# skhu101/TDNN-F_NAS

Hardware: AMD Instinct MI355X
Metric: LF-MMI training frames/sec per node (SWBD 7q TDNN-F) (higher is better)
Workload: dtype f32

## Files before the change

include/tdnnf_hip.h:

```cpp
#ifndef TDNNF_HIP_H_
#define TDNNF_HIP_H_

#include <stddef.h>
#include <stdint.h>

#ifdef __cplusplus
extern "C" {
#endif

#define TDNNF_OK 0
#define TDNNF_EINVAL 1
#define TDNNF_EHIP 2

#define TDNNF_MAX_OFFSETS 16

typedef struct {
  float *data;
  int rows, cols, stride;
} tdnnf_mat;

typedef void *tdnnf_stream;
typedef struct tdnnf_ng tdnnf_ng;

const char *tdnnf_last_error(void);
int tdnnf_abi_version(void);
int tdnnf_set_option(const char *name, int value);
int tdnnf_get_option(const char *name, int *value_out);

#define TDNNF_DARTS_USE_GUMBEL 1
#define TDNNF_DARTS_FREE_SELECT 2
#define TDNNF_DARTS_UNIFORM_SAMPLE 4
#define TDNNF_DARTS_USE_ENTROPY 8
#define TDNNF_DARTS_UPDATE_ALPHA 16

typedef struct {
  int row_stride;
  int num_offsets;
  int row_offsets[TDNNF_MAX_OFFSETS];
} tdnnf_tdnn_indexes;


int tdnnf_tdnn_darts_coef(const float *log_alpha_dev, int K, int flags, float temp_proportion,
                          const float *gumbel_u_dev, const float *sample_u_dev, int share_index,
                          float *coef_memo_dev, float *eff_coef_dev, tdnnf_stream stream);

int tdnnf_tdnn_propagate(const tdnnf_tdnn_indexes *indexes, const tdnnf_mat *in,
                         const float *linear_params_dev, int ldw, int Do, int Di,
                         const float *bias_dev, const float *eff_coef_dev, int init_mode,
                         tdnnf_mat *out, tdnnf_stream stream);

int tdnnf_tdnn_backprop_data(const tdnnf_tdnn_indexes *indexes, const tdnnf_mat *out_deriv,
                             const float *linear_params_dev, int ldw, int Do, int Di,
                             const float *eff_coef_dev, tdnnf_mat *in_deriv, tdnnf_stream stream);

size_t tdnnf_tdnn_update_workspace_bytes(int Do, int Di, int K, int num_rows);
int tdnnf_tdnn_update_simple(const tdnnf_tdnn_indexes *indexes, const tdnnf_mat *in_value,
                             const tdnnf_mat *out_deriv, int Do, int Di,
                             const float *eff_coef_dev, float lr, float *W_acc_dev, int ldw,
                             float *bias_acc_dev, void *workspace_dev, size_t workspace_bytes,
                             tdnnf_stream stream);

#define TDNNF_TAP_DOTS_SLABS 64
#define TDNNF_TAP_DOTS_DOUBLES(K) ((K) * (1 + TDNNF_TAP_DOTS_SLABS))

int tdnnf_tdnn_darts_alpha_update(const float *tap_grad_dev, int ldg, const float *linear_params_dev,
                                  int ldw, int Do, int Di, int K, const float *coef_memo_dev,
                                  int flags, int share_index, float temp_proportion, float lr,
                                  float *alpha_acc_dev, double *tap_dots_dev ,
                                  tdnnf_stream stream);

size_t tdnnf_tdnn_update_natural_gradient_workspace_bytes(int Do, int Di, int K, int num_rows, int has_bias);
int tdnnf_tdnn_update_natural_gradient(const tdnnf_tdnn_indexes *indexes, const tdnnf_mat *in_value,
                                       const tdnnf_mat *out_deriv, int Do, int Di,
                                       const float *linear_params_dev, int ldw_params,
                                       const float *coef_memo_dev, const float *eff_coef_dev, int flags,
                                       int share_index, float temp_proportion,
                                       tdnnf_ng *preconditioner_in, tdnnf_ng *preconditioner_out,
                                       float learning_rate, float *W_acc_dev, int ldw, float *bias_acc_dev,
                                       float *alpha_acc_dev, void *workspace_dev, size_t workspace_bytes,
                                       tdnnf_stream stream);


size_t tdnnf_colreduce_workspace_bytes(int rows, int cols);

int tdnnf_batchnorm_propagate(const tdnnf_mat *in, float epsilon, float target_rms, tdnnf_mat *out,
                              float *memo_dev, void *workspace_dev, size_t workspace_bytes, tdnnf_stream stream);
int tdnnf_batchnorm_backprop(const tdnnf_mat *out_value, const tdnnf_mat *out_deriv, float target_rms,
                             float *memo_dev, tdnnf_mat *in_deriv, void *workspace_dev, size_t workspace_bytes,
                             tdnnf_stream stream);
int tdnnf_batchnorm_store_stats(const float *memo_dev, int D, int num_frames, double *stats_dev,
                                tdnnf_stream stream);
int tdnnf_batchnorm_compute_derived(const double *stats_dev, int D, float epsilon, float target_rms,
                                    float *scale_dev, float *offset_dev, tdnnf_stream stream);
int tdnnf_batchnorm_test_propagate(const tdnnf_mat *in, const float *scale_dev, const float *offset_dev,
                                   tdnnf_mat *out, tdnnf_stream stream);
int tdnnf_batchnorm_test_backprop(const tdnnf_mat *out_deriv, const float *scale_dev, tdnnf_mat *in_deriv,
                                  tdnnf_stream stream);


int tdnnf_softmax_flops_propagate(const tdnnf_mat *in, const float *gumbel_u_dev, float temp_proportion,
                                  tdnnf_mat *out, tdnnf_stream stream);
int tdnnf_softmax_flops_backprop(const tdnnf_mat *out_value, tdnnf_mat *out_deriv, float scale,
                                 const float *flops_dev, int dim, float temp_proportion,
                                 tdnnf_mat *in_deriv, tdnnf_stream stream);
int tdnnf_onehot_propagate(const float *sample_u_dev, tdnnf_mat *out, tdnnf_stream stream);
int tdnnf_onehot_backprop(const tdnnf_mat *out_deriv, float lr, float *output_acc_dev, void *workspace_dev,
                          size_t workspace_bytes, tdnnf_stream stream);
int tdnnf_copyn_propagate(const tdnnf_mat *in, float scale, tdnnf_mat *out, tdnnf_stream stream);
int tdnnf_copyn_backprop(const tdnnf_mat *out_deriv, float scale, tdnnf_mat *in_deriv, tdnnf_stream stream);
int tdnnf_constant_function_propagate(const float *output_dev, tdnnf_mat *out, tdnnf_stream stream);
int tdnnf_constant_function_backprop(const tdnnf_mat *out_deriv, float lr, float *output_acc_dev,
                                     void *workspace_dev, size_t workspace_bytes, tdnnf_stream stream);
int tdnnf_flops_constraint_backprop(const float *flops_dev, float scale, int rows_in, int cols_in,
                                    tdnnf_mat *in_deriv, tdnnf_stream stream);

int tdnnf_elementwise_product_propagate(const tdnnf_mat *in, int output_dim, tdnnf_mat *out, tdnnf_stream);
int tdnnf_elementwise_product_backprop(const tdnnf_mat *in_value, const tdnnf_mat *out_deriv, int output_dim,
                                       tdnnf_mat *in_deriv, tdnnf_stream);
int tdnnf_relu_propagate(const tdnnf_mat *in, tdnnf_mat *out, tdnnf_stream);
int tdnnf_relu_backprop(const tdnnf_mat *out_value, const tdnnf_mat *out_deriv, tdnnf_mat *in_deriv, tdnnf_stream);
int tdnnf_relu_repair(const double *stats_dev, int dim, float self_repair_scale, float lower, float upper,
                      tdnnf_mat *in_deriv, tdnnf_stream);
int tdnnf_relu_store_stats(const tdnnf_mat *out_value, double *stats_dev, void *workspace_dev,
                           size_t workspace_bytes, tdnnf_stream);
int tdnnf_affine_propagate(const tdnnf_mat *in, const float *W_dev, int ldw, const float *bias_dev, int Do,
                           tdnnf_mat *out, tdnnf_stream);
int tdnnf_affine_backprop(const tdnnf_mat *out_deriv, const float *W_dev, int ldw, int Di, tdnnf_mat *in_deriv,
                          tdnnf_stream);
int tdnnf_affine_update_simple(const tdnnf_mat *in_value, const tdnnf_mat *out_deriv, float lr, float *W_acc_dev,
                               int ldw, float *bias_acc_dev, void *workspace_dev, size_t workspace_bytes,
                               tdnnf_stream);
size_t tdnnf_affine_update_natural_gradient_workspace_bytes(int Do, int Di, int num_rows, int has_bias);
int tdnnf_affine_update_natural_gradient(const tdnnf_mat *in_value, const tdnnf_mat *out_deriv,
                                         tdnnf_ng *preconditioner_in, tdnnf_ng *preconditioner_out,
                                         float learning_rate, float *W_acc_dev, int ldw, float *bias_acc_dev,
                                         void *workspace_dev, size_t workspace_bytes, tdnnf_stream);
int tdnnf_log_softmax_propagate(const tdnnf_mat *in, tdnnf_mat *out, tdnnf_stream);
int tdnnf_log_softmax_backprop(const tdnnf_mat *out_value, const tdnnf_mat *out_deriv, tdnnf_mat *in_deriv,
                               tdnnf_stream);
int tdnnf_sum_scaled(const tdnnf_mat *a, float sa, const tdnnf_mat *b, float sb, tdnnf_mat *out, tdnnf_stream);
int tdnnf_add_scaled(const tdnnf_mat *a, float s, tdnnf_mat *out, tdnnf_stream);
int tdnnf_general_dropout(const tdnnf_mat *in, const float *mask_dev, int num_seq, tdnnf_mat *out, tdnnf_stream);
int tdnnf_general_dropout_mask(const float *uniform_dev, long long n, float proportion, int continuous, float *mask_dev, tdnnf_stream);

typedef struct tdnnf_den_graph tdnnf_den_graph;
typedef struct tdnnf_supervision tdnnf_supervision;

int tdnnf_den_graph_create(int num_states, int num_arcs, int num_pdfs, const int *arc_src, const int *arc_dst,
                           const int *arc_pdf, const float *arc_prob, const float *initial_probs, int start_state,
                           tdnnf_den_graph **out);
void tdnnf_den_graph_destroy(tdnnf_den_graph *);
int tdnnf_supervision_create(int num_sequences, int frames_per_sequence, const int *seq_state_begin,
                             const int *seq_arc_begin, const int *state_time, const float *final_logprob,
                             const int *arc_src, const int *arc_dst, const int *arc_pdf, const float *arc_logprob,
                             float weight, tdnnf_supervision **out);
void tdnnf_supervision_destroy(tdnnf_supervision *);
int tdnnf_supervision_info(const tdnnf_supervision *, int *num_states, int *num_arcs, int *max_states_per_frame, int *wide);

int tdnnf_chain_set_denominator_mode(int mode);
int tdnnf_chain_den_mw_status(int *fallbacks, int *disabled, int reset);
size_t tdnnf_chain_workspace_bytes(const tdnnf_den_graph *, int num_sequences, int frames_per_sequence);
int tdnnf_chain_objf_and_deriv(const tdnnf_den_graph *, const tdnnf_supervision *, const tdnnf_mat *nnet_output,
                               const tdnnf_mat *xent_output , float leaky_hmm_coefficient,
                               float l2_regularize, float xent_regularize, double *results_dev,
                               tdnnf_mat *nnet_output_deriv, tdnnf_mat *xent_deriv, void *workspace_dev,
                               size_t workspace_bytes, tdnnf_stream);
int tdnnf_chain_numerator_part(const tdnnf_den_graph *, const tdnnf_supervision *, const tdnnf_mat *nnet_output, int part, double *results_dev,
                               tdnnf_mat *nnet_output_deriv, tdnnf_mat *xent_deriv, void *workspace_dev, size_t workspace_bytes, tdnnf_stream);

int tdnnf_ng_create(int rank, int update_period, float num_samples_history, float alpha, tdnnf_ng **out);
void tdnnf_ng_destroy(tdnnf_ng *);
int tdnnf_ng_freeze(tdnnf_ng *, int freeze);
int tdnnf_ng_precondition(tdnnf_ng *, tdnnf_mat *X, float *scale_host, tdnnf_stream);
size_t tdnnf_ng_stats_pass_workspace_bytes(int rank, int Di, int num_taps, int N);
int tdnnf_ng_stats_pass(const tdnnf_tdnn_indexes *ix, const tdnnf_mat *X, int Di, const float *eff_dev, const float *WT_dev,
                        const float *W_dev, int ldw, const float *bias_dev, tdnnf_mat *H, double *sumsq_dev, int sumsq_cap, int form,
                        void *workspace_dev, size_t workspace_bytes, tdnnf_stream);
const float *tdnnf_ng_scale_dev(const tdnnf_ng *);

size_t tdnnf_constrain_orthonormal_workspace_bytes(int rows, int cols);
int tdnnf_constrain_orthonormal(float scale, float *M_dev, int rows, int cols, int ld, void *workspace_dev,
                                size_t workspace_bytes, tdnnf_stream);
int tdnnf_axpy(const float *x_dev, float a, float *y_dev, size_t n, tdnnf_stream);
int tdnnf_dot(const float *x_dev, const float *y_dev, size_t n, double *result_host, tdnnf_stream);
size_t tdnnf_max_change_workspace_bytes(int num_comp);
int tdnnf_update_with_max_change(float *params_dev, float *delta_dev, int num_comp, const long long *comp_begin_host,
                                 const float *max_change_host, float max_param_change, float max_change_scale,
                                 float scale, int zero_delta, void *workspace_dev, size_t workspace_bytes,
                                 float *info_dev, tdnnf_stream);

int tdnnf_splice_input(const tdnnf_mat *feats, const tdnnf_mat *ivectors, int num_seq, int num_splice,
                       tdnnf_mat *out, tdnnf_stream);
int tdnnf_reorder_rows(const tdnnf_mat *in, int num_seq, int rho, int to_rho, tdnnf_mat *out, tdnnf_stream);

#define TDNNF_NET_MAX_LAYERS 32
typedef struct {
  int feat_dim, ivector_dim, num_pdfs;
  int hidden_dim, prefinal_small_dim;
  int num_layers;
  int bottleneck_dim[TDNNF_NET_MAX_LAYERS];
  int time_stride[TDNNF_NET_MAX_LAYERS];
  float bypass_scale;
  int frames_per_chunk, num_sequences;
  int frame_subsampling;
  float leaky_hmm, xent_regularize, chain_l2_regularize;
  float l2_hidden, l2_output;
// ... 121 lines not shown
```

tdnn-f_nas_amd/csrc/abi_tdnn.hip:

```cpp
#include <dlfcn.h>
#include <stdlib.h>
#include <string.h>

#include <string>

#include "common.h"
#include "gemm_f32.h"
#include "planes_gemm.h"

namespace tdnnf {

static thread_local std::string g_last_error;

void set_error(const char *fmt, ...) {
  char buf[1024];
  va_list ap;
  va_start(ap, fmt);
  vsnprintf(buf, sizeof(buf), fmt, ap);
  va_end(ap);
  g_last_error = buf;
}
int hip_status(hipError_t e, const char *what) {
  set_error("HIP error %d (%s) in %s", (int)e, hipGetErrorString(e), what);
  return TDNNF_EHIP;
}

Options &options() {
  static Options o;
  return o;
}

namespace {
typedef int (*roctx_push_t)(const char *);
typedef int (*roctx_pop_t)();
roctx_push_t g_roctx_push = nullptr;
roctx_pop_t g_roctx_pop = nullptr;
bool roctx_ready() {
  static const bool ok = [] {
    const char *e = getenv("TDNNF_ROCTX");
    if (e && atoi(e) == 0) return false;
    for (const char *lib : {"librocprofiler-sdk-roctx.so", "librocprofiler-sdk-roctx.so.1", "libroctx64.so", "libroctx64.so.4"}) {
      void *h = dlopen(lib, RTLD_NOW | RTLD_GLOBAL);
      if (!h) continue;
      g_roctx_push = (roctx_push_t)dlsym(h, "roctxRangePushA");
      g_roctx_pop = (roctx_pop_t)dlsym(h, "roctxRangePop");
      if (g_roctx_push && g_roctx_pop) return true;
    }
    return false;
  }();
  return ok;
}
}
TraceRange::TraceRange(const char *name) : on(roctx_ready()) {
  if (on) g_roctx_push(name);
}
TraceRange::~TraceRange() {
  if (on) g_roctx_pop();
}

static bool tdnn_rows_ok(const tdnnf_tdnn_indexes *ix, int rows_in, int N) {
  if (!ix || ix->num_offsets < 1 || ix->num_offsets > TDNNF_MAX_OFFSETS || ix->row_stride < 1) return false;
  for (int i = 0; i < ix->num_offsets; i++) {
    const long long need = (long long)ix->row_offsets[i] + (long long)ix->row_stride * N - (ix->row_stride - 1);
    if (ix->row_offsets[i] < 0 || (N > 0 && rows_in < need)) return false;
  }
  return true;
}

}

using namespace tdnnf;

extern "C" {

const char *tdnnf_last_error(void) { return g_last_error.c_str(); }
int tdnnf_abi_version(void) { return 1; }

static int *option_slot(const char *name) {
  Options &o = options();
  if (!name) return nullptr;
  const struct { const char *n; int *p; } table[] = {{"ng_grouped", &o.ng_grouped}, {"ng_fuse", &o.ng_fuse}, {"ng_early_in", &o.ng_early_in},
                                                     {"wgrad_stream", &o.wgrad_stream}, {"gemm_ring", &o.gemm_ring}, {"planes", &o.planes}, {"den_split", &o.den_split}, {"phase_events", &o.phase_events}, {"wgrad_lag", &o.wgrad_lag}, {"ng_bk", &o.ng_bk}, {"ng_valu", &o.ng_valu}, {"ng_pform", &o.ng_pform}, {"planes_group", &o.planes_group}, {"xent_behind_den", &o.xent_behind_den}, {"ng_early_fork", &o.ng_early_fork}, {"ng_diag_skip", &o.ng_diag_skip}, {"wgrad_small", &o.wgrad_small}, {"splitk_per_cu", &o.splitk_per_cu}, {"gemm_alt_taps", &o.gemm_alt_taps}, {"reverse_passes", &o.reverse_passes}, {"splitk_partial_round", &o.splitk_partial_round}, {"wgrad_on_caller", &o.wgrad_on_caller}, {"den_mw_test_abort", &o.den_mw_test_abort}, {"planes_check_bound", &o.planes_check_bound}, {"den_gamma_pairs", &o.den_gamma_pairs}, {"num_form", &o.num_form}, {"num_frontier_cap", &o.num_frontier_cap}};
  for (auto &e : table)
    if (strcmp(e.n, name) == 0) return e.p;
  return nullptr;
}
int tdnnf_set_option(const char *name, int value) {
  int *p = option_slot(name);
  TDNNF_REQUIRE(p, "set_option: unknown option '%s' (ng_grouped, ng_fuse, ng_early_in, wgrad_stream, gemm_ring, planes, den_split)", name ? name : "(null)");
  *p = value;
  return TDNNF_OK;
}
int tdnnf_get_option(const char *name, int *value) {
  int *p = option_slot(name);
  TDNNF_REQUIRE(p && value, "get_option: unknown option '%s'", name ? name : "(null)");
  *value = *p;
  return TDNNF_OK;
}

}

namespace tdnnf {
int tdnn_propagate_impl(const tdnnf_tdnn_indexes *ix, const tdnnf_mat *in, const float *W, int ldw, int Do, int Di,
                        const float *bias, const float *eff_coef, int init_mode, int relu, tdnnf_mat *out, tdnnf_stream stream,
                        float *colstats, int *colstats_rows) {
  TDNNF_REQUIRE(mat_ok(in) && mat_ok(out) && W, "tdnn_propagate: bad matrices");
  TDNNF_REQUIRE(Do > 0 && Di > 0 && in->cols == Di && out->cols == Do, "tdnn_propagate: dims: in.cols=%d Di=%d out.cols=%d Do=%d",
                in ? in->cols : -1, Di, out ? out->cols : -1, Do);
  TDNNF_REQUIRE(tdnn_rows_ok(ix, in->rows, out->rows), "tdnn_propagate: input has too few rows for the time offsets");
  TDNNF_REQUIRE(ldw >= ix->num_offsets * Di, "tdnn_propagate: ldw < K*Di");
  TDNNF_REQUIRE(init_mode >= 0 && init_mode <= 2 && (init_mode != 1 || bias), "tdnn_propagate: init_mode 1 needs a bias");
  RowsGemmArgs a;
  memset(&a, 0, sizeof(a));
  a.A = in->data;
  a.lda = (long long)in->stride * ix->row_stride;
  a.B = W;
  a.ldb = ldw;
  a.C = out->data;
  a.ldc = out->stride;
  a.M = out->rows;
  a.N = Do;
  a.bias = bias;
  a.coef = eff_coef;
  a.init_mode = init_mode;
  a.relu = relu;
  a.colstats = colstats;
  a.colstats_rows = colstats_rows;
  a.nseg = ix->num_offsets;
  for (int i = 0; i < a.nseg; i++) {
    a.seg[i].a_off = (long long)ix->row_offsets[i] * in->stride;
    a.seg[i].b_off = (long long)i * Di;
    a.seg[i].klen = Di;
    a.seg[i].m_lo = 0;
    a.seg[i].m_hi = out->rows;
  }
  TDNNF_HIP(rows_gemm(a, true, (hipStream_t)stream));
  return TDNNF_OK;
}
}

extern "C" {

int tdnnf_tdnn_propagate(const tdnnf_tdnn_indexes *ix, const tdnnf_mat *in, const float *W, int ldw, int Do, int Di,
                         const float *bias, const float *eff_coef, int init_mode, tdnnf_mat *out, tdnnf_stream stream) {
  return tdnn_propagate_impl(ix, in, W, ldw, Do, Di, bias, eff_coef, init_mode, 0, out, stream);
}

}

namespace tdnnf {
int tdnn_backprop_data_impl(const tdnnf_tdnn_indexes *ix, const tdnnf_mat *out_deriv, const float *W, int ldw, int Do,
                            int Di, const float *eff_coef, int overwrite, const tdnnf_mat *add, float add_scale, int add_lo,
                            tdnnf_mat *in_deriv, tdnnf_stream stream) {
  TDNNF_REQUIRE(mat_ok(in_deriv) && mat_ok(out_deriv) && W, "tdnn_backprop_data: bad matrices");
  TDNNF_REQUIRE(Do > 0 && Di > 0 && in_deriv->cols == Di && out_deriv->cols == Do, "tdnn_backprop_data: bad dims");
  TDNNF_REQUIRE(tdnn_rows_ok(ix, in_deriv->rows, out_deriv->rows), "tdnn_backprop_data: in_deriv has too few rows for the time offsets");
  TDNNF_REQUIRE(ldw >= ix->num_offsets * Di, "tdnn_backprop_data: ldw < K*Di");
  const int rho = ix->row_stride, N = out_deriv->rows, K = ix->num_offsets;
  if (N == 0) return TDNNF_OK;
  for (int cls = 0; cls < rho; cls++) {
    RowsGemmArgs a;
    memset(&a, 0, sizeof(a));
    float cf_dummy = 0;
    (void)cf_dummy;
    int nseg = 0, u_max = 0;
    int seg_tap[kMaxSeg];
    for (int i = 0; i < K; i++) {
      if (ix->row_offsets[i] % rho != cls) continue;
      const int shift = (ix->row_offsets[i] - cls) / rho;
      a.seg[nseg].a_off = -(long long)shift * out_deriv->stride;
      a.seg[nseg].b_off = (long long)i * Di;
      a.seg[nseg].klen = Do;
      a.seg[nseg].m_lo = shift;
      a.seg[nseg].m_hi = shift + N;
      if (shift + N > u_max) u_max = shift + N;
      seg_tap[nseg] = i;
      nseg++;
    }
    if (nseg == 0) continue;
    bool contiguous = true;
    for (int s = 1; s < nseg; s++) contiguous = contiguous && seg_tap[s] == seg_tap[s - 1] + 1;
    a.A = out_deriv->data;
    a.lda = out_deriv->stride;
    a.B = W;
    a.ldb = ldw;
    const float *WT = (ldw == K * Di && !planes_hint_b()) ? transposed_weights(W) : nullptr;
    if (WT) {
      a.B = WT;
      a.ldb = Do;
      for (int sg = 0; sg < nseg; sg++) a.seg[sg].b_off = (long long)seg_tap[sg] * Di * Do;
    }
    a.C = in_deriv->data + (long long)cls * in_deriv->stride;
    a.ldc = (long long)in_deriv->stride * rho;
    a.M = u_max;
    a.N = Di;
    a.init_mode = 0;
    if (overwrite) {
      TDNNF_REQUIRE(rho == 1 && u_max == in_deriv->rows, "tdnn_backprop_data: overwrite needs row_stride 1 and full row coverage");
      a.init_mode = 2;
    }
    if (add) {
      TDNNF_REQUIRE(rho == 1 && add->cols == Di && add_lo >= 0 && add_lo + add->rows <= in_deriv->rows, "tdnn_backprop_data: bad addend");
      a.add = add->data;
      a.ldadd = add->stride;
      a.add_scale = add_scale;
      a.add_lo = add_lo;
      a.add_hi = add_lo + add->rows;
    }
    TDNNF_REQUIRE(!(overwrite || add) || !eff_coef || contiguous, "tdnn_backprop_data: fused overwrite/addend needs a single launch");
    if (!eff_coef || contiguous) {
      a.coef = eff_coef ? eff_coef + seg_tap[0] : nullptr;
      a.nseg = nseg;
      TDNNF_HIP(rows_gemm(a, WT != nullptr, (hipStream_t)stream));
    } else {
      for (int s = 0; s < nseg; s++) {
        RowsGemmArgs b = a;
        b.seg[0] = a.seg[s];
        b.nseg = 1;
        b.coef = eff_coef + seg_tap[s];
        b.M = a.seg[s].m_hi;
        TDNNF_HIP(rows_gemm(b, WT != nullptr, (hipStream_t)stream));
      }
    }
  }
  return TDNNF_OK;
}
}

extern "C" {

int tdnnf_tdnn_backprop_data(const tdnnf_tdnn_indexes *ix, const tdnnf_mat *out_deriv, const float *W, int ldw, int Do,
                             int Di, const float *eff_coef, tdnnf_mat *in_deriv, tdnnf_stream stream) {
  return tdnn_backprop_data_impl(ix, out_deriv, W, ldw, Do, Di, eff_coef, 0, nullptr, 0.f, 0, in_deriv, stream);
}

size_t tdnnf_tdnn_update_workspace_bytes(int Do, int Di, int K, int num_rows) {
  return wgrad_workspace_bytes(Do, Di, K, num_rows);
}

}

namespace tdnnf {
int tdnn_update_simple_impl(const tdnnf_tdnn_indexes *ix, const tdnnf_mat *in_value, const tdnnf_mat *out_deriv, int Do,
                            int Di, const float *eff_coef, float lr, float *W_acc, int ldw, float *bias_acc, void *ws,
                            size_t ws_bytes, const int *active_dev, int max_active, tdnnf_stream stream, bool overwrite) {
  TDNNF_REQUIRE(mat_ok(in_value) && mat_ok(out_deriv) && W_acc, "tdnn_update_simple: bad matrices");
  TDNNF_REQUIRE(Do > 0 && Di > 0 && in_value->cols == Di && out_deriv->cols == Do, "tdnn_update_simple: bad dims");
  TDNNF_REQUIRE(tdnn_rows_ok(ix, in_value->rows, out_deriv->rows), "tdnn_update_simple: in_value has too few rows for the time offsets");
  TDNNF_REQUIRE(ldw >= ix->num_offsets * Di, "tdnn_update_simple: ldw < K*Di");
  if (out_deriv->rows == 0) return TDNNF_OK;
  TDNNF_REQUIRE(ws && ws_bytes >= wgrad_workspace_bytes(Do, Di, ix->num_offsets, out_deriv->rows), "tdnn_update_simple: workspace too small");
  WgradArgs a;
  memset(&a, 0, sizeof(a));
  a.dY = out_deriv->data;
  a.lddy = out_deriv->stride;
  a.X = in_value->data;
  a.ldx = in_value->stride;
  a.Do = Do;
  a.Di = Di;
  a.K = ix->num_offsets;
  a.N = out_deriv->rows;
  a.row_stride = ix->row_stride;
  for (int i = 0; i < a.K; i++) a.row_offsets[i] = ix->row_offsets[i];
  a.coef = eff_coef;
  a.scale = lr;
  a.G = W_acc;
  a.ldg = ldw;
  a.accumulate = overwrite ? 0 : 1;
  a.bias_acc = bias_acc;
  a.active = active_dev;
  a.max_active = max_active;
  TDNNF_HIP(wgrad(a, ws, ws_bytes, (hipStream_t)stream));
  return TDNNF_OK;
}
}

extern "C" {

int tdnnf_tdnn_update_simple(const tdnnf_tdnn_indexes *ix, const tdnnf_mat *in_value, const tdnnf_mat *out_deriv, int Do,
                             int Di, const float *eff_coef, float lr, float *W_acc, int ldw, float *bias_acc, void *ws,
                             size_t ws_bytes, tdnnf_stream stream) {
  return tdnn_update_simple_impl(ix, in_value, out_deriv, Do, Di, eff_coef, lr, W_acc, ldw, bias_acc, ws, ws_bytes, nullptr, 0, stream);
}

int tdnnf_affine_propagate(const tdnnf_mat *in, const float *W, int ldw, const float *bias, int Do, tdnnf_mat *out,
                           tdnnf_stream stream) {
  TDNNF_REQUIRE(mat_ok(in) && mat_ok(out) && W && Do > 0 && out->cols == Do && in->rows == out->rows && ldw >= in->cols,
                "affine_propagate: bad arguments");
  tdnnf_tdnn_indexes ix;
  memset(&ix, 0, sizeof(ix));
  ix.row_stride = 1;
  ix.num_offsets = 1;
  return tdnnf_tdnn_propagate(&ix, in, W, ldw, Do, in->cols, bias, nullptr, bias ? 1 : 2, out, stream);
}

int tdnnf_affine_backprop(const tdnnf_mat *out_deriv, const float *W, int ldw, int Di, tdnnf_mat *in_deriv, tdnnf_stream stream) {
  TDNNF_REQUIRE(mat_ok(out_deriv) && mat_ok(in_deriv) && W && Di > 0 && in_deriv->cols == Di && in_deriv->rows == out_deriv->rows && ldw >= Di,
                "affine_backprop: bad arguments");
  if (out_deriv->rows == 0) return TDNNF_OK;
  RowsGemmArgs a;
  memset(&a, 0, sizeof(a));
  a.A = out_deriv->data;
  a.lda = out_deriv->stride;
  a.B = W;
  a.ldb = ldw;
  const float *WT = (ldw == Di && !planes_hint_b()) ? transposed_weights(W) : nullptr;
  if (WT) {
    a.B = WT;
    a.ldb = out_deriv->cols;
  }
  a.C = in_deriv->data;
  a.ldc = in_deriv->stride;
  a.M = out_deriv->rows;
  a.N = Di;
  a.init_mode = 2;
  a.nseg = 1;
  a.seg[0].klen = out_deriv->cols;
  a.seg[0].m_lo = 0;
  a.seg[0].m_hi = out_deriv->rows;
  TDNNF_HIP(rows_gemm(a, WT != nullptr, (hipStream_t)stream));
  return TDNNF_OK;
}

int tdnnf_affine_update_simple(const tdnnf_mat *in_value, const tdnnf_mat *out_deriv, float lr, float *W_acc, int ldw,
                               float *bias_acc, void *ws, size_t ws_bytes, tdnnf_stream stream) {
  TDNNF_REQUIRE(mat_ok(in_value) && mat_ok(out_deriv) && in_value->rows == out_deriv->rows, "affine_update_simple: bad matrices");
  tdnnf_tdnn_indexes ix;
  memset(&ix, 0, sizeof(ix));
  ix.row_stride = 1;
  ix.num_offsets = 1;
  return tdnnf_tdnn_update_simple(&ix, in_value, out_deriv, out_deriv->cols, in_value->cols, nullptr, lr, W_acc, ldw,
                                  bias_acc, ws, ws_bytes, stream);
}

}
```

tdnn-f_nas_amd/csrc/common.h:

```cpp
#pragma once
#include <hip/hip_runtime.h>
#include <stdarg.h>
#include <stdio.h>

#include "tdnnf_hip.h"

namespace tdnnf {

struct MatView {
  float *data;
  int rows, cols, stride;
};
inline MatView view(const tdnnf_mat *m) { return MatView{m->data, m->rows, m->cols, m->stride}; }

void set_error(const char *fmt, ...);
int hip_status(hipError_t e, const char *what);

inline bool mat_ok(const tdnnf_mat *m) {
  return m && m->rows >= 0 && m->cols >= 0 && m->stride >= m->cols && (m->data || m->rows * m->cols == 0);
}
inline bool same_dim(const tdnnf_mat *a, const tdnnf_mat *b) { return a->rows == b->rows && a->cols == b->cols; }

inline bool vec4_ok(const MatView &m) {
  return (reinterpret_cast<uintptr_t>(m.data) & 15) == 0 && m.stride % 4 == 0 && m.cols % 4 == 0;
}

#define TDNNF_REQUIRE(cond, ...)            \
  do {                                      \
    if (!(cond)) {                          \
      ::tdnnf::set_error(__VA_ARGS__);      \
      return TDNNF_EINVAL;                  \
    }                                       \
  } while (0)

#define TDNNF_HIP(expr)                                         \
  do {                                                          \
    hipError_t e__ = (expr);                                    \
    if (e__ != hipSuccess) return ::tdnnf::hip_status(e__, #expr); \
  } while (0)

#define TDNNF_LAUNCH_CHECK(name) TDNNF_HIP(hipGetLastError())

struct Options {
  int ng_grouped = 1;
  int ng_fuse = 1;
  int ng_early_in = 1;
  int wgrad_stream = -1;
  int gemm_ring = 1;
  int planes = 1;
  int den_mw_test_abort = 0;
  int planes_group = 1;
  int planes_check_bound = 0;
  int wgrad_lag = 3;
  int wgrad_on_caller = 0;
  int splitk_partial_round = 1;
  int reverse_passes = 0;
  int gemm_alt_taps = 1;
  int splitk_per_cu = 2;
  int wgrad_small = 0;
  int ng_bk = 0;
  int ng_early_fork = 1;
  int xent_behind_den = -1;
  int ng_pform = 1;
  int ng_valu = 0;
  int ng_diag_skip = 0;
  int phase_events = 0;
  int den_split = -1;
  int num_form = 0;
  int num_frontier_cap = 0;
  int den_gamma_pairs = 0;
};
Options &options();

struct TraceRange {
  explicit TraceRange(const char *name);
  ~TraceRange();
  bool on;
};

__host__ __device__ inline float floor_keep_nan(float x, float f) { return x < f ? f : x; }

inline int grid_for(long long work, int block, int cap = 2048) {
  long long g = (work + block - 1) / block;
  if (g > cap) g = cap;
  if (g < 1) g = 1;
  return (int)g;
}

inline unsigned long long tdnnf_decision(unsigned long long step, unsigned long long k) {
  unsigned long long z = step * 0x9E3779B97F4A7C15ULL + k * 0xBF58476D1CE4E5B9ULL + 0x94D049BB133111EBULL;
  z = (z ^ (z >> 30)) * 0xBF58476D1CE4E5B9ULL;
  z = (z ^ (z >> 27)) * 0x94D049BB133111EBULL;
  return (z ^ (z >> 31)) >> 8;
}

constexpr int kFinCols = 8, kFinLanes = 32, kFinThreads = kFinCols * kFinLanes;
inline unsigned finalize_grid(int D) { return (unsigned)((D + kFinCols - 1) / kFinCols); }
#ifdef __HIPCC__
template <int NQ, class Acc>
__device__ __forceinline__ void finalize_sums(const float *partial, int chunks, long long qstride_rows, int D, int nq, Acc (&q)[NQ], Acc *red) {
  const int tc = threadIdx.x & (kFinCols - 1), lane = threadIdx.x / kFinCols, d = blockIdx.x * kFinCols + tc;
#pragma unroll
  for (int k = 0; k < NQ; k++) q[k] = 0;
  if (d < D) {
    const float *p = partial + d;
    const long long qs = qstride_rows * D;
    int c = lane;
    for (; c + 3 * kFinLanes < chunks; c += 4 * kFinLanes) {
      float v[NQ][4];
#pragma unroll
      for (int k = 0; k < NQ; k++) {
        if (k < nq) {
          const float *pk = p + (long long)k * qs;
          v[k][0] = pk[(long long)c * D]; v[k][1] = pk[(long long)(c + kFinLanes) * D];
          v[k][2] = pk[(long long)(c + 2 * kFinLanes) * D]; v[k][3] = pk[(long long)(c + 3 * kFinLanes) * D];
        }
      }
#pragma unroll
      for (int k = 0; k < NQ; k++) {
        if (k < nq) { q[k] += v[k][0]; q[k] += v[k][1]; q[k] += v[k][2]; q[k] += v[k][3]; }
      }
    }
    for (; c < chunks; c += kFinLanes) {
      float v[NQ];
#pragma unroll
      for (int k = 0; k < NQ; k++)
        if (k < nq) v[k] = p[(long long)k * qs + (long long)c * D];
#pragma unroll
      for (int k = 0; k < NQ; k++)
        if (k < nq) q[k] += v[k];
    }
  }
#pragma unroll
  for (int k = 0; k < NQ; k++) red[(k * kFinLanes + lane) * (kFinCols + 1) + tc] = q[k];
  __syncthreads();
  if (lane == 0) {
#pragma unroll
    for (int k = 0; k < NQ; k++) {
      Acc s = 0;
      for (int l = 0; l < kFinLanes; l++) s += red[(k * kFinLanes + l) * (kFinCols + 1) + tc];
      q[k] = s;
    }
  }
}
#endif

struct BnSync {
  int (*fn)(void *ctx, double *buf, long long count, tdnnf_stream stream);
  void *ctx;
  double *buf;
  int world;
};
BnSync *bn_sync_current();
struct BnSyncScope {
  BnSync *prev;
  explicit BnSyncScope(BnSync *b);
  ~BnSyncScope();
};

struct FroBoundScope {
  double *prev_buf;
  int *prev_blocks;
  FroBoundScope(double *buf, int *blocks);
  ~FroBoundScope();
};
double *fro_bound_buf();
int *fro_bound_blocks();

struct ColReducePlan {
  int chunks, rows_per_chunk;
};
ColReducePlan colreduce_plan(int rows, int cols);
size_t colreduce_bytes(int rows, int cols);
hipError_t colreduce_partial(int kind, MatView a, MatView b, float *partial, hipStream_t s);
hipError_t colreduce_partial_into(int kind, MatView a, MatView b, int chunks, int rows_per_chunk, int sq_row_offset, float *partial, hipStream_t s);
hipError_t batchnorm_stats_from_partials(const float *partial, int chunks, int rows, int cols, float epsilon, float target_rms, float *memo, hipStream_t s,
                                         double *store_stats = nullptr);
hipError_t batchnorm_stats(MatView a, float epsilon, float target_rms, float *memo, void *ws, hipStream_t s, double *store_stats = nullptr);
hipError_t colsum_add(MatView a, float scale, float *acc, void *ws, hipStream_t s);

bool log_softmax_propagate_with_aux(const tdnnf_mat *in, tdnnf_mat *out, tdnnf_mat *aux, float aux_scale, hipStream_t s);
float chain_supervision_weight(const tdnnf_supervision *sp);
size_t chain_split_region_bytes(const tdnnf_den_graph *g, int B, int T);
int chain_den(const tdnnf_den_graph *g, const tdnnf_supervision *sp, const tdnnf_mat *y, float leaky, tdnnf_mat *deriv, void *ws, hipStream_t s,
              bool beside_other_work = false, hipStream_t caller_aux = nullptr, hipEvent_t ev_recursions = nullptr, bool *ev_recorded = nullptr);
int chain_num_recursion(const tdnnf_supervision *sp, const tdnnf_den_graph *g, const tdnnf_mat *y, void *ws, hipStream_t s);
int chain_num_xent(const tdnnf_den_graph *g, const tdnnf_supervision *sp, const tdnnf_mat *y, const tdnnf_mat *xent_output, float xent_regularize,
                   tdnnf_mat *xent_deriv, void *ws, hipStream_t s, bool xent_deriv_initialised = false);
int chain_num(const tdnnf_den_graph *g, const tdnnf_supervision *sp, const tdnnf_mat *y, const tdnnf_mat *xent_output,
              float xent_regularize, tdnnf_mat *xent_deriv, void *ws, hipStream_t s, bool xent_deriv_initialised = false);
int chain_finish(const tdnnf_den_graph *g, const tdnnf_supervision *sp, const tdnnf_mat *y, float l2_regularize, double *results,
                 tdnnf_mat *deriv, tdnnf_mat *xent_deriv, void *ws, hipStream_t s);

int tdnn_propagate_impl(const tdnnf_tdnn_indexes *ix, const tdnnf_mat *in, const float *W, int ldw, int Do, int Di,
                        const float *bias, const float *eff_coef, int init_mode, int relu, tdnnf_mat *out, tdnnf_stream stream,
                        float *colstats = nullptr, int *colstats_rows = nullptr);
int tdnn_update_simple_impl(const tdnnf_tdnn_indexes *ix, const tdnnf_mat *in_value, const tdnnf_mat *out_deriv, int Do, int Di,
                            const float *eff_coef, float lr, float *W_acc, int ldw, float *bias_acc, void *ws, size_t ws_bytes,
                            const int *active_dev, int max_active, tdnnf_stream stream, bool overwrite = false);
int tdnn_backprop_data_impl(const tdnnf_tdnn_indexes *ix, const tdnnf_mat *out_deriv, const float *W, int ldw, int Do, int Di,
                            const float *eff_coef, int overwrite, const tdnnf_mat *add, float add_scale, int add_lo,
                            tdnnf_mat *in_deriv, tdnnf_stream stream);

}
```

tdnn-f_nas_amd/csrc/fused.h:

```cpp
#pragma once
#include "common.h"

namespace tdnnf {

struct PlanesSink {
  void *P;
  long long R;
  const float *rec;
};
hipError_t bn_apply_bypass(MatView x, const float *memo, int D, int period, MatView prev, float bypass, MatView out, hipStream_t s,
                           const float *mask = nullptr, int B = 1, const PlanesSink *planes = nullptr);

struct BwdPlanes {
  void *P;
  long long R;
  int lead;
  float *rec;
};

struct NgFuse {
  const float *W;
  int Rp, ldw;
  float *H;
  double *part;
  int part_cap;
};
bool bn_relu_bwd_ng_ok(MatView x, MatView dz, MatView d_aff, int Rp);
bool bn_relu_bwd_ng_pays(int rows);

size_t bn_relu_bwd_workspace_bytes(int rows, int cols);
hipError_t bn_relu_bwd(MatView x, MatView dz, float *memo, float target_rms, bool bn_test_mode, double *relu_stats, bool store_relu_stats,
                       bool self_repair, float self_repair_scale, MatView d_aff, float *bias_acc, float bias_scale,
                       void *ws, size_t ws_bytes, hipStream_t s, const float *mask = nullptr, int B = 1,
                       const NgFuse *ng = nullptr,
                       double *oderiv_stats = nullptr,
                       const BwdPlanes *planes = nullptr);

}
```

tdnn-f_nas_amd/csrc/fused.hip:

```cpp
#include <algorithm>

#include "common.h"
#include "device.h"
#include "fused.h"
#include "gemm_f32.h"
#include "planes_gemm.h"

namespace tdnnf {
namespace {

__device__ __forceinline__ void ld(const float *p, float (&v)[4], bool vec) {
  if (vec) {
    const float4 t = *reinterpret_cast<const float4 *>(p);
    v[0] = t.x; v[1] = t.y; v[2] = t.z; v[3] = t.w;
  } else {
    v[0] = p[0];
  }
}
__device__ __forceinline__ void st(float *p, const float (&v)[4], bool vec) {
  if (vec) *reinterpret_cast<float4 *>(p) = make_float4(v[0], v[1], v[2], v[3]);
  else p[0] = v[0];
}

__device__ __forceinline__ void store_planes4(const PlanesSink &pk, float ps, long long ra, int c, const float (&v)[4]) {
// ... 277 lines not shown
      wv[j] = make_float4(0.f, 0.f, 0.f, 0.f);
      if (n < ng.Rp) wv[j] = *reinterpret_cast<const float4 *>(ng.W + (long long)n * ng.ldw + k0 + kk);
    }
  };
  request(0);
  for (int k0 = 0; k0 < D; k0 += BK) {
    const int col = k0 + c4 * 4;
    const float4 mu = mu_n, sc = sc_n, vdm = vdm_n, tmp = tmp_n;
    float rep[4] = {0.f, 0.f, 0.f, 0.f};
    if (repairing) {
#pragma unroll
      for (int j = 0; j < 4; j++) {
        const float stv = (float)stv_n[j];
        const float v = (stv - 0.05f * count > 0.f ? 1.f : 0.f) + (stv - 0.95f * count > 0.f ? 1.f : 0.f) - 1.f;
        rep[j] = v * (-self_repair_scale / 0.5f);
      }
    }
    const float mu_[4] = {mu.x, mu.y, mu.z, mu.w}, sc_[4] = {sc.x, sc.y, sc.z, sc.w}, vdm_[4] = {vdm.x, vdm.y, vdm.z, vdm.w},
                tmp_[4] = {tmp.x, tmp.y, tmp.z, tmp.w};
    float cs[4] = {0.f, 0.f, 0.f, 0.f};
    float o[4][4];
#pragma unroll
    for (int i = 0; i < 4; i++) {
      const int r = r0 + rr + 32 * i;
#pragma unroll
      for (int j = 0; j < 4; j++) o[i][j] = 0.f;
      if (FULL || r < x.rows) {
        if (MASK) {
          const float *mk = mask + (long long)(r % B) * x.cols + col;
#pragma unroll
          for (int j = 0; j < 4; j++) dv[i][j] *= mk[j];
        }
#pragma unroll
        for (int j = 0; j < 4; j++) {
          const float z = (xv[i][j] - mu_[j]) * sc_[j];
          const float dr = (dv[i][j] + tmp_[j]) * sc_[j] + z * vdm_[j];
          float v = (xv[i][j] > 0.f ? 1.f : 0.f) * dr;
          if (rep[j] != 0.f) v += rep[j];
          o[i][j] = v;
          cs[j] += v;
          ssq += v * v;
        }
      }
      *reinterpret_cast<float4 *>(As + (rr + 32 * i) * LD + c4 * 4) = make_float4(o[i][0], o[i][1], o[i][2], o[i][3]);
    }
#pragma unroll
    for (int j = 0; j < NT; j++) {
      const int idx = t + 256 * j, n = idx >> 3, kk = (idx & 7) * 4;
      *reinterpret_cast<float4 *>(Bs + n * LD + kk) = wv[j];
    }
    if (k0 + BK < D) request(k0 + BK);
#pragma unroll
    for (int i = 0; i < 4; i++) {
      const int r = r0 + rr + 32 * i;
      if (FULL || r < x.rows) {
        st(d_aff.data + (long long)r * d_aff.stride + col, o[i], true);
        if constexpr (PLANES) store_planes4(pk, pks, (long long)pk_lead + r, col, o[i]);
      }
    }
#pragma unroll
    for (int j = 0; j < 4; j++) {
      float v = cs[j];
      v += __shfl_xor(v, 8, 64);
      v += __shfl_xor(v, 16, 64);
      v += __shfl_xor(v, 32, 64);
      if (lane < 8) colred[wave][lane * 4 + j] = v;
    }
    __syncthreads();
    {
      const float *as = As + (wave * 32 + li) * LD + lh * 4;
      const float *bs = Bs + li * LD + lh * 4;
#pragma unroll
      for (int kg = 0; kg < BK / 8; kg++) {
        const float4 a = *reinterpret_cast<const float4 *>(as + kg * 8);
#pragma unroll
        for (int j = 0; j < NT; j++) {
          const float4 b = *reinterpret_cast<const float4 *>(bs + j * 32 * LD + kg * 8);
          acc[j] = __builtin_amdgcn_mfma_f32_32x32x2f32(a.x, b.x, acc[j], 0, 0, 0);
          acc[j] = __builtin_amdgcn_mfma_f32_32x32x2f32(a.y, b.y, acc[j], 0, 0, 0);
          acc[j] = __builtin_amdgcn_mfma_f32_32x32x2f32(a.z, b.z, acc[j], 0, 0, 0);
          acc[j] = __builtin_amdgcn_mfma_f32_32x32x2f32(a.w, b.w, acc[j], 0, 0, 0);
        }
      }
    }
    if (t < BK) partial[(long long)blk * D + k0 + t] = (colred[0][t] + colred[1][t]) + (colred[2][t] + colred[3][t]);
    __syncthreads();
  }
#pragma unroll
  for (int j = 0; j < NT; j++) {
    const int n = j * 32 + li;
#pragma unroll
    for (int e = 0; e < 16; e++) {
      const int r = r0 + wave * 32 + (e & 3) + 8 * (e >> 2) + 4 * lh;
      if (n < ng.Rp && r < x.rows) ng.H[(long long)r * ng.Rp + n] = acc[j][e];
    }
  }
  double v = ssq;
  for (int o = 32; o > 0; o >>= 1) v += __shfl_xor(v, o, 64);
  if (lane == 0) red[wave] = v;
  __syncthreads();
  if (t == 0) ng.part[blk] = (red[0] + red[1]) + (red[2] + red[3]);
  if (blk == 0)
    for (int i = gridDim.x + t; i < ng.part_cap; i += 256) ng.part[i] = 0.0;
}

template <int NT, bool MASK, bool PLANES>
__global__ __launch_bounds__(256) void bn_relu_bwd_apply_ng_kernel(MatView x, MatView dz, const float *memo, int D, const double *repair_stats,
                                                                   float self_repair_scale, MatView d_aff, float *partial, const float *mask, int B,
                                                                   NgFuse ng, PlanesSink pk, int pk_lead, int rev) {
  const int blk = rev ? (int)gridDim.x - 1 - (int)blockIdx.x : (int)blockIdx.x;
  if (blk * 128 + 128 <= x.rows)
    bn_relu_bwd_apply_ng_body<NT, MASK, true, PLANES>(x, dz, memo, D, repair_stats, self_repair_scale, d_aff, partial, mask, B, ng, pk, pk_lead, blk);
  else bn_relu_bwd_apply_ng_body<NT, MASK, false, PLANES>(x, dz, memo, D, repair_stats, self_repair_scale, d_aff, partial, mask, B, ng, pk, pk_lead, blk);
}

__global__ __launch_bounds__(kFinThreads) void colsum_add_kernel(const float *partial, int chunks, int D, float scale, float *acc) {
  __shared__ float red[kFinLanes * (kFinCols + 1)];
  const int d = blockIdx.x * kFinCols + (threadIdx.x & (kFinCols - 1));
  float q[1];
  finalize_sums<1, float>(partial, chunks, chunks, D, 1, q, red);
  if (threadIdx.x < kFinCols && d < D) acc[d] += scale * q[0];
}

}

hipError_t bn_apply_bypass(MatView x, const float *memo, int D, int period, MatView prev, float bypass, MatView out, hipStream_t s, const float *mask, int B,
                           const PlanesSink *planes) {
  if (x.rows == 0) return hipSuccess;
  const bool vec = vec4_ok(x) && vec4_ok(out) && (!prev.data || vec4_ok(prev)) && D % 4 == 0 && (reinterpret_cast<uintptr_t>(memo) & 15) == 0 &&
                   (!mask || (reinterpret_cast<uintptr_t>(mask) & 15) == 0);
  const long long work = (long long)x.rows * (vec ? x.cols / 4 : x.cols);
  if (planes && !(vec && x.cols == D && D % 32 == 0 && planes->P && planes->rec)) return hipErrorInvalidValue;
  ProfHbmRange prof(4, 4.0 * x.rows * x.cols * ((prev.data ? 3.0 : 2.0) + (planes ? 1.0 : 0.0)), s);
  const PlanesSink none{nullptr, 0, nullptr};
  if (planes) hipLaunchKernelGGL((bn_apply_bypass_kernel<4, true>), dim3(grid_for((long long)((x.rows + 7) / 8) * 8 * (x.cols / 4), 256)), dim3(256), 0, s, x, memo, memo + 2 * D, D, period, prev, bypass, out, mask, B, *planes, 0);
  else if (vec) hipLaunchKernelGGL((bn_apply_bypass_kernel<4, false>), dim3(grid_for(work, 256)), dim3(256), 0, s, x, memo, memo + 2 * D, D, period, prev, bypass, out, mask, B, none, options().reverse_passes & 1);
  else hipLaunchKernelGGL((bn_apply_bypass_kernel<1, false>), dim3(grid_for(work, 256)), dim3(256), 0, s, x, memo, memo + 2 * D, D, period, prev, bypass, out, mask, B, none, 0);
  return hipGetLastError();
}

bool bn_relu_bwd_ng_ok(MatView x, MatView dz, MatView d_aff, int Rp) {
  return vec4_ok(x) && vec4_ok(dz) && vec4_ok(d_aff) && x.cols % 32 == 0 && Rp >= 1 && Rp <= 96 && x.rows >= 1;
}

bool bn_relu_bwd_ng_pays(int rows) {
  const int slots = 2 * device_cus();
  const int blocks = (rows + 127) / 128, rounds = (blocks + slots - 1) / slots;
  return 4 * blocks >= 3 * rounds * slots;
}

size_t bn_relu_bwd_workspace_bytes(int rows, int cols) {
  ColReducePlan p = colreduce_plan(rows, cols);
  const size_t blocks128 = ((size_t)rows + 127) / 128;
  return sizeof(float) * (5 * (size_t)p.chunks + std::max((size_t)p.chunks, blocks128)) * cols + 64;
}

hipError_t bn_relu_bwd(MatView x, MatView dz, float *memo, float target_rms, bool bn_test_mode, double *relu_stats, bool store_relu_stats,
                       bool self_repair, float self_repair_scale, MatView d_aff, float *bias_acc, float bias_scale,
                       void *ws, size_t ws_bytes, hipStream_t s, const float *mask, int B, const NgFuse *ng, double *oderiv_stats, const BwdPlanes *planes) {
  if (x.rows == 0) return hipSuccess;
  if (ws_bytes < bn_relu_bwd_workspace_bytes(x.rows, x.cols)) return hipErrorInvalidValue;
  if (ng && (!bn_relu_bwd_ng_ok(x, dz, d_aff, ng->Rp) || (reinterpret_cast<uintptr_t>(memo) & 15) || (reinterpret_cast<uintptr_t>(ng->W) & 15) || ng->ldw % 4))
    return hipErrorInvalidValue;
  const int D = x.cols;
  ProfHbmRange prof(5, 4.0 * x.rows * x.cols * 5.0, s);
  ColReducePlan pl = colreduce_plan(x.rows, D);
  const bool vec = vec4_ok(x) && vec4_ok(dz) && vec4_ok(d_aff);
  const int per = vec ? 256 : 64;
  dim3 grid((D + per - 1) / per, pl.chunks), block(256);
  float *partial = (float *)ws;
  float *bias_partial = partial + 5 * (size_t)pl.chunks * D;
  if (store_relu_stats) {
    if (vec) hipLaunchKernelGGL((bn_relu_bwd_reduce_kernel<4, true>), grid, block, 0, s, x, dz, memo, memo + 2 * D, pl.rows_per_chunk, pl.chunks, partial, mask, B);
    else hipLaunchKernelGGL((bn_relu_bwd_reduce_kernel<1, true>), grid, block, 0, s, x, dz, memo, memo + 2 * D, pl.rows_per_chunk, pl.chunks, partial, mask, B);
  } else {
    if (vec) hipLaunchKernelGGL((bn_relu_bwd_reduce_kernel<4, false>), grid, block, 0, s, x, dz, memo, memo + 2 * D, pl.rows_per_chunk, pl.chunks, partial, mask, B);
    else hipLaunchKernelGGL((bn_relu_bwd_reduce_kernel<1, false>), grid, block, 0, s, x, dz, memo, memo + 2 * D, pl.rows_per_chunk, pl.chunks, partial, mask, B);
  }
  double *fro2 = fro_bound_buf();
  if (fro2 && fro_bound_blocks()) *fro_bound_blocks() = (int)finalize_grid(D);
  const float repair_abs = self_repair ? 2.0f * fabsf(self_repair_scale) : 0.f;
  if (BnSync *sy = bn_test_mode ? nullptr : bn_sync_current()) {
    hipLaunchKernelGGL(bn_relu_bwd_finalize_kernel, dim3(finalize_grid(D)), dim3(kFinThreads), 0, s, partial, pl.chunks, D, x.rows, target_rms, memo,
                       store_relu_stats ? relu_stats : (double *)nullptr, 0, (double *)nullptr, sy->buf, (const double *)nullptr, 0);
    if (sy->fn(sy->ctx, sy->buf, 3LL * D, (tdnnf_stream)s)) return hipErrorUnknown;
    hipLaunchKernelGGL(bn_relu_bwd_finalize_kernel, dim3(finalize_grid(D)), dim3(kFinThreads), 0, s, partial, pl.chunks, D, x.rows * sy->world, target_rms, memo,
                       store_relu_stats ? relu_stats : (double *)nullptr, 0, oderiv_stats, (double *)nullptr, (const double *)sy->buf, x.rows, fro2, repair_abs);
  } else {
    hipLaunchKernelGGL(bn_relu_bwd_finalize_kernel, dim3(finalize_grid(D)), dim3(kFinThreads), 0, s, partial, pl.chunks, D, x.rows, target_rms, memo,
                       store_relu_stats ? relu_stats : (double *)nullptr, bn_test_mode ? 1 : 0, oderiv_stats, (double *)nullptr, (const double *)nullptr, 0, fro2,
                       repair_abs);
  }
  const double *rep = self_repair ? relu_stats : nullptr;
  PlanesSink pk{nullptr, 0, nullptr};
  int pk_lead = 0;
  if (planes && planes->P) {
    if (!(fro2 && vec && x.cols % 16 == 0)) return hipErrorInvalidValue;
    hipError_t e = planes_scale_bound(fro2, (int)finalize_grid(D), (double)x.rows * D, 1.0f, 0.0f, nullptr, planes->rec, s);
    if (e != hipSuccess) return e;
    pk = PlanesSink{planes->P, planes->R, planes->rec};
    pk_lead = planes->lead;
  }
  if (ng) {
    const int blocks = (x.rows + 127) / 128;
#define APPLY_NG(NT)                                                                                                                                     \
  do {                                                                                                                                               \
    if (pk.P && mask) hipLaunchKernelGGL((bn_relu_bwd_apply_ng_kernel<NT, true, true>), dim3(blocks), block, 0, s, x, dz, memo, D, rep, self_repair_scale, d_aff, bias_partial, mask, B, *ng, pk, pk_lead, (options().reverse_passes >> 1) & 1); \
    else if (pk.P) hipLaunchKernelGGL((bn_relu_bwd_apply_ng_kernel<NT, false, true>), dim3(blocks), block, 0, s, x, dz, memo, D, rep, self_repair_scale, d_aff, bias_partial, mask, B, *ng, pk, pk_lead, (options().reverse_passes >> 1) & 1); \
    else if (mask) hipLaunchKernelGGL((bn_relu_bwd_apply_ng_kernel<NT, true, false>), dim3(blocks), block, 0, s, x, dz, memo, D, rep, self_repair_scale, d_aff, bias_partial, mask, B, *ng, pk, pk_lead, (options().reverse_passes >> 1) & 1); \
    else hipLaunchKernelGGL((bn_relu_bwd_apply_ng_kernel<NT, false, false>), dim3(blocks), block, 0, s, x, dz, memo, D, rep, self_repair_scale, d_aff, bias_partial, mask, B, *ng, pk, pk_lead, (options().reverse_passes >> 1) & 1);    \
  } while (0)
    if (ng->Rp <= 32) APPLY_NG(1);
    else if (ng->Rp <= 64) APPLY_NG(2);
    else APPLY_NG(3);
#undef APPLY_NG
    if (bias_acc) hipLaunchKernelGGL(colsum_add_kernel, dim3(finalize_grid(D)), dim3(kFinThreads), 0, s, bias_partial, blocks, D, bias_scale, bias_acc);
    return hipGetLastError();
  }
  if (pk.P) hipLaunchKernelGGL((bn_relu_bwd_apply_kernel<4, true>), grid, block, 0, s, x, dz, memo, D, rep, self_repair_scale, pl.rows_per_chunk, pl.chunks, d_aff, bias_partial, mask, B, pk, pk_lead, (options().reverse_passes >> 1) & 1);
  else if (vec) hipLaunchKernelGGL((bn_relu_bwd_apply_kernel<4, false>), grid, block, 0, s, x, dz, memo, D, rep, self_repair_scale, pl.rows_per_chunk, pl.chunks, d_aff, bias_partial, mask, B, pk, pk_lead, (options().reverse_passes >> 1) & 1);
  else hipLaunchKernelGGL((bn_relu_bwd_apply_kernel<1, false>), grid, block, 0, s, x, dz, memo, D, rep, self_repair_scale, pl.rows_per_chunk, pl.chunks, d_aff, bias_partial, mask, B, pk, pk_lead, (options().reverse_passes >> 1) & 1);
  if (bias_acc) hipLaunchKernelGGL(colsum_add_kernel, dim3(finalize_grid(D)), dim3(kFinThreads), 0, s, bias_partial, pl.chunks, D, bias_scale, bias_acc);
  return hipGetLastError();
}

}
```

tdnn-f_nas_amd/csrc/gemm_f32.h:

```cpp
#pragma once
#include <hip/hip_runtime.h>
#include <stddef.h>
#include <stdint.h>

#include <vector>

#include "prof.h"

namespace tdnnf {

constexpr int kMaxSeg = 16;

struct GemmSeg {
  long long a_off;
  long long b_off;
  int klen;
  int m_lo, m_hi;
};

struct RowsGemmArgs {
  const float *A;
  long long lda;
  const float *B;
  long long ldb;
  float *C;
  long long ldc;
  int M, N;
  const float *bias;
  const float *coef;
  int init_mode;
  int relu;
  int c_vec;
  const float *add;
  long long ldadd;
  float add_scale;
  int add_lo, add_hi;
  int ksplit;
  int kchunk;
  float *partial;
  double *sumsq;
  int sumsq_cap;
  float *colstats;
  int *colstats_rows;
  int colstats_stride;
  int prec;
  int serial_epilogue;
  int alt_seg_order;
  int nseg;
  GemmSeg seg[kMaxSeg];
  const float *col_scale;
  const float *col_offset;
  int post_add;
  const int *row_map;
};
inline bool rows_gemm_has_post(const RowsGemmArgs &a) { return a.col_scale || a.col_offset || a.post_add || a.row_map; }

struct SplitKScratchOverride {
  float *prev_buf;
  size_t prev_bytes;
  SplitKScratchOverride(float *buf, size_t bytes);
  ~SplitKScratchOverride();
};

struct GemmPrecisionScope {
  int prev;
  explicit GemmPrecisionScope(int prec);
  ~GemmPrecisionScope();
};
int gemm_precision_default();
struct TransposedWeightsScope {
  const float *prev_w, *prev_wt;
  long long prev_n;
  TransposedWeightsScope(const float *w_base, const float *wt_base, long long n);
  ~TransposedWeightsScope();
};
const float *transposed_weights(const float *W);

inline bool aligned16(const void *p) { return (reinterpret_cast<uintptr_t>(p) & 15) == 0; }

inline int rows_gemm_colstats_cap(int M) { return (M + 63) / 64 + 64; }
inline int rows_gemm_sumsq_blocks(int M) { return (M + 127) / 128 > 1024 ? (M + 127) / 128 : 1024; }

hipError_t rows_gemm(const RowsGemmArgs &args, bool b_kcontig, hipStream_t stream);

struct RowsGemmGroup;
bool rows_gemm_group_ok(const RowsGemmArgs &a);
hipError_t rows_gemm_group(const std::vector<RowsGemmArgs> &calls, RowsGemmGroup **cache, hipStream_t stream);
void rows_gemm_group_destroy(RowsGemmGroup *g);

struct WgradArgs {
  const float *dY;
  long long lddy;
  const float *X;
  long long ldx;
  int Do, Di, K, N;
  int row_stride;
  int row_offsets[kMaxSeg];
  const float *coef;
  float scale;
  float *G;
  long long ldg;
  int accumulate;
  float *bias_acc;
  const int *active;
  int max_active;
  int prec;
  int xcd_order;
};
size_t wgrad_workspace_bytes(int Do, int Di, int K, int N);
hipError_t wgrad(const WgradArgs &args, void *workspace, size_t workspace_bytes, hipStream_t stream);

}
```

tdnn-f_nas_amd/csrc/net_step.hip:

```cpp
#include <math.h>
#include <string.h>

#include <string>
#include <vector>

#include "common.h"
#include "fused.h"
#include "gemm_f32.h"
#include "net.h"
#include "ng.h"

namespace tdnnf {
namespace {

__global__ void add_scaled_taps_kernel(const float *G, const float *coef, float *acc, int Do, int KDi, int Di) {
  const long long total = (long long)Do * KDi;
  for (long long e = blockIdx.x * 256LL + threadIdx.x; e < total; e += gridDim.x * 256LL) acc[e] += coef[(e % KDi) / Di] * G[e];
}
__global__ void scaled_taps_to_kernel(const float *G, const float *coef, int Do, int KDi, int Di, float *T, int ldT) {
  const long long total = (long long)Do * KDi;
  for (long long e = blockIdx.x * 256LL + threadIdx.x; e < total; e += gridDim.x * 256LL) {
    const int o = (int)(e / KDi), c = (int)(e % KDi);
    T[(size_t)o * ldT + c] = (coef ? coef[c / Di] : 1.0f) * G[e];
  }
// ... 125 lines not shown
}

using namespace tdnnf;

namespace {

__global__ void dropout_mask_kernel(const float *u, float p, long long n, float *mask) {
  for (long long i = blockIdx.x * (long long)blockDim.x + threadIdx.x; i < n; i += (long long)gridDim.x * blockDim.x)
    mask[i] = 1.0f - 2.0f * p + 4.0f * p * u[i];
}

__global__ void bn_test_memo_kernel(const double *stats, int D, float epsilon, float target_rms, float *memo) {
  const int d = blockIdx.x * blockDim.x + threadIdx.x;
  if (d >= D) return;
  const double count = stats[0];
  const float off = (float)(stats[1 + d] * (-1.0 / count));
  float sc = (float)(stats[1 + D + d] * (1.0 / count));
  sc += -1.0f * off * off;
  memo[D + d] = sc;
  sc = floor_keep_nan(sc, 0.f) + epsilon;
  sc = target_rms / sqrtf(sc);
  memo[d] = -off;
  memo[2 * D + d] = sc;
  memo[3 * D + d] = 0.f;
  memo[4 * D + d] = 0.f;
}
int bn_test_memo(float *memo, const double *stats, int cols, hipStream_t s) {
  hipLaunchKernelGGL(bn_test_memo_kernel, dim3((cols + 255) / 256), dim3(256), 0, s, stats, cols, 1.0e-3f, 1.0f, memo);
  TDNNF_LAUNCH_CHECK();
  return TDNNF_OK;
}
int bn_fwd(tdnnf_net *n, float *in, float *out, int rows, int cols, float *memo, double *stats, hipStream_t s) {
  tdnnf_mat a = M(in, rows, cols), o = M(out, rows, cols);
  if (n->cfg.cv_update) {
    CK(bn_test_memo(memo, stats, cols, s));
    const MatView none{nullptr, 0, 0, 0};
    TDNNF_HIP(bn_apply_bypass(view(&a), memo, cols, ldpad(cols), none, 0.f, view(&o), s));
    return TDNNF_OK;
  }
  CK(tdnnf_batchnorm_propagate(&a, 1.0e-3f, 1.0f, &o, memo, n->ws, n->ws_bytes, s));
  return tdnnf_batchnorm_store_stats(memo, cols, rows, stats, s);
}
int affine_relu_bn_stats(tdnnf_net *n, const tdnnf_tdnn_indexes *ix, const tdnnf_mat *in, const float *W, int ldw, int Do, int Di, const float *bias,
                         const float *eff, tdnnf_mat *out, float *memo, double *stats, hipStream_t s) {
  if (n->cfg.cv_update) {
    CK(tdnn_propagate_impl(ix, in, W, ldw, Do, Di, bias, eff, 1, 1, out, s));
    return bn_test_memo(memo, stats, Do, s);
  }
  int prows = 0;
  const bool room = n->ws_bytes >= sizeof(float) * 2 * (size_t)Do * rows_gemm_colstats_cap(out->rows);
  CK(tdnn_propagate_impl(ix, in, W, ldw, Do, Di, bias, eff, 1, 1, out, s, room ? (float *)n->ws : nullptr, room ? &prows : nullptr));
  if (prows > 0) TDNNF_HIP(batchnorm_stats_from_partials((const float *)n->ws, prows, out->rows, Do, 1.0e-3f, 1.0f, memo, s, stats));
  else TDNNF_HIP(batchnorm_stats(view(out), 1.0e-3f, 1.0f, memo, n->ws, s, stats));
  return TDNNF_OK;
}
int bn_stats(tdnnf_net *n, float *x, int rows, int cols, float *memo, double *stats, hipStream_t s) {
  if (n->cfg.cv_update) return bn_test_memo(memo, stats, cols, s);
  tdnnf_mat a = M(x, rows, cols);
  TDNNF_HIP(batchnorm_stats(view(&a), 1.0e-3f, 1.0f, memo, n->ws, s, stats));
  return TDNNF_OK;
}

BnChoice bn_choice(const tdnnf_net_config &c) {
  BnChoice bc;
  memset(&bc, 0, sizeof(bc));
  bc.C = c.bn_num_choices;
  bc.mode = c.bn_mode;
  int run = 0;
  for (int k = 0; k < 8; k++) {
    if (k < bc.C) run += c.bn_choice_dims[k];
    bc.cum[k] = run;
  }
  bc.flops_scale = c.bn_flops_scale;
  bc.temp = c.bn_mode == 2 ? c.bn_temp_proportion : 1.0f;
  return bc;
}

bool den_uses_split() { return options().den_split >= 0 ? options().den_split != 0 : true; }

int create_streams_and_events(tdnnf_net *n, const tdnnf_den_graph *den) {
  n->den_split = den_uses_split();
  n->chain_ws_bytes = tdnnf_chain_workspace_bytes(den, n->B, n->Tout) - (n->den_split ? 0 : chain_split_region_bytes(den, n->B, n->Tout));
  TDNNF_HIP(hipMalloc(&n->chain_ws, n->chain_ws_bytes));
  TDNNF_HIP(hipStreamCreateWithFlags(&n->s2, hipStreamNonBlocking));
  TDNNF_HIP(hipEventCreateWithFlags(&n->ev_fork, hipEventDisableTiming));
  TDNNF_HIP(hipEventCreateWithFlags(&n->ev_den, hipEventDisableTiming));
  TDNNF_HIP(hipEventCreateWithFlags(&n->ev_num, hipEventDisableTiming));
  TDNNF_HIP(hipStreamCreateWithFlags(&n->s3, hipStreamNonBlocking));
  TDNNF_HIP(hipEventCreateWithFlags(&n->ev_s3, hipEventDisableTiming));
  TDNNF_HIP(hipEventCreateWithFlags(&n->ev_fin0, hipEventDisableTiming));
  TDNNF_HIP(hipEventCreateWithFlags(&n->ev_fin, hipEventDisableTiming));
  if (n->early_on) {
    TDNNF_HIP(hipEventCreateWithFlags(&n->ev_early_in, hipEventDisableTiming));
    TDNNF_HIP(hipEventCreateWithFlags(&n->ev_early, hipEventDisableTiming));
    n->early.assign(n->comps.size(), tdnnf_net::EarlyIn());
  }
  if (n->early_on && !n->wg_on) TDNNF_HIP(hipStreamCreateWithFlags(&n->s4, hipStreamNonBlocking));
  if (n->wg_on) {
    TDNNF_HIP(hipStreamCreateWithFlags(&n->s4, hipStreamNonBlocking));
    if (n->ws5) TDNNF_HIP(hipStreamCreateWithFlags(&n->s5, hipStreamNonBlocking));
    for (int i = 0; i < 4; i++) TDNNF_HIP(hipEventCreateWithFlags(&n->ev_pg[i], hipEventDisableTiming));
    TDNNF_HIP(hipEventCreateWithFlags(&n->ev_pg_in, hipEventDisableTiming));
  }
  TDNNF_HIP(hipEventCreateWithFlags(&n->ev_ngc, hipEventDisableTiming));
  return TDNNF_OK;
}

enum { kP = 1, kT = 2 };
struct FroBound {
  int blocks = 0;
  float mul = 1.0f, add_coef = 0.0f;
  const float *add_rec = nullptr;
};
const PlanesOperand *hint_of(const PlanesOperand &o) { return o.base ? &o : nullptr; }
int max_off(const Tdnn &td) {
  int m = 0;
  for (int i = 0; i < td.K; i++) m = std::max(m, td.ix.row_offsets[i]);
  return m;
}

struct Step {
  tdnnf_net *const n;
  const tdnnf_mat *const feats, *const ivectors;
  const tdnnf_den_graph *const den;
  const tdnnf_supervision *const sup;
  double *const results;
  const long long step;
  const hipStream_t s;
  const tdnnf_net_config &c = n->cfg;
  const int B = n->B, Hd = c.hidden_dim, S = c.prefinal_small_dim, P = c.num_pdfs, lda_dim = 3 * c.feat_dim + c.ivector_dim;
  const int N0 = N_of(n->g_lda, B), No = n->Tout * B, np = n->planes_np, Ltop = c.num_layers - 1;
  const bool cv = c.cv_update != 0;
  const bool use_ng = c.use_natural_gradient != 0;
  const bool pl_on = np != 0 && !n->wg_on;
  const bool lag3 = n->wg_on && n->wg_lag == 3 && n->dC2 != nullptr;
  const bool early_at_fork = n->early_on && !n->wg_on && !n->early_group && options().ng_early_fork != 0;
  const bool drop = n->dropout_masks && n->dropout_proportion > 0.f;
  const float mask_max = drop ? 1.0f + 2.0f * n->dropout_proportion : 1.0f;
  tdnnf_tdnn_indexes ix1;
  const MatView none{nullptr, 0, 0, 0};
  tdnnf_mat lda_out = M(n->lda_out, N0, lda_dim), pl = M(n->prefinal_l_out, No, S), top;
  tdnnf_mat y = M(n->head[0].y, No, P), dy = M(n->d_y, No, P), dx = M(n->d_xent, No, P), lsm = M(n->xent_logsoftmax, No, P);
  tdnnf_mat d_pl = M(n->d_small, No, S);
  bool early_refresh = false;
  bool darts_coef_done = false;
  std::vector<PlanesSplitArgs> wsplits;
  unsigned long long coin_k = 0, relu_k = 0;
  std::vector<PlanesOperand> po_in = std::vector<PlanesOperand>(n->layers.size()), po_lin = po_in;
  PlanesOperand po_lda, po_top, po_pl, po_b1[2], po_b2[2], po_dpl;
  FroBound fb_next;
  PlanesOperand po_next;
  float *prev = nullptr;
  int fused_comp = -1;
  bool den_joined = false;
  bool caller_used = false;
  float *d_cur = n->dA, *d_next = n->dB;

  Step(tdnnf_net *n_, const tdnnf_mat *feats_, const tdnnf_mat *ivectors_, const tdnnf_den_graph *den_, const tdnnf_supervision *sup_, double *results_,
       long long step_, hipStream_t s_)
      : n(n_), feats(feats_), ivectors(ivectors_), den(den_), sup(sup_), results(results_), step(step_), s(s_) {
    memset(&ix1, 0, sizeof(ix1));
    ix1.row_stride = 1;
    ix1.num_offsets = 1;
  }

  int coin() { return (int)(::tdnnf::tdnnf_decision((unsigned long long)step, 2 * coin_k++) & 1); }
  const float *mask_of(int m) const { return drop ? n->dropout_masks + (size_t)m * B * Hd : nullptr; }
  const PlanesOperand *wplanes(int comp) const { return pl_on && n->pw[comp].P ? &n->pw[comp] : nullptr; }
  float *dC_of(int l) const { return !lag3 ? n->dC : (((Ltop - l) & 1) ? n->dC2 : n->dC); }
  float *dS_of(int l) const { return !lag3 ? nullptr : n->dS[(Ltop - l) & 1]; }
  unsigned side_streams() const { return 1u + (n->wg_two ? 1u : 0u) + (n->s5 ? 1u : 0u); }
  std::vector<tdnnf_ng *> all_ng() const {
    std::vector<tdnnf_ng *> v;
    for (auto *list : {&n->ng_in, &n->ng_out})
      for (tdnnf_ng *g : *list)
        if (g) v.push_back(g);
    return v;
  }
  int wait_last_wgrads(hipStream_t st, unsigned streams) {
    for (unsigned b = 1; b <= streams && b <= n->pg_count; b++) TDNNF_HIP(hipStreamWaitEvent(st, n->ev_pg[(n->pg_count - b) & 3], 0));
    return TDNNF_OK;
  }

  static bool slot_same_shape(tdnnf_net::PlaneSlot &ps, const tdnnf_mat &m, int lead, long long R, int layouts) {
    const long long cfg5[5] = {m.rows, m.cols, lead, R, layouts};
    const bool same = memcmp(cfg5, ps.last, sizeof(cfg5)) == 0;
    memcpy(ps.last, cfg5, sizeof(cfg5));
    return same;
  }
  PlanesOperand slot_operand(const tdnnf_mat &m, const tdnnf_net::PlaneSlot &ps, long long R, int lead, long long kb_alloc) const {
    PlanesOperand o;
    o.base = m.data; o.rows = m.rows; o.cols = m.cols; o.ld = m.stride; o.np = np;
    o.P = ps.P; o.R = R; o.lead = lead; o.kb_alloc = kb_alloc; o.scale = np == 2 ? ps.scale : nullptr;
    return o;
  }
  int split(const tdnnf_mat &m, int lead, int want, PlanesOperand *o, hipStream_t st, const FroBound &fb = FroBound()) {
    *o = PlanesOperand();
    if (!pl_on) return TDNNF_OK;
    auto it = n->plane_slots.find(m.data);
    if (it == n->plane_slots.end() || m.rows <= 0) return TDNNF_OK;
    tdnnf_net::PlaneSlot &ps = it->second;
    if (m.cols >= 1024) want = kP;
    PlanesSplitArgs a;
    a.np = np; a.x = view(&m); a.scale = ps.scale; a.sumsq_ws = n->planes_ws;
    if (np == 2 && fb.blocks > 0 && (fb.add_coef == 0.f || fb.add_rec)) {
      a.fro2_bound = n->fro_buf; a.fro2_blocks = fb.blocks; a.fro_mul = fb.mul; a.add_coef = fb.add_coef; a.add_rec = fb.add_rec;
    }
    lead = (lead + 15) & ~15;
    a.lead = lead;
    a.R = planes_rows_padded((long long)2 * lead + m.rows + 256);
    a.Rt = planes_rows_padded(((m.cols + 255) / 256) * 256LL);
    a.P = (want & kP) ? ps.P : nullptr;
    a.PT = (want & kT) ? ps.PT : nullptr;
    const long long kb_alloc = (planes_kblocks(m.cols) + 15) / 16 * 16;
    TDNNF_REQUIRE(planes_bytes(np, a.R, kb_alloc) <= ps.bytesP && planes_bytes(np, a.Rt, planes_t_kblocks(m.rows)) <= ps.bytesPT,
                  "net_forward_backward: plane slot too small for a %d x %d matrix", m.rows, m.cols);
    a.pads_done = slot_same_shape(ps, m, lead, a.R, want);
    TDNNF_HIP(planes_split(a, st));
    *o = slot_operand(m, ps, a.R, lead, kb_alloc);
    o->P = a.P; o->PT = a.PT; o->Rt = a.Rt;
    return TDNNF_OK;
  }
  int split_weights(int comp, const float *coef, int period, bool group = false) {
    PlanesOperand &o = n->pw[comp];
    if (!o.P) return TDNNF_OK;
    o.base = net_W(n, comp);
    o.coef = coef;
    o.coef_period = period;
    PlanesSplitArgs a;
    a.np = np; a.x = MatView{net_W(n, comp), o.rows, o.cols, o.cols}; a.lead = 0; a.R = o.R; a.P = const_cast<void *>(o.P); a.Rt = o.Rt;
    a.PT = const_cast<void *>(o.PT); a.scale = n->pw_scale[comp]; a.sumsq_ws = n->planes_ws;
    a.col_coef = coef; a.col_coef_period = period;
    o.scale = np == 2 ? n->pw_scale[comp] : nullptr;
    a.pads_done = n->fb_count > 1;
    if (group && options().planes_group && planes_split_group_ok(a)) wsplits.push_back(a);
    else TDNNF_HIP(planes_split(a, s));
    return TDNNF_OK;
  }
  int bwd_planes(const tdnnf_mat &d, int lead, BwdPlanes *bp, PlanesOperand *po) {
    *bp = BwdPlanes{nullptr, 0, 0, nullptr};
    *po = PlanesOperand();
    if (!(pl_on && np == 2 && d.cols % 16 == 0 && d.cols >= 1024)) return TDNNF_OK;
    auto it = n->plane_slots.find(d.data);
    if (it == n->plane_slots.end()) return TDNNF_OK;
    tdnnf_net::PlaneSlot &ps = it->second;
    lead = (lead + 15) & ~15;
    const long long R = planes_rows_padded((long long)2 * lead + d.rows + 256), kb_alloc = (planes_kblocks(d.cols) + 15) / 16 * 16;
    TDNNF_REQUIRE(planes_bytes(np, R, kb_alloc) <= ps.bytesP, "net_forward_backward: plane slot too small for a %d x %d matrix", d.rows, d.cols);
    if (!slot_same_shape(ps, d, lead, R, kP)) TDNNF_HIP(planes_pad(np, ps.P, planes_kblocks(d.cols), R, lead, d.rows, s));
    *bp = BwdPlanes{ps.P, R, lead, ps.scale};
    *po = slot_operand(d, ps, R, lead, kb_alloc);
    return TDNNF_OK;
  }
  int bn_apply_planes(const tdnnf_mat &x, const float *memo, const MatView &byp, float bypass, const tdnnf_mat &out, const float *mask, const FroBound &fb,
                      PlanesOperand *po) {
    *po = PlanesOperand();
    auto it = (pl_on && np == 2 && fb.blocks > 0 && (fb.add_coef == 0.f || fb.add_rec) && out.cols == Hd && out.stride == ldpad(Hd)) ? n->plane_slots.find(out.data)
                                                                                                                                         : n->plane_slots.end();
    if (it == n->plane_slots.end()) {
      TDNNF_HIP(bn_apply_bypass(view(&x), memo, Hd, ldpad(Hd), byp, bypass, view(&out), s, mask, B));
      return TDNNF_OK;
    }
    tdnnf_net::PlaneSlot &ps = it->second;
    const long long R = planes_rows_padded((long long)out.rows + 256), kb_alloc = (planes_kblocks(out.cols) + 15) / 16 * 16;
    TDNNF_REQUIRE(planes_bytes(np, R, kb_alloc) <= ps.bytesP, "net_forward_backward: plane slot too small for a %d x %d matrix", out.rows, out.cols);
    TDNNF_HIP(planes_scale_bound(n->fro_buf, fb.blocks, (double)out.rows * out.cols, fb.mul, fb.add_coef, fb.add_rec, ps.scale, s));
    const bool held = ps.last[0] >= 0;
    if (!slot_same_shape(ps, out, 0, R, kP) && held) {
      TDNNF_HIP(planes_pad(np, ps.P, planes_kblocks(out.cols), R, 0, out.rows, s));
    }
    const PlanesSink sink{ps.P, R, ps.scale};
    TDNNF_HIP(bn_apply_bypass(view(&x), memo, Hd, ldpad(Hd), byp, bypass, view(&out), s, mask, B, &sink));
    if (options().planes_check_bound) TDNNF_HIP(planes_check_bound(view(&out), ps.scale, n->planes_ws, s));
    *po = slot_operand(out, ps, R, 0, kb_alloc);
    return TDNNF_OK;
  }
  int darts_coef(TdnnfLayer &L) {
    for (Tdnn *td : {&L.lin, &L.aff}) {
      const float *u = n->draws + td->draw0;
      CK(tdnnf_tdnn_darts_coef(net_alpha(n, td->comp), td->K, c.darts_flags, c.darts_temp_proportion, u, u + td->K, td->share, td->memo,
                               td->memo + TDNNF_MAX_OFFSETS, s));
      hipLaunchKernelGGL(active_taps_kernel, dim3(1), dim3(64), 0, s, td->memo + TDNNF_MAX_OFFSETS, td->K, td->active);
    }
    return TDNNF_OK;
  }

  int begin() {
    n->fb_count++;
    CK(phase_mark(n, 0, s));
    n->wg_two = false;
    TDNNF_HIP(hipMemsetAsync(n->gtmp, 0, sizeof(float) * (size_t)n->num_params, s));
    if (n->ng_bsum_all && n->ng_bsum_floats) TDNNF_HIP(hipMemsetAsync(n->ng_bsum_all, 0, sizeof(float) * n->ng_bsum_floats, s));
    n->pg_count = 0;
    n->early_any = false;
    n->ng_cur.clear();
    if (!(c.use_natural_gradient && n->s3)) return TDNNF_OK;
    TDNNF_HIP(hipEventRecord(n->ev_fin0, s));
    TDNNF_HIP(hipStreamWaitEvent(n->s3, n->ev_fin0, 0));
    SplitKScratchOverride side_scratch(n->s3_scratch, n->s3_scratch_bytes);
    if (n->ngfin) {
      int did = 0;
      CK(ng_fin_run(n->ngfin, n->s3, false, &did));
      early_refresh = did != 0;
    } else {
      for (tdnnf_ng *g : all_ng()) {
        int did = 0;
// ... 150 lines not shown
  }
  bool early_eligible(int comp, int which) const {
    const auto &E = n->early[comp];
    if (E.done == n->fb_count || (which == 0 && is_head_comp(comp))) return false;
    if (E.recorded != n->fb_count - 1 || !n->ng_in[comp] || !n->ng_out[comp] || ng_dim(n->ng_in[comp]) == 0 || ng_dim(n->ng_out[comp]) == 0) return false;
    return n->comps[comp].lr_factor != 0.f && n->ngc[comp].H_in;
  }
  int launch_early_in(int which) {
    if (!(use_ng && n->early_on)) return TDNNF_OK;
    std::vector<int> who;
    for (int comp = (int)n->comps.size() - 1; comp >= 0; comp--)
      if (early_eligible(comp, which)) who.push_back(comp);
    if (who.empty()) return TDNNF_OK;
    TDNNF_HIP(hipEventRecord(n->ev_early_in, s));
    TDNNF_HIP(hipStreamWaitEvent(n->s4, n->ev_early_in, 0));
    if (early_refresh) TDNNF_HIP(hipStreamWaitEvent(n->s4, n->ev_fin, 0));
    NgInput xin;
    if (n->early_group) {
      std::vector<RowsGemmArgs> calls;
      std::vector<int> grouped;
      for (int comp : who) {
        memcpy(&xin, n->early[comp].xin, sizeof(xin));
        RowsGemmArgs a;
        CK(ng_stats_main_prepare(n->ng_in[comp], xin, n->ngc[comp].H_in, n->ngc[comp].part_in, n->s4, &a));
        if (!rows_gemm_group_ok(a)) continue;
        calls.push_back(a);
        grouped.push_back(comp);
      }
      if (calls.empty()) return TDNNF_OK;
      TDNNF_HIP(rows_gemm_group(calls, &n->early_launch, n->s4));
      for (int comp : grouped) n->early[comp].done = n->fb_count;
    } else {
      SplitKScratchOverride early_scratch(n->s4_scratch, n->s4_scratch_bytes);
      for (int comp : who) {
        memcpy(&xin, n->early[comp].xin, sizeof(xin));
        CK(ng_stats_main(n->ng_in[comp], xin, n->ngc[comp].H_in, n->ngc[comp].part_in, n->ws4, n->ws_bytes, n->s4));
        n->early[comp].done = n->fb_count;
      }
    }
    TDNNF_HIP(hipEventRecord(n->ev_early, n->s4));
    n->early_any = true;
    return TDNNF_OK;
  }

  int forward_heads_and_objective() {
    if (early_at_fork) {
      CK(finish_refreshes());
      CK(launch_early_in(0));
    }
    top = M(prev, No, Hd);
    if (po_next.base == top.data && po_next.rows == top.rows) po_top = po_next;
    else CK(split(top, 0, kP | kT, &po_top, s, fb_next));
    {
      PlanesHintScope ph(hint_of(po_top), wplanes(n->c_prefinal_l));
      CK(tdnnf_affine_propagate(&top, net_W(n, n->c_prefinal_l), Hd, nullptr, S, &pl, s));
    }
    CK(split(pl, 0, kP | kT, &po_pl, s));
    for (int h = 0; h < 2; h++) {
      CK(forward_head(h));
      if (h == 0) CK(fork_objective());
    }
    tdnnf_mat yx = M(n->head[1].y, No, P);
    const bool dense_first = log_softmax_propagate_with_aux(&yx, &lsm, &dx, -c.xent_regularize * chain_supervision_weight(sup), s);
    if (!dense_first) CK(tdnnf_log_softmax_propagate(&yx, &lsm, s));
    TDNNF_HIP(hipStreamWaitEvent(s, n->ev_num, 0));
    CK(chain_num_xent(den, sup, &y, &lsm, c.xent_regularize, &dx, n->chain_ws, s, dense_first));
    if (!dense_first) CK(tdnnf_log_softmax_backprop(&lsm, &dx, &dx, s));
    return phase_mark(n, 2, s);
  }
  int forward_head(int h) {
    auto &H = n->head[h];
    tdnnf_mat ar = M(H.aff_relu, No, Hd), lo = M(H.lin_out, No, S), b1 = M(H.bn1_out, No, Hd), b2 = M(H.bn2_out, No, S), yh = M(H.y, No, P);
    FroBound fb_b1;
    {
      PlanesHintScope ph(hint_of(po_pl), wplanes(H.c_affine));
      FroBoundScope fbs(pl_on ? n->fro_buf : nullptr, &fb_b1.blocks);
      CK(affine_relu_bn_stats(n, &ix1, &pl, net_W(n, H.c_affine), S, Hd, S, net_bias(n, H.c_affine), nullptr, &ar, H.bn1_memo, H.bn1_stats, s));
    }
    CK(bn_apply_planes(ar, H.bn1_memo, none, 0.f, b1, nullptr, fb_b1, &po_b1[h]));
    if (!po_b1[h].base) CK(split(b1, 0, kP | kT, &po_b1[h], s, fb_b1));
    {
      PlanesHintScope ph(hint_of(po_b1[h]), wplanes(H.c_linear));
      CK(tdnnf_affine_propagate(&b1, net_W(n, H.c_linear), Hd, nullptr, S, &lo, s));
    }
    CK(bn_fwd(n, H.lin_out, H.bn2_out, No, S, H.bn2_memo, H.bn2_stats, s));
    CK(split(b2, 0, kP | kT, &po_b2[h], s));
    PlanesHintScope ph(hint_of(po_b2[h]), wplanes(H.c_output));
    return tdnnf_affine_propagate(&b2, net_W(n, H.c_output), S, net_bias(n, H.c_output), P, &yh, s);
  }
  int fork_objective() {
    TraceRange trace_den("chain denominator forward-backward (second stream)");
    TDNNF_HIP(hipEventRecord(n->ev_fork, s));
    TDNNF_HIP(hipStreamWaitEvent(n->s2, n->ev_fork, 0));
    const bool den_split = n->den_split;
    TDNNF_HIP(hipStreamWaitEvent(n->s3, n->ev_fork, 0));
    const int xbd = options().xent_behind_den;
    const bool behind = den_split && (xbd > 0 || (xbd < 0 && !n->wg_on));
    if (behind && !n->ev_den_rec) TDNNF_HIP(hipEventCreateWithFlags(&n->ev_den_rec, hipEventDisableTiming));
    bool rec = false;
    CK(chain_den(den, sup, &y, c.leaky_hmm, &dy, n->chain_ws, n->s2, !den_split, n->s3, behind ? n->ev_den_rec : nullptr, &rec));
    if (rec) TDNNF_HIP(hipStreamWaitEvent(s, n->ev_den_rec, 0));
    TDNNF_HIP(hipEventRecord(n->ev_den, n->s2));
    hipStream_t sn = n->s3;
    if (n->wg_on && den_split) {
      sn = n->s4;
      TDNNF_HIP(hipStreamWaitEvent(sn, n->ev_fork, 0));
    }
    CK(chain_num_recursion(sup, den, &y, n->chain_ws, sn));
    TDNNF_HIP(hipEventRecord(n->ev_num, sn));
    return TDNNF_OK;
  }

  int capture(const std::string &name, const tdnnf_mat &m) {
    if (!n->capture_on) return TDNNF_OK;
    tdnnf_mat *dst = nullptr;
    for (auto &kv : n->named)
      if (kv.first == name) dst = &kv.second;
    if (!dst) {
      float *p = nullptr;
      TDNNF_HIP(hipMalloc((void **)&p, sizeof(float) * (size_t)std::max(1, m.rows) * ldpad(m.cols)));
      n->captured.push_back(p);
      n->named.push_back({name, M(p, m.rows, m.cols)});
      dst = &n->named.back().second;
    }
    TDNNF_REQUIRE(dst->rows == m.rows && dst->cols == m.cols, "net_forward_backward: captured %s changed shape", name.c_str());
    return tdnnf_sum_scaled(&m, 1.0f, nullptr, 0.f, dst, s);
  }
  int out_stats_fuse(int comp, MatView xv, MatView dzv, MatView dv, NgFuse &f) {
    fused_comp = -1;
    if (!c.use_natural_gradient || n->ng_out.empty() || !n->ng_out[comp] || n->comps[comp].lr_factor == 0.f) return 0;
    if (options().ng_fuse == 0) return 0;
    const bool fuse_always = options().ng_fuse == 2;
    auto &C = n->ngc[comp];
    const float *W = nullptr;
    int Rp = 0, ldw = 0;
    CK(ng_external_begin(n->ng_out[comp], dv.cols, &W, &Rp, &ldw, s));
    if (!W || !bn_relu_bwd_ng_ok(xv, dzv, dv, Rp) || !(fuse_always || bn_relu_bwd_ng_pays(dv.rows))) return 0;
    f.W = W; f.Rp = Rp; f.ldw = ldw; f.H = C.H_out; f.part = C.part_out; f.part_cap = rows_gemm_sumsq_blocks(dv.rows);
    fused_comp = comp;
    return 1;
  }
  double *oderiv_of(double *relu_stats, int relu_index) {
    std::vector<char> &nz = *n->oderiv_nonzero;
    if ((int)nz.size() < c.num_layers + 3) nz.resize(c.num_layers + 3, 0);
    const bool skip = nz[relu_index] && ::tdnnf::tdnnf_decision((unsigned long long)step, 2 * (4096 + relu_k)) % 4 == 0;
    relu_k++;
    if (!skip) nz[relu_index] = 1;
    return skip ? nullptr : relu_stats + 1 + 2 * Hd;
  }
  int bn_relu_backward(float *relu_out, const tdnnf_mat &d_in, const tdnnf_mat &d_out, int lead, float *memo, double *relu_stats, float *bias_acc, int comp,
                       int relu_index, const float *mask, FroBound *fb, PlanesOperand *po) {
    const bool store = coin() || step == 0;
    const bool repair = c.relu_self_repair_scale > 0.f && coin();
    tdnnf_mat x = M(relu_out, d_in.rows, Hd);
    NgFuse f;
    const int fuse = out_stats_fuse(comp, view(&x), view(&d_in), view(&d_out), f);
    if (fuse < 0) return TDNNF_EINVAL;
    FroBoundScope fbs(pl_on ? n->fro_buf : nullptr, &fb->blocks);
    BwdPlanes bp{nullptr, 0, 0, nullptr};
    PlanesOperand tmp;
    CK(bwd_planes(d_out, lead, &bp, &tmp));
    TDNNF_HIP(bn_relu_bwd(view(&x), view(&d_in), memo, 1.0f, cv, relu_stats, store, repair, c.relu_self_repair_scale, view(&d_out), bias_acc, 1.0f,
                          n->ws, n->ws_bytes, s, mask, B, fuse ? &f : nullptr, oderiv_of(relu_stats, relu_index), bp.P ? &bp : nullptr));
    if (bp.P) *po = tmp;
    if (bp.P && options().planes_check_bound) TDNNF_HIP(planes_check_bound(view(&d_out), bp.rec, n->planes_ws, s));
    return TDNNF_OK;
  }
  int close_bucket(int key) {
    if (use_ng) CK(ng_close(key));
    for (auto &gb : n->buckets) {
      if (gb.close_key != key) continue;
      hipStream_t cs = s;
      if (!use_ng && n->wg_on && n->pg_count > 0) CK(wait_last_wgrads(s, side_streams()));
      if (use_ng) {
        TDNNF_HIP(hipEventRecord(gb.handoff, s));
        TDNNF_HIP(hipStreamWaitEvent(n->s3, gb.handoff, 0));
        cs = n->s3;
      }
      const long long cnt = gb.end - gb.begin;
      if (cnt > 0)
        hipLaunchKernelGGL(commit_grads_kernel, dim3(grid_for(cnt, 256)), dim3(256), 0, cs, n->grads + gb.begin, n->gtmp + gb.begin, cnt, results);
      TDNNF_HIP(hipEventRecord(gb.ready, cs));
    }
    return TDNNF_OK;
  }
  float *bias_target(int comp) const {
    if (n->comps[comp].lr_factor == 0.f) return nullptr;
    if (!use_ng) return net_Bg(n, comp);
    return n->ngc[comp].bsum;
  }
  int handed_off(hipStream_t sw, bool on_caller) {
    if (!n->wg_on || on_caller) return TDNNF_OK;
    TDNNF_HIP(hipEventRecord(n->ev_pg[n->pg_count & 3], sw));
    const unsigned lag = lag3 ? 3u : 1u;
    if (n->pg_count >= lag) TDNNF_HIP(hipStreamWaitEvent(s, n->ev_pg[(n->pg_count - lag) & 3], 0));
    n->pg_count++;
    return TDNNF_OK;
  }
  int param_grad(int comp, const tdnnf_tdnn_indexes &ix, int K, int Di, int Do, tdnnf_mat *x, tdnnf_mat *dyv, const float *eff, bool bias_done,
                 const int *active, int max_active, bool from_tapgrad) {
    const int ldw = K * Di;
    float *bias_acc = net_Bg(n, comp);
    if (n->comps[comp].lr_factor == 0.f) return TDNNF_OK;
    hipStream_t sw = s;
    void *wsw = n->ws;
    const bool on_caller = n->wg_on && options().wgrad_on_caller != 0 && n->early_any && !den_joined;
    if (on_caller) caller_used = true;
    float *scr = nullptr;
    if (n->wg_on && !on_caller) {
      const int ns = (n->wg_two ? 2 : 1) + (n->s5 ? 1 : 0), k = (int)(n->pg_count % (unsigned)ns);
      const int which = k == 0 ? 0 : (k == 1 && n->wg_two) ? 1 : 2;
      sw = which == 0 ? n->s4 : which == 1 ? n->s2 : n->s5;
      wsw = which == 0 ? n->ws4 : which == 1 ? n->ws2 : n->ws5;
      scr = which == 0 ? n->s4_scratch : which == 1 ? n->s2_scratch : n->s5_scratch;
      TDNNF_HIP(hipEventRecord(n->ev_pg_in, s));
      TDNNF_HIP(hipStreamWaitEvent(sw, n->ev_pg_in, 0));
    }
    SplitKScratchOverride sw_scratch(scr, scr ? n->s4_scratch_bytes : 0);
    if (!use_ng) {
      CK(tdnn_update_simple_impl(&ix, x, dyv, Do, Di, eff, 1.0f, net_Wg(n, comp), ldw, bias_done ? nullptr : bias_acc, wsw, n->ws_bytes, active, max_active, sw));
      return handed_off(sw, on_caller);
    }
    const int N = dyv->rows, ones = bias_acc ? 1 : 0, Dx = ldw + ones, ldT = (Dx + 3) & ~3;
    auto &C = n->ngc[comp];
    TDNNF_REQUIRE(C.T && C.N == N, "net_forward_backward: component %s has no natural-gradient buffers for %d rows", n->comps[comp].name.c_str(), N);
    float *T = C.T;
    const bool grouped = n->ng_grouped && ng_dim(n->ng_in[comp]) != 0 && ng_dim(n->ng_out[comp]) != 0;
    const bool overwrite = !from_tapgrad && !active && eff == nullptr && (ones || ldT == ldw);
    if (!overwrite) TDNNF_HIP(hipMemsetAsync(T, 0, sizeof(float) * (size_t)Do * ldT, sw));
    if (from_tapgrad)
      hipLaunchKernelGGL(scaled_taps_to_kernel, dim3(grid_for((long long)Do * ldw, 256)), dim3(256), 0, sw, n->tapgrad, eff, Do, ldw, Di, T, ldT);
    else
      CK(tdnn_update_simple_impl(&ix, x, dyv, Do, Di, eff, 1.0f, T, ldT, nullptr, wsw, n->ws_bytes, active, max_active, sw, overwrite));
    if (ones) {
      if (!bias_done) TDNNF_HIP(colsum_add(view(dyv), 1.0f, C.bsum, wsw, sw));
      if (!grouped) hipLaunchKernelGGL(set_column_kernel, dim3((Do + 255) / 256), dim3(256), 0, sw, C.bsum, Do, T, ldT, ldw);
    }
    NgInput xin;
    memset(&xin, 0, sizeof(xin));
    xin.x = view(x); xin.ix = ix; xin.Di = Di; xin.ones = ones; xin.N = N; xin.eff = eff; xin.active = active; xin.max_active = max_active;
    static_assert(sizeof(NgInput) <= sizeof(tdnnf_net::EarlyIn::xin), "EarlyIn::xin too small");
    if (n->early_on && n->early[comp].done == n->fb_count) {
      TDNNF_REQUIRE(memcmp(n->early[comp].xin, &xin, sizeof(xin)) == 0, "net_forward_backward: the input of component %s moved between minibatches",
                    n->comps[comp].name.c_str());
      if (n->early_group) {
        TDNNF_HIP(hipStreamWaitEvent(sw, n->ev_early, 0));
        CK(ng_stats_main_finish(n->ng_in[comp], xin, C.H_in, wsw, n->ws_bytes, sw));
      }
    } else {
      CK(ng_stats_main(n->ng_in[comp], xin, C.H_in, C.part_in, wsw, n->ws_bytes, sw));
    }
    if (n->early_on) {
      memcpy(n->early[comp].xin, &xin, sizeof(xin));
      n->early[comp].recorded = n->fb_count;
    }
    NgInput yin;
    memset(&yin, 0, sizeof(yin));
    yin.x = view(dyv); yin.ix.row_stride = 1; yin.ix.num_offsets = 1; yin.Di = Do; yin.N = N;
    if (fused_comp == comp) {
      fused_comp = -1;
      CK(ng_external_end(n->ng_out[comp], yin, C.H_out, wsw, n->ws_bytes, sw));
    } else {
      CK(ng_stats_main(n->ng_out[comp], yin, C.H_out, C.part_out, wsw, n->ws_bytes, sw));
    }
    if (grouped) {
      n->ng_cur.push_back(comp);
      CK(handed_off(sw, on_caller));
      if (from_tapgrad && n->wg_on) TDNNF_HIP(hipStreamWaitEvent(s, n->ev_pg[(n->pg_count - 1) & 3], 0));
      return TDNNF_OK;
    }
    TDNNF_HIP(hipEventRecord(n->ev_ngc, sw));
    TDNNF_HIP(hipStreamWaitEvent(n->s3, n->ev_ngc, 0));
    {
      SplitKScratchOverride side_scratch(n->s3_scratch, n->s3_scratch_bytes);
      CK(ng_stats_side(n->ng_in[comp], C.H_in, C.part_in, n->ng_side_ws, n->ngset_ws_bytes, n->s3));
      CK(ng_stats_side(n->ng_out[comp], C.H_out, C.part_out, n->ng_side_ws, n->ngset_ws_bytes, n->s3));
      CK(ng_project(n->ng_in[comp], n->ng_out[comp], T, Do, Dx, ldT, n->ngTmp, n->s3));
    }
    hipLaunchKernelGGL(ng_commit_kernel, dim3(grid_for((long long)Do * Dx, 256)), dim3(256), 0, n->s3, T, ldT, Do, ldw, ng_scale_dev(n->ng_in[comp]),
                       ng_scale_dev(n->ng_out[comp]), net_Wg(n, comp), bias_acc);
    CK(handed_off(sw, on_caller));
    if (from_tapgrad && n->wg_on) TDNNF_HIP(hipStreamWaitEvent(s, n->ev_pg[(n->pg_count - 1) & 3], 0));
    return TDNNF_OK;
  }
  int ng_close(int key) {
    if (n->ng_cur.empty()) return TDNNF_OK;
    bool closes = false;
    for (auto &gb : n->buckets) closes = closes || gb.close_key == key;
    if (!closes) return TDNNF_OK;
    tdnnf_net::NgBucket *nb = nullptr;
    for (auto &b : n->ng_buckets)
      if (b.key == key) nb = &b;
    if (!nb) {
      std::vector<NgGroupComp> gc;
      for (int comp : n->ng_cur) {
        const CompDesc &cd = n->comps[comp];
        auto &C = n->ngc[comp];
        NgGroupComp g;
        g.in = n->ng_in[comp]; g.out = n->ng_out[comp];
        g.T = C.T; g.Do = cd.rows; g.ldw = cd.cols; g.Dx = cd.cols + (cd.has_bias ? 1 : 0); g.ldT = (g.Dx + 3) & ~3;
        g.bsum = cd.has_bias ? C.bsum : nullptr;
        g.H_in = C.H_in; g.H_out = C.H_out; g.part_in = C.part_in; g.part_out = C.part_out; g.N = C.N;
        g.W_acc = net_Wg(n, comp); g.bias_acc = net_Bg(n, comp);
        gc.push_back(g);
      }
      NgGroup *grp = nullptr;
      CK(ng_group_create(gc, &grp));
      n->ng_buckets.push_back(tdnnf_net::NgBucket{key, n->ng_cur, grp});
      nb = &n->ng_buckets.back();
    }
    TDNNF_REQUIRE(nb->comps == n->ng_cur, "net_forward_backward: the components of gradient bucket %d changed between minibatches", key);
    if (n->wg_on && n->pg_count > 0) {
      CK(wait_last_wgrads(n->s3, side_streams()));
      if (caller_used) {
        TDNNF_HIP(hipEventRecord(n->ev_ngc, s));
        TDNNF_HIP(hipStreamWaitEvent(n->s3, n->ev_ngc, 0));
// ... 22 lines not shown
                           net_Wg(n, td.comp), td.Do, ldw, td.Di);
        if (!bias_done) TDNNF_HIP(colsum_add(view(dyv), 1.0f, net_Bg(n, td.comp), n->ws, s));
        return TDNNF_OK;
      }
    }
    const bool compact = td.darts && (c.darts_flags & TDNNF_DARTS_UNIFORM_SAMPLE) && td.K > 2;
    return param_grad(td.comp, td.ix, td.K, td.Di, td.Do, x, dyv, eff, bias_done, compact ? td.active : nullptr, compact ? 2 : 0, tap_ready);
  }

  int backward_heads() {
    if (!early_at_fork) CK(finish_refreshes());
    if (n->wg_on) CK(launch_early_in(2));
    for (int h = 1; h >= 0; h--) CK(backward_head(h));
    CK(capture("prefinal-l.deriv", d_pl));
    CK(split(d_pl, 0, kP | kT, &po_dpl, s));
    {
      PlanesHintScope ph(hint_of(po_dpl), hint_of(po_top));
      CK(param_grad(n->c_prefinal_l, ix1, 1, Hd, S, &top, &d_pl, nullptr, false, nullptr, 0, false));
    }
    CK(close_bucket(-2));
    return phase_mark(n, 3, s);
  }
  int backward_head(int h) {
    auto &H = n->head[h];
    TraceRange trace_head(h == 0 ? "backward prefinal-chain / output" : "backward prefinal-xent / output-xent");
    if (h == 0) {
      TDNNF_HIP(hipStreamWaitEvent(s, n->ev_den, 0));
      den_joined = true;
      n->wg_two = n->wg_on && n->ws2 != nullptr;
      CK(chain_finish(den, sup, &y, c.chain_l2_regularize, results, &dy, nullptr, n->chain_ws, s));
    }
    tdnnf_mat dout = h == 0 ? dy : dx;
    tdnnf_mat b2 = M(H.bn2_out, No, S), b1 = M(H.bn1_out, No, Hd);
    float *d_b1_buf = !lag3 ? n->dA : dC_of(h == 1 ? Ltop : Ltop - 1), *d_b2_buf = !lag3 ? n->d_small2 : n->dS[h == 1 ? 0 : 1];
    tdnnf_mat d_b2 = M(d_b2_buf, No, S), d_b1 = M(d_b1_buf, No, Hd);
    const std::string hname = h == 0 ? "prefinal-chain" : "prefinal-xent";
    if (h == 1) CK(capture("output-xent.deriv", dout));
    PlanesOperand po_d;
    CK(split(dout, 0, kP | kT, &po_d, s));
    {
      PlanesHintScope ph(hint_of(po_d), hint_of(po_b2[h]));
      CK(param_grad(H.c_output, ix1, 1, S, P, &b2, &dout, nullptr, false, nullptr, 0, false));
    }
    {
      PlanesHintScope ph(hint_of(po_d), wplanes(H.c_output));
      CK(tdnnf_affine_backprop(&dout, net_W(n, H.c_output), S, S, &d_b2, s));
    }
    CK(capture(hname + ".batchnorm2.deriv", d_b2));
    if (cv) CK(tdnnf_batchnorm_test_backprop(&d_b2, H.bn2_memo + 2 * S, &d_b2, s));
    else CK(tdnnf_batchnorm_backprop(&b2, &d_b2, 1.0f, H.bn2_memo, &d_b2, n->ws, n->ws_bytes, s));
    CK(capture(hname + ".linear.deriv", d_b2));
    CK(split(d_b2, 0, kP | kT, &po_d, s));
    {
      PlanesHintScope ph(hint_of(po_d), hint_of(po_b1[h]));
      CK(param_grad(H.c_linear, ix1, 1, Hd, S, &b1, &d_b2, nullptr, false, nullptr, 0, false));
    }
    {
      PlanesHintScope ph(hint_of(po_d), wplanes(H.c_linear));
      CK(tdnnf_affine_backprop(&d_b2, net_W(n, H.c_linear), Hd, Hd, &d_b1, s));
    }
    CK(capture(hname + ".batchnorm1.deriv", d_b1));
    FroBound fb_d;
    CK(bn_relu_backward(H.aff_relu, d_b1, d_b1, 0, H.bn1_memo, H.relu_stats, bias_target(H.c_affine), H.c_affine, c.num_layers + 1 + h, nullptr, &fb_d,
                        &po_d));
    CK(capture(hname + ".affine.deriv", d_b1));
    if (!po_d.base || po_d.base != d_b1.data) CK(split(d_b1, 0, kP | kT, &po_d, s, fb_d));
    {
      PlanesHintScope ph(hint_of(po_d), hint_of(po_pl));
      CK(param_grad(H.c_affine, ix1, 1, S, Hd, &pl, &d_b1, nullptr, true, nullptr, 0, false));
    }
    PlanesHintScope ph_bp(hint_of(po_d), wplanes(H.c_affine));
    if (h == 1) {
      CK(tdnnf_affine_backprop(&d_b1, net_W(n, H.c_affine), S, S, &d_pl, s));
      if (!n->wg_on) CK(launch_early_in(early_at_fork ? 1 : 2));
    } else {
      tdnnf_mat tmp = M(!lag3 ? n->d_small2 : n->dS[0], No, S);
      CK(tdnnf_affine_backprop(&d_b1, net_W(n, H.c_affine), S, S, &tmp, s));
      CK(tdnnf_add_scaled(&tmp, 1.0f, &d_pl, s));
    }
    return TDNNF_OK;
  }
  int backward_trunk() {
    {
      tdnnf_mat d_top = M(d_cur, No, Hd);
      PlanesHintScope ph(hint_of(po_dpl), wplanes(n->c_prefinal_l));
      CK(tdnnf_affine_backprop(&d_pl, net_W(n, n->c_prefinal_l), Hd, Hd, &d_top, s));
    }
    for (int l = c.num_layers - 1; l >= 0; l--) CK(backward_layer(l));
    {
      FroBound fb_d;
      PlanesOperand po_d;
      tdnnf_mat d_aff = M(d_cur, N0, Hd);
      CK(bn_relu_backward(n->t1_relu, d_aff, d_aff, 0, n->t1_bn_memo, n->t1_relu_stats, bias_target(n->tdnn1.comp), n->tdnn1.comp, 0, mask_of(0), &fb_d, &po_d));
      if (!po_d.base) CK(split(d_aff, 0, kT, &po_d, s, fb_d));
      PlanesHintScope ph(hint_of(po_d), hint_of(po_lda));
      CK(param_grad(n->tdnn1.comp, ix1, 1, lda_dim, Hd, &lda_out, &d_aff, nullptr, true, nullptr, 0, false));
    }
    CK(close_bucket(-1));
    return phase_mark(n, 4, s);
  }
  int backward_layer(int l) {
    TdnnfLayer &L = n->layers[l];
    float *in_act = l > 0 ? n->layers[l - 1].noop_out : n->t1_bn;
    const int no = L.aff.rows_out, nl = L.lin.rows_out, ni = N_of(L.gin, B);
    tdnnf_mat d_out = M(d_cur, no, Hd), d_aff = M(dC_of(l), no, Hd);
    const std::string lname = "tdnnf" + std::to_string(l + 2);
    TraceRange trace_layer(("backward " + lname).c_str());
    CK(capture(lname + ".noop.deriv", d_out));
    FroBound fb_daff;
    PlanesOperand po_daff, po_dlin;
    CK(bn_relu_backward(L.relu_out, d_out, d_aff, max_off(L.aff), L.bn_memo, L.relu_stats, bias_target(L.aff.comp), L.aff.comp, 1 + l, mask_of(l + 1), &fb_daff,
                        &po_daff));
    CK(capture(lname + ".affine.deriv", d_aff));
    tdnnf_mat lin = M(L.lin_out, nl, L.bn);
    tdnnf_mat aff_in = L.perm ? M(L.lin_perm, nl, L.bn) : (L.c_arch >= 0 ? M(L.lin_masked, nl, L.bn) : lin);
    const float *lin_eff = L.lin.darts ? L.lin.memo + TDNNF_MAX_OFFSETS : nullptr;
    const float *aff_eff = L.aff.darts ? L.aff.memo + TDNNF_MAX_OFFSETS : nullptr;
    ProfFlopsScale taps_active(L.lin.darts && (c.darts_flags & TDNNF_DARTS_UNIFORM_SAMPLE) && L.lin.K > 2 ? 2.0 / L.lin.K : 1.0);
    if (pl_on && !po_daff.base) CK(split(d_aff, max_off(L.aff), kP | kT, &po_daff, s, fb_daff));
    {
      PlanesHintScope ph(hint_of(po_daff), hint_of(po_lin[l]));
      CK(tdnn_wgrad(L.aff, &aff_in, &d_aff, aff_eff, true));
    }
    PlanesHintScope ph_aff_bp(hint_of(po_daff), wplanes(L.aff.comp));
    tdnnf_mat d_lin = M(lag3 ? (L.perm ? n->d_small2 : dS_of(l)) : n->d_small, nl, L.bn);
    if (L.perm) {
      TDNNF_HIP(hipMemsetAsync(d_lin.data, 0, sizeof(float) * (size_t)nl * d_lin.stride, s));
      CK(tdnnf_tdnn_backprop_data(&L.aff.ix, &d_aff, net_W(n, L.aff.comp), L.aff.K * L.bn, Hd, L.bn, aff_eff, &d_lin, s));
      tdnnf_mat un = M(lag3 ? dS_of(l) : n->d_small2, nl, L.bn);
      CK(tdnnf_reorder_rows(&d_lin, B, L.aff.ix.row_stride, 0, &un, s));
      d_lin = un;
    } else {
      CK(tdnn_backprop_data_impl(&L.aff.ix, &d_aff, net_W(n, L.aff.comp), L.aff.K * L.bn, Hd, L.bn, aff_eff, 1, nullptr, 0.f, 0, &d_lin, s));
    }
    if (L.c_arch >= 0) {
      const int chunks = (nl + 511) / 512;
      hipLaunchKernelGGL(colsum_prod_partial_kernel, dim3((L.bn + 255) / 256, chunks), dim3(256), 0, s, view(&lin), view(&d_lin), 512, (float *)n->ws);
      hipLaunchKernelGGL(bn_choice_backward_kernel, dim3(1), dim3(256), 0, s, bn_choice(c), (const float *)n->ws, chunks, L.arch_p, net_Wg(n, L.c_arch));
      hipLaunchKernelGGL(col_scale_kernel, dim3(grid_for((long long)nl * L.bn, 256)), dim3(256), 0, s, view(&d_lin), L.arch_mask, view(&d_lin));
    }
    CK(capture(lname + ".linear.deriv", d_lin));
    tdnnf_mat in = M(in_act, ni, Hd);
    if (pl_on) CK(split(d_lin, max_off(L.lin), kP | kT, &po_dlin, s));
    {
      PlanesHintScope ph(hint_of(po_dlin), hint_of(po_in[l]));
      CK(tdnn_wgrad(L.lin, &in, &d_lin, lin_eff, false));
    }
    CK(close_bucket(l));
    PlanesHintScope ph_lin_bp(hint_of(po_dlin), wplanes(L.lin.comp));
    tdnnf_mat d_in = M(d_next, ni, Hd);
    tdnnf_mat d_byp = sub_grid_view(d_next, L.gin, L.gout, B, Hd);
    if (d_byp.rows == d_out.rows) {
      const int row0 = (int)((d_byp.data - d_in.data) / d_in.stride);
      CK(tdnn_backprop_data_impl(&L.lin.ix, &d_lin, net_W(n, L.lin.comp), L.lin.K * Hd, L.bn, Hd, lin_eff, 1, &d_out, c.bypass_scale, row0,
                                 &d_in, s));
    } else {
      CK(tdnn_backprop_data_impl(&L.lin.ix, &d_lin, net_W(n, L.lin.comp), L.lin.K * Hd, L.bn, Hd, lin_eff, 1, nullptr, 0.f, 0, &d_in, s));
      tdnnf_mat d_o = tdnnf_mat{d_cur, L.gout.n, d_byp.cols, B * ldpad(Hd)};
      CK(tdnnf_add_scaled(&d_o, c.bypass_scale, &d_byp, s));
    }
    std::swap(d_cur, d_next);
    return TDNNF_OK;
  }
  int join() {
    if (n->wg_on) CK(wait_last_wgrads(s, 3));
    n->wg_two = false;
    if (use_ng) {
      TDNNF_HIP(hipEventRecord(n->ev_s3, n->s3));
      TDNNF_HIP(hipStreamWaitEvent(s, n->ev_s3, 0));
    }
    CK(phase_mark(n, 5, s));
    TDNNF_LAUNCH_CHECK();
    return TDNNF_OK;
  }

  int run() {
    CK(begin());
    BnSyncScope bn_sync_scope(n->bn_sync.fn && !c.cv_update ? &n->bn_sync : nullptr);
    GemmPrecisionScope gemm_arith(c.gemm_precision == 2 ? 3 : c.gemm_precision == 3 ? 4 : c.gemm_precision);
    CK(weight_planes());
    TransposedWeightsScope gemm_wt(n->params, n->paramsT, n->paramsT ? n->num_params : 0);
    CK(transpose_weights());
    TraceRange trace_step("tdnnf_net_forward_backward");
    CK(forward_trunk());
    CK(forward_heads_and_objective());
    CK(backward_heads());
    CK(backward_trunk());
    return join();
  }
};

}

extern "C" {

int tdnnf_net_forward_backward(tdnnf_net *n, const tdnnf_mat *feats, const tdnnf_mat *ivectors, const tdnnf_den_graph *den,
                               const tdnnf_supervision *sup, double *results, long long step, tdnnf_stream stream) {
  TDNNF_REQUIRE(n && n->params && n->grads, "net_forward_backward: call net_set_buffers first");
  TDNNF_REQUIRE(mat_ok(feats) && mat_ok(ivectors) && den && sup && results, "net_forward_backward: bad arguments");
  const tdnnf_net_config &c = n->cfg;
  TDNNF_REQUIRE(feats->rows == n->g_feat.n * n->B && feats->cols == c.feat_dim, "net_forward_backward: feats must be %d x %d (t-major)",
                n->g_feat.n * n->B, c.feat_dim);
  TDNNF_REQUIRE(ivectors->rows == n->B && ivectors->cols == c.ivector_dim, "net_forward_backward: ivectors must be %d x %d", n->B, c.ivector_dim);
  if (!n->chain_ws) CK(create_streams_and_events(n, den));
  return Step(n, feats, ivectors, den, sup, results, step, (hipStream_t)stream).run();
}

int tdnnf_net_phase_times(tdnnf_net *n, double *ms_out, int capacity, int *count) {
  TDNNF_REQUIRE(n && ms_out && count && capacity >= tdnnf_net::kPhases - 1, "net_phase_times: bad arguments (capacity >= 7)");
  *count = 0;
  for (int k = 0; k < tdnnf_net::kPhases; k++)
    if (!n->phase_rec[k]) return TDNNF_OK;
  TDNNF_HIP(hipEventSynchronize(n->ev_phase[tdnnf_net::kPhases - 1]));
  for (int k = 0; k + 1 < tdnnf_net::kPhases; k++) {
    float ms = 0.f;
    TDNNF_HIP(hipEventElapsedTime(&ms, n->ev_phase[k], n->ev_phase[k + 1]));
    ms_out[k] = ms;
  }
  *count = tdnnf_net::kPhases - 1;
  return TDNNF_OK;
}

}
```

tdnn-f_nas_amd/csrc/rows_gemm.hip:

```cpp
#include <algorithm>
#include <cstring>
#include <vector>

#include "common.h"
#include "device.h"
#include "gemm_f32.h"
#include "gemm_ring.h"
#include "planes_gemm.h"
#include "rows_gemm_kernels.h"

namespace tdnnf {
namespace {

float *g_scratch_override = nullptr;
size_t g_scratch_override_bytes = 0;
int g_gemm_prec = 0;
const float *g_tw_w = nullptr, *g_tw_wt = nullptr;
long long g_tw_n = 0;

struct KRange {
  long long ktot;
  bool k4;
};
KRange k_range(const RowsGemmArgs &a) {
  KRange k{0, true};
  for (int i = 0; i < a.nseg; i++) {
    k.ktot += a.seg[i].klen;
    k.k4 = k.k4 && (a.seg[i].klen % 4 == 0 || a.nseg == 1);
  }
  return k;
}
bool is_two_tap_shift(const RowsGemmArgs &a) {
  return a.nseg == 2 && a.seg[0].klen == a.seg[1].klen && a.lda > 0 && a.seg[0].a_off != a.seg[1].a_off && (a.seg[1].a_off - a.seg[0].a_off) % a.lda == 0;
}
int usable_rows(const GemmSeg &sg, int M) {
  const int lo = sg.m_lo > 0 ? sg.m_lo : 0, hi = sg.m_hi < M ? sg.m_hi : M;
  return hi > lo ? hi - lo : 0;
}
bool operands_vec4(const RowsGemmArgs &a) {
  bool vec = aligned16(a.A) && aligned16(a.B) && a.lda % 4 == 0 && a.ldb % 4 == 0;
  for (int i = 0; i < a.nseg; i++) vec = vec && a.seg[i].a_off % 4 == 0 && a.seg[i].b_off % 4 == 0;
  return vec;
}

template <int BM, int BN, int BK>
constexpr size_t rows_lds_bytes(bool b_kc) {
  return sizeof(float) * 2 * (BM * (BK + 4) + (b_kc ? BN * (BK + 4) : BK * (BN + 4)));
}
template <int BM, int BN, int BK, int NP>
constexpr size_t rows_x3_lds_bytes() {
  return sizeof(__bf16) * 2 * NP * (size_t)(BM + BN) * (BK + 8);
}

template <int WM, int WN, int TM, int TN, int BK, int NP, int TAG>
void launch_rows_x3_tagged(dim3 grid, const RowsGemmArgs &a, int ntm, int ntn, hipStream_t s) {
  constexpr int D = 1;
  constexpr size_t lds = rows_x3_lds_bytes<WM * TM * 32, WN * TN * 32, BK, NP>();
  static const bool opted = opt_in_lds(rows_gemm_x3_kernel<WM, WN, TM, TN, BK, NP, D, TAG>, lds);
  (void)opted;
  hipLaunchKernelGGL((rows_gemm_x3_kernel<WM, WN, TM, TN, BK, NP, D, TAG>), grid, dim3(256), lds, s, a, ntm, ntn);
}

template <int WM, int WN, int TM, int TN, int BK, int TAG>
void launch_rows_kernel_tagged(dim3 grid, const RowsGemmArgs &a, int ntm, int ntn, bool b_kc, bool vec, hipStream_t s) {
  constexpr int BM = WM * TM * 32, BN = WN * TN * 32;
  constexpr size_t lds_kc = rows_lds_bytes<BM, BN, BK>(true), lds_nc = rows_lds_bytes<BM, BN, BK>(false);
  static const bool opted = opt_in_lds(rows_gemm_kernel<WM, WN, TM, TN, BK, true, 4, TAG>, lds_kc) && opt_in_lds(rows_gemm_kernel<WM, WN, TM, TN, BK, true, 1, TAG>, lds_kc) &&
                            opt_in_lds(rows_gemm_kernel<WM, WN, TM, TN, BK, false, 4, TAG>, lds_nc) && opt_in_lds(rows_gemm_kernel<WM, WN, TM, TN, BK, false, 1, TAG>, lds_nc);
  (void)opted;
  const dim3 block(256);
  if (b_kc) {
    if (vec) hipLaunchKernelGGL((rows_gemm_kernel<WM, WN, TM, TN, BK, true, 4, TAG>), grid, block, lds_kc, s, a, ntm, ntn);
    else hipLaunchKernelGGL((rows_gemm_kernel<WM, WN, TM, TN, BK, true, 1, TAG>), grid, block, lds_kc, s, a, ntm, ntn);
  } else {
    if (vec) hipLaunchKernelGGL((rows_gemm_kernel<WM, WN, TM, TN, BK, false, 4, TAG>), grid, block, lds_nc, s, a, ntm, ntn);
    else hipLaunchKernelGGL((rows_gemm_kernel<WM, WN, TM, TN, BK, false, 1, TAG>), grid, block, lds_nc, s, a, ntm, ntn);
  }
}
template <int WM, int WN, int TM, int TN, int BK>
void launch_rows_kernel(dim3 grid, const RowsGemmArgs &a, int ntm, int ntn, bool b_kc, bool vec, hipStream_t s) {
  const bool ng = prof_class_override() == 3;
  if (a.prec == 1 && b_kc && vec) {
    if (ng) launch_rows_x3_tagged<WM, WN, TM, TN, BK, 2, 1>(grid, a, ntm, ntn, s);
    else launch_rows_x3_tagged<WM, WN, TM, TN, BK, 2, 0>(grid, a, ntm, ntn, s);
    return;
  }
  if (a.prec == 3 && b_kc && vec) {
    if constexpr (BK == 16) {
      if (ng) launch_rows_x3_tagged<WM, WN, TM, TN, BK, 3, 1>(grid, a, ntm, ntn, s);
      else launch_rows_x3_tagged<WM, WN, TM, TN, BK, 3, 0>(grid, a, ntm, ntn, s);
      return;
    }
  }
  if (ng) launch_rows_kernel_tagged<WM, WN, TM, TN, BK, 1>(grid, a, ntm, ntn, b_kc, vec, s);
  else launch_rows_kernel_tagged<WM, WN, TM, TN, BK, 0>(grid, a, ntm, ntn, b_kc, vec, s);
}

template <int WM, int WN, int TM, int TN>
constexpr bool kRingTile = (WM == 2 && WN == 2 && TM == 2 && TN == 2) || (WM == 4 && WN == 1 && TM == 1 && TN == 5);
inline bool ring_applies(const RowsGemmArgs &a, bool b_kc, bool vec, int tile_cols) {
  return prof_class_override() != 3 && (tile_cols == 128 || rows_gemm_ring_mode() >= 2) && rows_gemm_ring_ok(a, b_kc, vec);
}

template <int WM, int WN, int TM, int TN, int BK>
hipError_t launch_rows(const RowsGemmArgs &a, bool b_kc, bool vec, hipStream_t s) {
  constexpr int BM = WM * TM * 32, BN = WN * TN * 32;
  const int ntm = (a.M + BM - 1) / BM, ntn = (a.N + BN - 1) / BN;
  if constexpr (kRingTile<WM, WN, TM, TN>) {
    if (ring_applies(a, b_kc, vec, BN)) return rows_gemm_ring(a, b_kc, BN, s);
  }
  launch_rows_kernel<WM, WN, TM, TN, BK>(dim3(ntm * ntn), a, ntm, ntn, b_kc, vec, s);
  return hipGetLastError();
}

template <int WM, int WN, int TM, int TN, int BK>
void launch_split_k(RowsGemmArgs at, int ntm, int ntn, int S, long long ktot, float *scratch, bool b_kc, bool vec, hipStream_t s) {
  const long long kt = (ktot + BK - 1) / BK;
  at.kchunk = (int)(((kt + S - 1) / S) * BK);
  at.ksplit = (int)((ktot + at.kchunk - 1) / at.kchunk);
  at.partial = scratch;
  launch_rows_kernel<WM, WN, TM, TN, BK>(dim3(ntm * ntn * at.ksplit), at, ntm, ntn, b_kc, vec, s);
  const long long total = (long long)at.M * at.N;
  hipLaunchKernelGGL(splitk_reduce_kernel, dim3((unsigned)std::min<long long>((total + 255) / 256, 2048)), dim3(256), 0, s, at);
}

template <int WM, int WN, int TM, int TN, int BK>
int rows_slots_per_cu(int prec) {
  int per_cu = (WM * TM == 4 && WN * TN == 4 && BK == 16 && prec == 0) ? 3 : 2;
  if (prec == 3 && WN * TN == 5) per_cu = 1;
  if (WM * TM == 2 && prec == 0) per_cu = 4;
  return per_cu;
}
template <int WM, int WN, int TM, int TN, int BK>
int rows_slots(int prec) {
  return rows_slots_per_cu<WM, WN, TM, TN, BK>(prec) * device_cus();
}

constexpr size_t kScratchDefaultBytes = 64u << 20;
float *splitk_scratch(size_t *bytes) {
  if (g_scratch_override) {
    *bytes = g_scratch_override_bytes;
    return g_scratch_override;
  }
  static float *buf = nullptr;
  static bool tried = false;
  if (!tried) {
    tried = true;
    if (hipMalloc((void **)&buf, kScratchDefaultBytes) != hipSuccess) buf = nullptr;
    (void)hipGetLastError();
  }
  *bytes = kScratchDefaultBytes;
  return buf;
}

template <int WM, int WN, int TM, int TN, int BK>
hipError_t launch_rows_balanced(const RowsGemmArgs &a, bool b_kc, bool vec, int cls, double flops, hipStream_t s) {
  constexpr int BM = WM * TM * 32, BN = WN * TN * 32;
  const int ntm = (a.M + BM - 1) / BM, ntn = (a.N + BN - 1) / BN;
  int slots = rows_slots<WM, WN, TM, TN, BK>((b_kc && vec) ? a.prec : 0);
  if constexpr (kRingTile<WM, WN, TM, TN>) {
    if (ring_applies(a, b_kc, vec, BN)) slots = rows_gemm_ring_slots(BN);
  }
  const int tiles = ntm * ntn;
  const int q = tiles / slots, r = tiles % slots;
  const bool stats = a.colstats != nullptr;
  const auto [ktot, k4] = k_range(a);
  const int main_mt = (q * slots) / ntn;
  float *scratch = nullptr;
  size_t scratch_bytes = 0;
  int S_partial = 0;
  if (!stats && q == 0 && tiles * 4 > slots && k4 && options().splitk_partial_round) {
    const int cus = device_cus();
    const long long kt = (ktot + BK - 1) / BK;
    double best = (double)((tiles + cus - 1) / cus);
    for (int S = 2; S <= 8; S++) {
      if (kt / S < 24) break;
      const double cost = (double)(((long long)tiles * S + cus - 1) / cus) / S + 0.02 * S;
      if (cost < best - 1e-9) {
        best = cost;
        S_partial = S;
      }
    }
  }
  if (!stats && (tiles * 4 <= slots || S_partial >= 2) && k4 && ktot >= 16 * BK && (scratch = splitk_scratch(&scratch_bytes))) {
    const long long kt = (ktot + BK - 1) / BK;
    int S = S_partial >= 2 ? S_partial : slots / tiles;
    if (S_partial < 2 && options().splitk_per_cu == 1) S = std::max(2, device_cus() / tiles);
    if (S > kt / 4) S = (int)(kt / 4);
    const size_t need = sizeof(float) * (size_t)S * a.M * ((a.N + 3) & ~3);
    if (S >= 2 && need <= scratch_bytes) {
      ProfScope ps(cls, flops, s);
      launch_split_k<WM, WN, TM, TN, BK>(a, ntm, ntn, S, ktot, scratch, b_kc, vec, s);
      return hipGetLastError();
    }
  }
  if (q >= 1 && r > 0 && 2 * r <= slots && main_mt > 0 && main_mt < ntm && k4 && ktot >= 8 * BK && (scratch = splitk_scratch(&scratch_bytes))) {
    const int m_main = main_mt * BM;
    RowsGemmArgs am = a;
    am.M = m_main;
    const int tail_rows = a.M - m_main;
    const long long kt_tail = (ktot + BK - 1) / BK;
    const int tail_tiles0 = ((tail_rows + BM - 1) / BM) * ntn;
    int S_tail = slots / tail_tiles0;
    if (S_tail > kt_tail / 2) S_tail = (int)(kt_tail / 2);
    const bool tail_split = S_tail >= 2 && sizeof(float) * (size_t)S_tail * tail_rows * ((a.N + 3) & ~3) <= scratch_bytes;
    ColReducePlan tail_plan = colreduce_plan(tail_rows, a.N);
    if (stats) {
      am.colstats_stride = main_mt + (tail_split ? tail_plan.chunks : (tail_rows + BM - 1) / BM);
      *a.colstats_rows = am.colstats_stride;
    }
    {
      ProfScope ps(cls, flops * m_main / a.M, s);
      hipError_t e = launch_rows<WM, WN, TM, TN, BK>(am, b_kc, vec, s);
      if (e != hipSuccess) return e;
    }
    RowsGemmArgs at = a;
    at.M = a.M - m_main;
    at.A = a.A + (long long)m_main * a.lda;
    at.C = a.C + (long long)m_main * a.ldc;
    for (int i = 0; i < at.nseg; i++) {
      at.seg[i].m_lo -= m_main;
      at.seg[i].m_hi -= m_main;
    }
    at.add_lo -= m_main;
    at.add_hi -= m_main;
    if (stats) {
      at.colstats = a.colstats + (long long)main_mt * a.N;
      at.colstats_stride = am.colstats_stride;
    }
    if (tail_split) {
      {
        ProfScope ps(cls, flops * at.M / a.M, s);
        launch_split_k<WM, WN, TM, TN, BK>(at, (at.M + BM - 1) / BM, ntn, S_tail, ktot, scratch, b_kc, vec, s);
      }
      if (stats) {
        MatView ct{at.C, at.M, at.N, (int)at.ldc};
        hipError_t e = colreduce_partial_into(1, ct, ct, tail_plan.chunks, tail_plan.rows_per_chunk, am.colstats_stride, at.colstats, s);
        if (e != hipSuccess) return e;
      }
      return hipGetLastError();
    }
    ProfScope ps(cls, flops * at.M / a.M, s);
    return launch_rows<WM, WN, TM, TN, BK>(at, b_kc, vec, s);
  }
  ProfScope ps(cls, flops, s);
  if (stats) {
    RowsGemmArgs as = a;
    as.colstats_stride = ntm;
    *a.colstats_rows = ntm;
    return launch_rows<WM, WN, TM, TN, BK>(as, b_kc, vec, s);
  }
  return launch_rows<WM, WN, TM, TN, BK>(a, b_kc, vec, s);
}

template <int WM, int WN, int TM, int TN, int BK>
hipError_t launch_rows_sumsq(const RowsGemmArgs &a, bool b_kc, bool vec, hipStream_t s) {
  constexpr int BM = WM * TM * 32;
  const int tiles = (a.M + BM - 1) / BM, slots = rows_slots<WM, WN, TM, TN, BK>(0);
  const auto [ktot, k4] = k_range(a);
  float *scratch = nullptr;
  size_t scratch_bytes = 0;
  if (tiles * 4 <= slots && k4 && ktot >= 16 * BK && (scratch = splitk_scratch(&scratch_bytes))) {
    const long long kt = (ktot + BK - 1) / BK;
    int S = slots / tiles;
    if (S > kt / 4) S = (int)(kt / 4);
    if (S > 16) S = 16;
    const size_t need = sizeof(float) * (size_t)S * a.M * ((a.N + 3) & ~3);
    if (S >= 2 && need <= scratch_bytes && tiles * S <= a.sumsq_cap) {
      launch_split_k<WM, WN, TM, TN, BK>(a, tiles, 1, S, ktot, scratch, b_kc, vec, s);
      return hipGetLastError();
    }
  }
  return launch_rows<WM, WN, TM, TN, BK>(a, b_kc, vec, s);
}

template <int WM, int WN, int TM, int TN, int BK>
hipError_t launch_rows_post(const RowsGemmArgs &a, bool vec, int cls, double flops, hipStream_t s) {
  constexpr int BM = WM * TM * 32, BN = WN * TN * 32;
  const int ntm = (a.M + BM - 1) / BM, ntn = (a.N + BN - 1) / BN;
  constexpr size_t lds = rows_lds_bytes<BM, BN, BK>(true);
  static const bool opted = opt_in_lds(rows_gemm_post_kernel<WM, WN, TM, TN, BK, 4>, lds) && opt_in_lds(rows_gemm_post_kernel<WM, WN, TM, TN, BK, 1>, lds);
  (void)opted;
  ProfScope ps(cls, flops, s);
  if (vec) hipLaunchKernelGGL((rows_gemm_post_kernel<WM, WN, TM, TN, BK, 4>), dim3(ntm * ntn), dim3(256), lds, s, a, ntm, ntn);
  else hipLaunchKernelGGL((rows_gemm_post_kernel<WM, WN, TM, TN, BK, 1>), dim3(ntm * ntn), dim3(256), lds, s, a, ntm, ntn);
  return hipGetLastError();
}

inline long long floordiv(long long a, long long b) { return a >= 0 ? a / b : -((-a + b - 1) / b); }

bool planes_try_rows(const RowsGemmArgs &a, bool b_kc, int np, double flops, hipStream_t s, hipError_t *err) {
  const PlanesOperand *ha = planes_hint_a(), *hb = planes_hint_b();
  if (!ha || !hb || ha->np != np || hb->np != np || !ha->P || a.sumsq || a.ksplit > 1 || a.nseg > 16) return false;
  if (ha->coef || (a.coef == nullptr) != (hb->coef == nullptr)) return false;
  long long coef_t0 = 0;
  if (a.coef) {
    coef_t0 = a.coef - hb->coef;
    if (coef_t0 < 0 || coef_t0 >= 16 || hb->coef_period <= 0) return false;
  }
  if (a.lda != ha->ld || a.A < ha->base || (a.A - ha->base) % ha->ld != 0) return false;
  const long long arow0 = (a.A - ha->base) / ha->ld;
  const int BM = planes_gemm_tile_rows(a.N), BN = planes_gemm_tile_cols(a.N);
  const long long m_pad = (long long)((a.M + BM - 1) / BM) * BM, n_pad = (long long)((a.N + BN - 1) / BN) * BN;
  PlanesGemmArgs g;
  memset(&g, 0, sizeof(g));
  g.np = np;
  g.A = ha->P; g.RA = ha->R; g.scale_a = ha->scale; g.scale_b = hb->scale;
  if (a.ldb != hb->ld || a.B < hb->base) return false;
  const long long boff0 = a.B - hb->base;
  if (b_kc) {
    if (!hb->P) return false;
    g.B = hb->P; g.RB = hb->R;
  } else {
    if (!hb->PT) return false;
    g.B = hb->PT; g.RB = hb->Rt;
  }
  for (int i = 0; i < a.nseg; i++) {
    const GemmSeg &sg = a.seg[i];
    const long long shift = floordiv(sg.a_off, ha->ld), c0 = sg.a_off - shift * ha->ld;
    if (c0 % 16 != 0 || c0 + sg.klen > ha->cols || sg.klen <= 0) return false;
    const long long first = arow0 + shift;
    const int lo = sg.m_lo > 0 ? sg.m_lo : 0, hi = sg.m_hi < a.M ? sg.m_hi : a.M;
    if (hi <= lo) return false;
    if (first + lo < 0 || first + hi > ha->rows) return false;
    if (lo > 0 && first + lo != 0) return false;
    if (hi < a.M && first + hi != ha->rows) return false;
    if (ha->lead + first < 0 || ha->lead + first + m_pad > ha->R) return false;
    g.seg[i].a_row = ha->lead + first;
    g.seg[i].a_kb0 = (int)(c0 / 16);
    g.seg[i].nkb = (sg.klen + 15) / 16;
    if (sg.klen % 16 != 0 && c0 + sg.klen != ha->cols) return false;
    const long long bo = boff0 + sg.b_off;
    if (b_kc) {
      const long long brow = bo / hb->ld, bc0 = bo % hb->ld;
      if (bo < 0 || bc0 % 16 != 0 || bc0 + sg.klen > hb->cols || brow + a.N > hb->rows || brow + n_pad > hb->R) return false;
      if (sg.klen % 16 != 0 && bc0 + sg.klen != hb->cols) return false;
      if (a.coef && (bc0 % hb->coef_period != 0 || bc0 / hb->coef_period != coef_t0 + i || sg.klen > hb->coef_period)) return false;
      g.seg[i].b_row = brow;
      g.seg[i].b_kb0 = (int)(bc0 / 16);
    } else {
      const long long krow = bo / hb->ld, ncol = bo % hb->ld;
      if (bo < 0 || krow % 16 != 0 || krow + sg.klen > hb->rows || ncol + a.N > hb->cols || ncol + n_pad > hb->Rt) return false;
      if (sg.klen % 16 != 0 && krow + sg.klen != hb->rows) return false;
      if (a.coef && (ncol % hb->coef_period != 0 || ncol / hb->coef_period != coef_t0 + i || a.N > hb->coef_period)) return false;
      g.seg[i].b_row = ncol;
      g.seg[i].b_kb0 = (int)(krow / 16);
    }
  }
  g.nseg = a.nseg;
  g.alt_seg_order = a.alt_seg_order && a.nseg == 2 && g.seg[0].nkb == g.seg[1].nkb && g.seg[0].a_kb0 == g.seg[1].a_kb0 && g.seg[0].a_row != g.seg[1].a_row;
  if (g.alt_seg_order && options().gemm_alt_taps == 2 && g.seg[0].nkb >= 24 && !a.coef) {
    const PlanesSeg s0 = g.seg[0], s1 = g.seg[1];
    const int nchunk = std::min(16, s0.nkb / 6), per = (s0.nkb + nchunk - 1) / nchunk;
    int n = 0;
    for (int c = 0; c < nchunk; c++) {
      const int k0 = c * per, kn = std::min(per, s0.nkb - k0);
      if (kn <= 0) break;
      for (const PlanesSeg *sp : {&s0, &s1}) {
        PlanesSeg q = *sp;
        q.a_kb0 += k0;
        q.b_kb0 += k0;
        q.nkb = kn;
        g.seg[n++] = q;
      }
    }
    g.nseg = n;
    g.alt_seg_order = 0;
  }
  g.skip_coef = a.coef;
  g.C = a.C; g.ldc = a.ldc; g.M = a.M; g.N = a.N;
  g.bias = a.bias; g.init_mode = a.init_mode; g.relu = a.relu;
  g.add = a.add; g.ldadd = a.ldadd; g.add_scale = a.add_scale; g.add_lo = a.add_lo; g.add_hi = a.add_hi;
  ProfScope ps(BN == 160 ? 1 : 0, flops, s);
  g_planes_routed_rows++;
  {
    const int cus = device_cus();
    g.M = a.M;
    g.N = a.N;
    const int BMl = planes_gemm_launch_tile_rows(g);
    const int ntm = (a.M + BMl - 1) / BMl, ntn = (a.N + BN - 1) / BN, tiles = ntm * ntn, slots = cus * (BMl == 128 ? 2 : 1), q = tiles / slots, r = tiles % slots;
    int nkb = 0;
    for (int i = 0; i < g.nseg; i++) nkb += g.seg[i].nkb;
    const int main_mt = (q * slots) / ntn;
    const bool stats = a.colstats && a.colstats_rows && g.init_mode != 0;
    if (stats) {
      g.colstats = a.colstats;
      g.colstats_stride = ntm;
      *a.colstats_rows = ntm;
    }
    size_t scratch_bytes = 0;
    float *scratch = nullptr;
    if (q >= 1 && r > 0 && 2 * r <= slots && main_mt > 0 && main_mt < ntm && nkb >= 48 && BMl == BM && (scratch = splitk_scratch(&scratch_bytes))) {
      const int m_main = main_mt * BM, tail_rows = a.M - m_main, tail_tiles = ((tail_rows + BM - 1) / BM) * ntn;
      int S = std::min(cus / tail_tiles, nkb / 4);
      const long long ldp = (a.N + 3) & ~3;
      if (S >= 2 && sizeof(float) * (size_t)S * tail_rows * ldp <= scratch_bytes) {
        PlanesGemmArgs gm = g;
        gm.M = m_main;
        const ColReducePlan tail_plan = colreduce_plan(tail_rows, a.N);
        if (stats) {
          gm.colstats_stride = main_mt + tail_plan.chunks;
          *a.colstats_rows = gm.colstats_stride;
        }
        *err = planes_gemm(gm, s);
        if (*err != hipSuccess) return true;
        PlanesGemmArgs gt = g;
        gt.colstats = nullptr;
        gt.M = tail_rows;
        gt.C = g.C + (long long)m_main * g.ldc;
        for (int i = 0; i < gt.nseg; i++) gt.seg[i].a_row += m_main;
        if (gt.add) {
          gt.add_lo = g.add_lo - m_main;
          gt.add_hi = g.add_hi - m_main;
          gt.add = g.add;
        }
        const int kbps = (nkb + S - 1) / S;
        gt.ksplit = (nkb + kbps - 1) / kbps;
        gt.kb_per_split = kbps;
        gt.partial = scratch;
        gt.partial_stride = (long long)tail_rows * ldp;
        gt.ldp_m = ldp;
        gt.ldp_n = 1;
        if (gt.ksplit >= 2) {
          *err = planes_gemm(gt, s);
          if (*err == hipSuccess) *err = planes_splitk_finish(gt, s);
        } else {
          gt.ksplit = 0;
          gt.partial = nullptr;
          *err = planes_gemm(gt, s);
        }
        if (stats && *err == hipSuccess) {
          MatView ct{gt.C, tail_rows, a.N, (int)gt.ldc};
          *err = colreduce_partial_into(1, ct, ct, tail_plan.chunks, tail_plan.rows_per_chunk, gm.colstats_stride, a.colstats + (long long)main_mt * a.N, s);
        }
        return true;
      }
    }
  }
  *err = planes_gemm(g, s);
  return true;
}

}

SplitKScratchOverride::SplitKScratchOverride(float *buf, size_t bytes) : prev_buf(g_scratch_override), prev_bytes(g_scratch_override_bytes) {
  g_scratch_override = buf;
  g_scratch_override_bytes = bytes;
}
SplitKScratchOverride::~SplitKScratchOverride() {
  g_scratch_override = prev_buf;
  g_scratch_override_bytes = prev_bytes;
}
GemmPrecisionScope::GemmPrecisionScope(int prec) : prev(g_gemm_prec) { g_gemm_prec = prec; }
GemmPrecisionScope::~GemmPrecisionScope() { g_gemm_prec = prev; }
int gemm_precision_default() { return g_gemm_prec; }
TransposedWeightsScope::TransposedWeightsScope(const float *w_base, const float *wt_base, long long n) : prev_w(g_tw_w), prev_wt(g_tw_wt), prev_n(g_tw_n) {
  g_tw_w = w_base;
  g_tw_wt = wt_base;
  g_tw_n = n;
}
TransposedWeightsScope::~TransposedWeightsScope() {
  g_tw_w = prev_w;
  g_tw_wt = prev_wt;
  g_tw_n = prev_n;
}
const float *transposed_weights(const float *W) {
  if (!g_tw_w || !g_tw_wt || W < g_tw_w || W >= g_tw_w + g_tw_n) return nullptr;
  return g_tw_wt + (W - g_tw_w);
}

hipError_t rows_gemm(const RowsGemmArgs &a_in, bool b_kc, hipStream_t s) {
  if (a_in.M <= 0 || a_in.N <= 0 || a_in.nseg <= 0) return hipSuccess;
  RowsGemmArgs a = a_in;
  a.c_vec = aligned16(a.C) && a.ldc % 4 == 0 && (a.init_mode != 1 || aligned16(a.bias)) && (!a.add || (aligned16(a.add) && a.ldadd % 4 == 0));
  const bool vec = operands_vec4(a);
  const int waste128 = ((a.N + 127) / 128) * 128 - a.N, waste160 = ((a.N + 159) / 160) * 160 - a.N;
  const long long ktot = k_range(a).ktot;
  double flops = 0;
  for (int i = 0; i < a.nseg; i++) flops += 2.0 * usable_rows(a.seg[i], a.M) * a.N * a.seg[i].klen;
  if (prof_on()) {
    double a_elems = 0, b_elems = 0;
    bool taps = true;
    for (int i = 1; i < a.nseg; i++)
      taps = taps && a.seg[i].klen == a.seg[0].klen && a.lda > 0 && (a.seg[i].a_off - a.seg[0].a_off) % a.lda == 0;
    if (taps) {
      long long lo = a.seg[0].a_off, hi = a.seg[0].a_off;
      for (int i = 1; i < a.nseg; i++) {
        lo = std::min(lo, a.seg[i].a_off);
        hi = std::max(hi, a.seg[i].a_off);
      }
      a_elems = ((double)a.M + (double)(hi - lo) / (double)a.lda) * a.seg[0].klen;
    }
    for (int i = 0; i < a.nseg; i++) {
      if (!taps) a_elems += (double)usable_rows(a.seg[i], a.M) * a.seg[i].klen;
      b_elems += (double)a.seg[i].klen * a.N;
    }
    double c_elems = (double)a.M * a.N * (a.init_mode == 0 ? 2.0 : 1.0);
    if (a.add) c_elems += (double)(std::min(a.add_hi, a.M) - std::max(a.add_lo, 0)) * a.N;
    prof_next_gemm(flops, 4.0 * (a_elems + b_elems + c_elems));
  }
  a.serial_epilogue = 0;
  a.alt_seg_order = options().gemm_alt_taps && is_two_tap_shift(a);
  if (rows_gemm_has_post(a)) {
    if (!b_kc || a.init_mode == 0 || a.sumsq || a.ksplit > 1 || (a.init_mode == 1 && !a.bias)) return hipErrorInvalidValue;
    a.prec = 0;
    a.colstats = nullptr;
    if (a.colstats_rows) *a.colstats_rows = 0;
    a.c_vec = a.c_vec && (!a.col_scale || aligned16(a.col_scale)) && (!a.col_offset || aligned16(a.col_offset));
    if (waste160 < waste128) return launch_rows_post<4, 1, 1, 5, 16>(a, vec, 1, flops, s);
    if ((long long)((a.M + 127) / 128) * ((a.N + 127) / 128) < 768) return launch_rows_post<2, 2, 1, 2, 16>(a, vec, 0, flops, s);
    if (ktot <= 512) return launch_rows_post<2, 2, 2, 2, 16>(a, vec, 0, flops, s);
    return launch_rows_post<2, 2, 2, 2, 32>(a, vec, 0, flops, s);
  }
  if (a.prec == 0) a.prec = g_gemm_prec;
  if (a.prec == 2) a.prec = 0;
  if (a.prec == 4 || (a.prec == 3 && options().planes)) {
    hipError_t pe = hipSuccess;
    if (planes_try_rows(a, b_kc, a.prec == 4 ? 2 : 3, flops, s, &pe)) return pe;
    if (a.prec == 4) a.prec = 0;
  }
  if (!(b_kc && vec)) a.prec = 0;
  if (a.colstats_rows) *a.colstats_rows = 0;
  if (!a.colstats_rows || a.prec != 0 || a.sumsq || a.N <= 32 || waste160 < waste128 || a.ksplit > 1) a.colstats = nullptr;
  if (a.sumsq) {
    if (a.N > 128) return hipErrorInvalidValue;
    a.sumsq_cap = rows_gemm_sumsq_blocks(a.M);
    ProfScope ps(0, flops, s);
    if (a.N <= 32) return (options().ng_bk & 1) ? launch_rows_sumsq<4, 1, 1, 1, 64>(a, b_kc, vec, s) : launch_rows_sumsq<4, 1, 1, 1, 32>(a, b_kc, vec, s);
    if (a.N <= 64 && a.N > 32 && (options().ng_bk & 8) == 0) return launch_rows_sumsq<4, 1, 1, 2, 32>(a, b_kc, vec, s);
    if (a.N <= 96 && a.N > 64 && ((options().ng_bk & 4) || ktot >= 2048)) return launch_rows_sumsq<2, 2, 2, 2, 32>(a, b_kc, vec, s);
    if (a.N <= 96) return (options().ng_bk & 2) ? launch_rows_sumsq<4, 1, 1, 3, 32>(a, b_kc, vec, s) : launch_rows_sumsq<4, 1, 1, 3, 16>(a, b_kc, vec, s);
    return launch_rows_sumsq<2, 2, 2, 2, 32>(a, b_kc, vec, s);
  }
  if (a.N <= 32 && a.M >= 1024) {
    ProfScope ps(0, flops, s);
    return (options().ng_bk & 1) ? launch_rows<4, 1, 1, 1, 64>(a, b_kc, vec, s) : launch_rows<4, 1, 1, 1, 32>(a, b_kc, vec, s);
  }
  if (waste160 < waste128) return launch_rows_balanced<4, 1, 1, 5, 16>(a, b_kc, vec, 1, flops, s);
  {
    const long long tiles128 = (long long)((a.M + 127) / 128) * ((a.N + 127) / 128);
    const bool small = tiles128 < 768;
    if (small && a.prec == 0 && !a.sumsq) return launch_rows_balanced<2, 2, 1, 2, 16>(a, b_kc, vec, 0, flops, s);
    if ((ktot <= 512 && a.prec == 0) || a.prec == 3) return launch_rows_balanced<2, 2, 2, 2, 16>(a, b_kc, vec, 0, flops, s);
  }
  return launch_rows_balanced<2, 2, 2, 2, 32>(a, b_kc, vec, 0, flops, s);
}

struct RowsGemmGroup {
  std::vector<RowsGemmArgs> args;
  std::vector<int> first;
  RowsGemmArgs *d_args = nullptr;
  int *d_first = nullptr;
  int capacity = 0;
};
void rows_gemm_group_destroy(RowsGemmGroup *g) {
  if (!g) return;
  if (g->d_args) hipFree(g->d_args);
  if (g->d_first) hipFree(g->d_first);
  delete g;
}
bool rows_gemm_group_ok(const RowsGemmArgs &a) {
  if (a.M <= 0 || a.N <= 0 || a.N > 32 || !a.sumsq || a.nseg <= 0 || a.ksplit > 1 || a.colstats || a.add) return false;
  return operands_vec4(a);
}
hipError_t rows_gemm_group(const std::vector<RowsGemmArgs> &calls, RowsGemmGroup **cache, hipStream_t s) {
  if (calls.empty()) return hipSuccess;
  if (!*cache) *cache = new RowsGemmGroup();
  RowsGemmGroup &g = **cache;
  std::vector<RowsGemmArgs> prep(calls.size());
  std::vector<int> first(calls.size() + 1, 0);
  double flops = 0, bytes = 0;
  for (size_t i = 0; i < calls.size(); i++) {
    RowsGemmArgs a = calls[i];
    if (!rows_gemm_group_ok(a)) return hipErrorInvalidValue;
    a.c_vec = aligned16(a.C) && a.ldc % 4 == 0 && (a.init_mode != 1 || aligned16(a.bias));
    a.sumsq_cap = rows_gemm_sumsq_blocks(a.M);
    a.serial_epilogue = 0;
    a.ksplit = 0;
    a.partial = nullptr;
    a.prec = 0;
    a.colstats = nullptr;
    a.colstats_rows = nullptr;
    a.alt_seg_order = options().gemm_alt_taps && is_two_tap_shift(a);
    prep[i] = a;
    first[i + 1] = first[i] + (a.M + 127) / 128;
    const double kt = (double)k_range(a).ktot;
    flops += 2.0 * a.M * a.N * kt;
    bytes += 4.0 * ((double)a.M * kt + kt * a.N + (double)a.M * a.N);
  }
  const bool same = g.args.size() == prep.size() && memcmp(g.args.data(), prep.data(), sizeof(RowsGemmArgs) * prep.size()) == 0 && g.first == first;
  if (!same) {
    if (g.capacity < (int)prep.size()) {
      if (g.d_args) hipFree(g.d_args);
      if (g.d_first) hipFree(g.d_first);
      hipError_t e = hipMalloc((void **)&g.d_args, sizeof(RowsGemmArgs) * prep.size());
      if (e != hipSuccess) return e;
      e = hipMalloc((void **)&g.d_first, sizeof(int) * (prep.size() + 1));
      if (e != hipSuccess) return e;
      g.capacity = (int)prep.size();
    }
    g.args = prep;
    g.first = first;
    hipError_t e = hipMemcpyAsync(g.d_args, g.args.data(), sizeof(RowsGemmArgs) * prep.size(), hipMemcpyHostToDevice, s);
    if (e != hipSuccess) return e;
    e = hipMemcpyAsync(g.d_first, g.first.data(), sizeof(int) * first.size(), hipMemcpyHostToDevice, s);
    if (e != hipSuccess) return e;
  }
  constexpr size_t lds = rows_lds_bytes<128, 32, 32>(true);
  ProfGemmRange prof(3, flops, bytes, s);
  RowsGemmTasks t{g.d_args, g.d_first, (int)prep.size()};
  hipLaunchKernelGGL((rows_gemm_group_kernel<4, 1, 1, 1, 32, true, 4>), dim3(first.back()), dim3(256), lds, s, t);
  return hipGetLastError();
}

}
```

tdnn-f_nas_amd/csrc/rows_gemm_kernels.h:

```cpp
#pragma once
#include "common.h"
#include "gemm_dev.h"
#include "gemm_f32.h"

namespace tdnnf {
namespace {

__device__ __forceinline__ void post_store4(const RowsGemmArgs &p, int m, int n, float4 v, float4 pre, float4 addv) {
  v.x += pre.x; v.y += pre.y; v.z += pre.z; v.w += pre.w;
  if (!p.post_add) { v.x += p.add_scale * addv.x; v.y += p.add_scale * addv.y; v.z += p.add_scale * addv.z; v.w += p.add_scale * addv.w; }
  if (p.relu) { v.x = floor_keep_nan(v.x, 0.f); v.y = floor_keep_nan(v.y, 0.f); v.z = floor_keep_nan(v.z, 0.f); v.w = floor_keep_nan(v.w, 0.f); }
  const float4 sc = p.col_scale ? *reinterpret_cast<const float4 *>(p.col_scale + n) : make_float4(1.f, 1.f, 1.f, 1.f);
  const float4 of = p.col_offset ? *reinterpret_cast<const float4 *>(p.col_offset + n) : make_float4(0.f, 0.f, 0.f, 0.f);
  const float as = p.post_add ? p.add_scale : 0.f;
  v.x = sc.x * v.x + of.x + as * addv.x;
  v.y = sc.y * v.y + of.y + as * addv.y;
  v.z = sc.z * v.z + of.z + as * addv.z;
  v.w = sc.w * v.w + of.w + as * addv.w;
  const int mo = p.row_map ? p.row_map[m] : m;
  if (mo >= 0) *reinterpret_cast<float4 *>(p.C + (long long)mo * p.ldc + n) = v;
}
__device__ __forceinline__ void post_store1(const RowsGemmArgs &p, int m, int n, float x) {
  if (p.init_mode == 1) x += p.bias[n];
  const float a = (p.add && m >= p.add_lo && m < p.add_hi) ? p.add[(long long)(m - p.add_lo) * p.ldadd + n] : 0.f;
  if (!p.post_add) x += p.add_scale * a;
  if (p.relu) x = floor_keep_nan(x, 0.f);
  x = (p.col_scale ? p.col_scale[n] : 1.f) * x + (p.col_offset ? p.col_offset[n] : 0.f) + (p.post_add ? p.add_scale * a : 0.f);
  const int mo = p.row_map ? p.row_map[m] : m;
  if (mo >= 0) p.C[(long long)mo * p.ldc + n] = x;
}

template <int WM, int WN, int TM, int TN, int BK, bool B_KC, int VEC, bool POST = false>
__device__ __forceinline__ void rows_gemm_block(const RowsGemmArgs &p, int ntm, int ntn, int bx, int gx) {
  constexpr int BM = WM * TM * 32, BN = WN * TN * 32;
  constexpr int LDAS = BK + 4;
  constexpr int LDBS = B_KC ? BK + 4 : BN + 4;
  constexpr int A_TILE = BM * LDAS;
  constexpr int B_TILE = B_KC ? BN * LDBS : BK * LDBS;
  constexpr int A_F4 = (BM * BK / 4 + 255) / 256;
  constexpr int B_F4 = (BN * BK / 4 + 255) / 256;
  constexpr int KF4 = BK / 4;
  extern __shared__ __attribute__((aligned(16))) float smem[];
  float *As = smem;
  float *Bs = smem + 2 * A_TILE;

  const int nblk = ntm * ntn;
  int bid = bx;
  {
    const int q = nblk / 8, r = nblk % 8, xcd = bid % 8, j = bid / 8;
    bid = (xcd < r ? xcd * (q + 1) : r * (q + 1) + (xcd - r) * q) + j;
  }
  int sp = 0;
  if (p.ksplit > 1) {
    sp = bx % p.ksplit;
    bid = bx / p.ksplit;
  }
  const long long k_begin = (long long)sp * p.kchunk, k_end = p.ksplit > 1 ? k_begin + p.kchunk : (1LL << 60);
  const int tile_m = bid / ntn, tile_n = bid % ntn;
  const int m0 = tile_m * BM, n0 = tile_n * BN;
  const int t = threadIdx.x, lane = t & 63, wave = t >> 6;
  const int wm = wave / WN, wn = wave % WN;
  const int li = lane & 31, lh = lane >> 5;

  f32x16 acc[TM][TN];
#pragma unroll
  for (int a = 0; a < TM; a++)
#pragma unroll
    for (int b = 0; b < TN; b++)
#pragma unroll
      for (int r = 0; r < 16; r++) acc[a][b][r] = 0.f;

  const bool rev_seg = p.alt_seg_order && (tile_m & 1);
  int seg = -1, sgi = 0, kc = 0, klen = 0;
  long long seg_kstart = 0, seg_knext = 0;
  float cf = 1.f;
  auto next_seg = [&]() {
    for (++seg; seg < p.nseg; ++seg) {
      sgi = rev_seg ? p.nseg - 1 - seg : seg;
      seg_kstart = seg_knext;
      seg_knext += p.seg[sgi].klen;
      cf = p.coef ? p.coef[sgi] : 1.f;
      const long long lo = k_begin > seg_kstart ? k_begin - seg_kstart : 0;
      const long long hi = k_end < seg_knext ? k_end - seg_kstart : p.seg[sgi].klen;
      if (cf != 0.f && hi > lo) {
        kc = (int)lo;
        klen = (int)hi;
        return;
      }
    }
    kc = 0;
    klen = 0;
  };
  next_seg();

  float4 ra[A_F4], rb[B_F4];
  float cf_tile = 1.f;
  float ssq = 0.f;
  auto add_ssq = [&]() {
    float q0 = 0.f, q1 = 0.f;
#pragma unroll
    for (int j = 0; j < A_F4; j++) {
      asm volatile("v_fmac_f32 %0, %2, %2\n v_fmac_f32 %1, %3, %3\n v_fmac_f32 %0, %4, %4\n v_fmac_f32 %1, %5, %5"
                   : "+v"(q0), "+v"(q1)
                   : "v"(ra[j].x), "v"(ra[j].y), "v"(ra[j].z), "v"(ra[j].w));
    }
    ssq += cf_tile * cf_tile * (q0 + q1);
  };
  const float *aptr[A_F4], *bptr[B_F4];
  int astep[A_F4], bstep[B_F4];
  int ptr_seg = -1;
  auto setup_ptrs = [&]() {
    const GemmSeg sg = p.seg[sgi];
    const float *zero = reinterpret_cast<const float *>(&g_zero4);
#pragma unroll
    for (int j = 0; j < A_F4; j++) {
      const int idx = t + 256 * j, row = idx / KF4, m = m0 + row;
      const bool rv = (BM * BK / 4 % 256 == 0 || idx < BM * BK / 4) && m < p.M && m >= sg.m_lo && m < sg.m_hi;
      aptr[j] = rv ? p.A + sg.a_off + (long long)m * p.lda + (idx % KF4) * 4 : zero;
      astep[j] = rv ? 1 : 0;
    }
#pragma unroll
    for (int j = 0; j < B_F4; j++) {
      const int idx = t + 256 * j;
      bool rv;
      if (B_KC) {
        const int n = n0 + idx / KF4;
        rv = (BN * BK / 4 % 256 == 0 || idx < BN * BK / 4) && n < p.N;
        bptr[j] = rv ? p.B + sg.b_off + (long long)n * p.ldb + (idx % KF4) * 4 : zero;
        bstep[j] = rv ? 1 : 0;
      } else {
        const int kr = idx / (BN / 4), n = n0 + (idx % (BN / 4)) * 4;
        rv = (BN * BK / 4 % 256 == 0 || idx < BN * BK / 4) && n + 3 < p.N;
        bptr[j] = rv ? p.B + sg.b_off + (long long)kr * p.ldb + n : zero;
        bstep[j] = rv ? (int)p.ldb : 0;
      }
    }
    ptr_seg = seg;
  };
  const bool fast_ok = VEC == 4 && (B_KC || p.N % 4 == 0);
  auto load_tile = [&]() {
    if (fast_ok && kc + BK <= klen) {
      if (ptr_seg != seg) setup_ptrs();
#pragma unroll
      for (int j = 0; j < A_F4; j++) ra[j] = *reinterpret_cast<const float4 *>(aptr[j] + (long long)kc * astep[j]);
#pragma unroll
      for (int j = 0; j < B_F4; j++) rb[j] = *reinterpret_cast<const float4 *>(bptr[j] + (long long)kc * bstep[j]);
      cf_tile = cf;
      return;
    }
    const GemmSeg sg = p.seg[sgi];
    const float *Ab = p.A + sg.a_off;
    const float *Bb = p.B + sg.b_off;
#pragma unroll
    for (int j = 0; j < A_F4; j++) {
      const int idx = t + 256 * j;
      const int row = idx / KF4, k = kc + (idx % KF4) * 4;
      const int m = m0 + row;
      const bool rv = (BM * BK / 4 % 256 == 0 || idx < BM * BK / 4) && m < p.M && m >= sg.m_lo && m < sg.m_hi;
      const float *ptr = Ab + (long long)m * p.lda + k;
      ra[j] = ld4(ptr, rv && k < klen, rv && k + 1 < klen, rv && k + 2 < klen, rv && k + 3 < klen, VEC == 4);
    }
    if (B_KC) {
#pragma unroll
      for (int j = 0; j < B_F4; j++) {
        const int idx = t + 256 * j;
        const int row = idx / KF4, k = kc + (idx % KF4) * 4;
        const int n = n0 + row;
        const bool rv = (BN * BK / 4 % 256 == 0 || idx < BN * BK / 4) && n < p.N;
        const float *ptr = Bb + (long long)n * p.ldb + k;
        rb[j] = ld4(ptr, rv && k < klen, rv && k + 1 < klen, rv && k + 2 < klen, rv && k + 3 < klen, VEC == 4);
      }
    } else {
      constexpr int NF4 = BN / 4;
#pragma unroll
      for (int j = 0; j < B_F4; j++) {
        const int idx = t + 256 * j;
        const int kr = idx / NF4, n = n0 + (idx % NF4) * 4;
        const bool rv = (BN * BK / 4 % 256 == 0 || idx < BN * BK / 4) && kc + kr < klen;
        const float *ptr = Bb + (long long)(kc + kr) * p.ldb + n;
        rb[j] = ld4(ptr, rv && n < p.N, rv && n + 1 < p.N, rv && n + 2 < p.N, rv && n + 3 < p.N, VEC == 4);
      }
    }
    cf_tile = cf;
  };
  auto store_tile = [&](int buf) {
    float *as = As + buf * A_TILE, *bs = Bs + buf * B_TILE;
    if (p.sumsq) add_ssq();
    if (p.coef) {
#pragma unroll
      for (int j = 0; j < B_F4; j++) {
        rb[j].x *= cf_tile; rb[j].y *= cf_tile; rb[j].z *= cf_tile; rb[j].w *= cf_tile;
      }
    }
#pragma unroll
    for (int j = 0; j < A_F4; j++) {
      const int idx = t + 256 * j;
      if (BM * BK / 4 % 256 == 0 || idx < BM * BK / 4)
        *reinterpret_cast<float4 *>(as + (idx / KF4) * LDAS + (idx % KF4) * 4) = ra[j];
    }
#pragma unroll
    for (int j = 0; j < B_F4; j++) {
      const int idx = t + 256 * j;
      if (BN * BK / 4 % 256 == 0 || idx < BN * BK / 4) {
        if (B_KC)
          *reinterpret_cast<float4 *>(bs + (idx / KF4) * LDBS + (idx % KF4) * 4) = rb[j];
        else
          *reinterpret_cast<float4 *>(bs + (idx / (BN / 4)) * LDBS + (idx % (BN / 4)) * 4) = rb[j];
      }
    }
  };
  auto compute = [&](int buf) {
    const float *as = As + buf * A_TILE + (wm * TM * 32 + li) * LDAS + lh * 4;
    const float *bs = B_KC ? Bs + buf * B_TILE + (wn * TN * 32 + li) * LDBS + lh * 4
                           : Bs + buf * B_TILE + (lh * 4) * LDBS + wn * TN * 32 + li;
#pragma unroll
    for (int kg = 0; kg < BK / 8; kg++) {
      float4 a[TM], b[TN];
#pragma unroll
      for (int i = 0; i < TM; i++) a[i] = *reinterpret_cast<const float4 *>(as + i * 32 * LDAS + kg * 8);
#pragma unroll
      for (int i = 0; i < TN; i++) {
        if (B_KC) {
          b[i] = *reinterpret_cast<const float4 *>(bs + i * 32 * LDBS + kg * 8);
        } else {
          const float *q = bs + (kg * 8) * LDBS + i * 32;
          b[i] = make_float4(q[0], q[LDBS], q[2 * LDBS], q[3 * LDBS]);
        }
      }
#pragma unroll
      for (int i = 0; i < TM; i++)
#pragma unroll
        for (int j = 0; j < TN; j++) {
          acc[i][j] = __builtin_amdgcn_mfma_f32_32x32x2f32(a[i].x, b[j].x, acc[i][j], 0, 0, 0);
          acc[i][j] = __builtin_amdgcn_mfma_f32_32x32x2f32(a[i].y, b[j].y, acc[i][j], 0, 0, 0);
          acc[i][j] = __builtin_amdgcn_mfma_f32_32x32x2f32(a[i].z, b[j].z, acc[i][j], 0, 0, 0);
          acc[i][j] = __builtin_amdgcn_mfma_f32_32x32x2f32(a[i].w, b[j].w, acc[i][j], 0, 0, 0);
        }
    }
  };

  if (seg < p.nseg) {
    load_tile();
    store_tile(0);
    __syncthreads();
    int buf = 0;
    while (true) {
      kc += BK;
      if (kc >= klen) next_seg();
      const bool more = seg < p.nseg;
      if (more) load_tile();
      compute(buf);
      if (!more) break;
      store_tile(buf ^ 1);
      __syncthreads();
      buf ^= 1;
    }
  }

  constexpr int LDCS = BN + 4;
  constexpr int SMEM_FLOATS = 2 * (A_TILE + B_TILE);
  constexpr int HALF = (BM * LDCS <= SMEM_FLOATS) ? BM : ((BM / 2) * LDCS <= SMEM_FLOATS ? BM / 2 : BM / 4);
  static_assert(HALF * LDCS <= SMEM_FLOATS, "epilogue tile does not fit the staging LDS");
  static_assert(HALF % (TM * 32) == 0, "a wave's rows must not straddle epilogue passes");
  float *Cs = smem;
  const bool cvec = p.c_vec != 0;
  __syncthreads();
  if (p.sumsq) {
    double v = ssq;
    for (int o = 32; o > 0; o >>= 1) v += __shfl_xor(v, o, 64);
    double *red = reinterpret_cast<double *>(smem);
    if (lane == 0) red[wave] = v;
    __syncthreads();
    if (t == 0) p.sumsq[p.ksplit > 1 ? bx : bid] = (red[0] + red[1]) + (red[2] + red[3]);
    if (bx == 0)
      for (int i = gx + t; i < p.sumsq_cap; i += 256) p.sumsq[i] = 0.0;
    __syncthreads();
  }
  constexpr bool kColStats = 256 % (BN / 4) == 0 && (HALF * (BN / 4)) % 256 == 0;
  const bool colstats = kColStats && p.colstats && p.ksplit <= 1;
  float cs[4] = {0.f, 0.f, 0.f, 0.f}, cq[4] = {0.f, 0.f, 0.f, 0.f};
#pragma unroll
  for (int pass = 0; pass < BM / HALF; pass++) {
    if ((wm * TM * 32) / HALF == pass) {
#pragma unroll
      for (int i = 0; i < TM; i++)
#pragma unroll
        for (int j = 0; j < TN; j++)
#pragma unroll
          for (int r = 0; r < 16; r++) {
            const int row = (wm * TM + i) * 32 + (r & 3) + 8 * (r >> 2) + 4 * lh - pass * HALF;
            Cs[row * LDCS + (wn * TN + j) * 32 + li] = acc[i][j][r];
          }
    }
    constexpr int kSeg = HALF * (BN / 4) / 256;
    constexpr int kGrp = kSeg % 8 == 0 ? 8 : (kSeg % 5 == 0 ? 5 : (kSeg % 4 == 0 ? 4 : (kSeg % 2 == 0 ? 2 : 1)));
    constexpr bool kFastShape = (HALF * (BN / 4)) % 256 == 0;
    const bool fast_tile = kFastShape && cvec && p.ksplit <= 1 && !p.serial_epilogue && m0 + BM <= p.M && n0 + BN <= p.N;
    if (fast_tile) {
      __syncthreads();
#pragma unroll
      for (int g = 0; g < kSeg; g += kGrp) {
        float4 pre[kGrp], addv[kGrp];
        const float *zero = reinterpret_cast<const float *>(&g_zero4);
#pragma unroll
        for (int u = 0; u < kGrp; u++) {
          const int idx = t + 256 * (g + u), m = m0 + pass * HALF + idx / (BN / 4), n = n0 + (idx % (BN / 4)) * 4;
          const float *pp = p.init_mode == 0 ? p.C + (long long)m * p.ldc + n : (p.init_mode == 1 ? p.bias + n : zero);
          const float *pa = (p.add && m >= p.add_lo && m < p.add_hi) ? p.add + (long long)(m - p.add_lo) * p.ldadd + n : zero;
          pre[u] = *reinterpret_cast<const float4 *>(pp);
          addv[u] = *reinterpret_cast<const float4 *>(pa);
        }
#pragma unroll
        for (int u = 0; u < kGrp; u++) {
          const int idx = t + 256 * (g + u), row = idx / (BN / 4), c4 = (idx % (BN / 4)) * 4;
          const int m = m0 + pass * HALF + row, n = n0 + c4;
          float4 v = *reinterpret_cast<const float4 *>(Cs + row * LDCS + c4);
          if constexpr (POST) {
            post_store4(p, m, n, v, pre[u], addv[u]);
            continue;
          }
          v.x += pre[u].x + p.add_scale * addv[u].x;
          v.y += pre[u].y + p.add_scale * addv[u].y;
          v.z += pre[u].z + p.add_scale * addv[u].z;
          v.w += pre[u].w + p.add_scale * addv[u].w;
          if (p.relu) { v.x = floor_keep_nan(v.x, 0.f); v.y = floor_keep_nan(v.y, 0.f); v.z = floor_keep_nan(v.z, 0.f); v.w = floor_keep_nan(v.w, 0.f); }
          *reinterpret_cast<float4 *>(p.C + (long long)m * p.ldc + n) = v;
          if (kColStats && colstats) {
            cs[0] += v.x; cs[1] += v.y; cs[2] += v.z; cs[3] += v.w;
            cq[0] += v.x * v.x; cq[1] += v.y * v.y; cq[2] += v.z * v.z; cq[3] += v.w * v.w;
          }
        }
      }
      if (pass + 1 < BM / HALF) __syncthreads();
      continue;
    }
    __syncthreads();
    for (int idx = t; idx < HALF * (BN / 4); idx += 256) {
      const int row = idx / (BN / 4), c4 = (idx % (BN / 4)) * 4;
      const int m = m0 + pass * HALF + row, n = n0 + c4;
      if (m >= p.M || n >= p.N) continue;
      float4 v = *reinterpret_cast<const float4 *>(Cs + row * LDCS + c4);
      if (p.ksplit > 1) {
        const int ldp = (p.N + 3) & ~3;
        *reinterpret_cast<float4 *>(p.partial + ((long long)sp * p.M + m) * ldp + n) = v;
        continue;
      }
      if constexpr (POST) {
        if (cvec && n + 3 < p.N) {
          const float4 z = make_float4(0.f, 0.f, 0.f, 0.f);
          const float4 b = p.init_mode == 1 ? *reinterpret_cast<const float4 *>(p.bias + n) : z;
          const float4 o = (p.add && m >= p.add_lo && m < p.add_hi) ? *reinterpret_cast<const float4 *>(p.add + (long long)(m - p.add_lo) * p.ldadd + n) : z;
          post_store4(p, m, n, v, b, o);
        } else {
          const float vv[4] = {v.x, v.y, v.z, v.w};
#pragma unroll
          for (int e = 0; e < 4; e++)
            if (n + e < p.N) post_store1(p, m, n + e, vv[e]);
        }
        continue;
      }
      float *c = p.C + (long long)m * p.ldc + n;
      if (cvec && n + 3 < p.N) {
        if (p.init_mode == 1) {
          const float4 b = *reinterpret_cast<const float4 *>(p.bias + n);
          v.x += b.x; v.y += b.y; v.z += b.z; v.w += b.w;
        } else if (p.init_mode == 0) {
          const float4 o = *reinterpret_cast<const float4 *>(c);
          v.x += o.x; v.y += o.y; v.z += o.z; v.w += o.w;
        }
        if (p.add && m >= p.add_lo && m < p.add_hi) {
          const float4 o = *reinterpret_cast<const float4 *>(p.add + (long long)(m - p.add_lo) * p.ldadd + n);
          v.x += p.add_scale * o.x; v.y += p.add_scale * o.y; v.z += p.add_scale * o.z; v.w += p.add_scale * o.w;
        }
        if (p.relu) { v.x = floor_keep_nan(v.x, 0.f); v.y = floor_keep_nan(v.y, 0.f); v.z = floor_keep_nan(v.z, 0.f); v.w = floor_keep_nan(v.w, 0.f); }
        *reinterpret_cast<float4 *>(c) = v;
        if (colstats) {
          cs[0] += v.x; cs[1] += v.y; cs[2] += v.z; cs[3] += v.w;
          cq[0] += v.x * v.x; cq[1] += v.y * v.y; cq[2] += v.z * v.z; cq[3] += v.w * v.w;
        }
      } else {
        const float vv[4] = {v.x, v.y, v.z, v.w};
#pragma unroll
        for (int e = 0; e < 4; e++) {
          if (n + e < p.N) {
            float x = vv[e];
            if (p.init_mode == 1) x += p.bias[n + e];
            else if (p.init_mode == 0) x += c[e];
            if (p.add && m >= p.add_lo && m < p.add_hi) x += p.add_scale * p.add[(long long)(m - p.add_lo) * p.ldadd + n + e];
            if (p.relu) x = floor_keep_nan(x, 0.f);
            c[e] = x;
            if (colstats) { cs[e] += x; cq[e] += x * x; }
          }
        }
      }
    }
    if (pass + 1 < BM / HALF) __syncthreads();
  }
  if (kColStats && colstats) {
    constexpr int G = BN / 4;
    __syncthreads();
    float *red = smem;
#pragma unroll
    for (int e = 0; e < 4; e++) {
      red[((t / G) * BN + (t % G) * 4 + e) * 2] = cs[e];
      red[((t / G) * BN + (t % G) * 4 + e) * 2 + 1] = cq[e];
    }
    __syncthreads();
    if (t < BN && n0 + t < p.N) {
      float a0 = 0.f, a1 = 0.f;
#pragma unroll
      for (int g = 0; g < 256 / G; g++) {
        a0 += red[(g * BN + t) * 2];
        a1 += red[(g * BN + t) * 2 + 1];
      }
      p.colstats[(long long)tile_m * p.N + n0 + t] = a0;
      p.colstats[((long long)p.colstats_stride + tile_m) * p.N + n0 + t] = a1;
    }
  }
}

template <int WM, int WN, int TM, int TN, int BK, bool B_KC, int VEC, int TAG = 0>
__global__ __launch_bounds__(256) void rows_gemm_kernel(const RowsGemmArgs p, int ntm, int ntn) {
  rows_gemm_block<WM, WN, TM, TN, BK, B_KC, VEC>(p, ntm, ntn, (int)blockIdx.x, (int)gridDim.x);
}
template <int WM, int WN, int TM, int TN, int BK, int VEC>
__global__ __launch_bounds__(256) void rows_gemm_post_kernel(const RowsGemmArgs p, int ntm, int ntn) {
  rows_gemm_block<WM, WN, TM, TN, BK, true, VEC, true>(p, ntm, ntn, (int)blockIdx.x, (int)gridDim.x);
}
struct RowsGemmTasks {
  const RowsGemmArgs *args;
  const int *first;
  int ntasks;
};
template <int WM, int WN, int TM, int TN, int BK, bool B_KC, int VEC>
__global__ __launch_bounds__(256) void rows_gemm_group_kernel(RowsGemmTasks g) {
  int lo = 0, hi = g.ntasks;
  while (hi - lo > 1) {
    const int mid = (lo + hi) >> 1;
    if ((int)blockIdx.x >= g.first[mid]) lo = mid;
    else hi = mid;
  }
  const int b0 = g.first[lo], nb = g.first[lo + 1] - b0;
  rows_gemm_block<WM, WN, TM, TN, BK, B_KC, VEC>(g.args[lo], nb, 1, (int)blockIdx.x - b0, nb);
}

template <int WM, int WN, int TM, int TN, int BK, int NP, int D, int TAG = 0>
__global__ __launch_bounds__(256, 2) void rows_gemm_x3_kernel(const RowsGemmArgs p, int ntm, int ntn) {
  constexpr int VEC = 4;
  constexpr bool B_KC = true;
  constexpr int BM = WM * TM * 32, BN = WN * TN * 32;
  constexpr int LDH = BK + 8;
  constexpr int A_TILE = NP * BM * LDH / 2;
  constexpr int B_TILE = NP * BN * LDH / 2;
  constexpr int A_F4 = (BM * BK / 4 + 255) / 256;
  constexpr int B_F4 = (BN * BK / 4 + 255) / 256;
  constexpr int KF4 = BK / 4;
  extern __shared__ __attribute__((aligned(16))) float smem[];
  float *As = smem;
  float *Bs = smem + 2 * A_TILE;

  const int nblk = ntm * ntn;
  int bid = blockIdx.x;
  {
    const int q = nblk / 8, r = nblk % 8, xcd = bid % 8, j = bid / 8;
    bid = (xcd < r ? xcd * (q + 1) : r * (q + 1) + (xcd - r) * q) + j;
  }
  int sp = 0;
  if (p.ksplit > 1) {
    sp = blockIdx.x % p.ksplit;
    bid = blockIdx.x / p.ksplit;
  }
  const long long k_begin = (long long)sp * p.kchunk, k_end = p.ksplit > 1 ? k_begin + p.kchunk : (1LL << 60);
  const int tile_m = bid / ntn, tile_n = bid % ntn;
  const int m0 = tile_m * BM, n0 = tile_n * BN;
  const int t = threadIdx.x, lane = t & 63, wave = t >> 6;
  const int wm = wave / WN, wn = wave % WN;
  const int li = lane & 31, lh = lane >> 5;

  f32x16 acc[TM][TN];
#pragma unroll
  for (int a = 0; a < TM; a++)
#pragma unroll
    for (int b = 0; b < TN; b++)
#pragma unroll
      for (int r = 0; r < 16; r++) acc[a][b][r] = 0.f;

  int seg = -1, kc = 0, klen = 0;
  long long seg_kstart = 0, seg_knext = 0;
  float cf = 1.f;
  auto next_seg = [&]() {
    for (++seg; seg < p.nseg; ++seg) {
      seg_kstart = seg_knext;
      seg_knext += p.seg[seg].klen;
      cf = p.coef ? p.coef[seg] : 1.f;
      const long long lo = k_begin > seg_kstart ? k_begin - seg_kstart : 0;
      const long long hi = k_end < seg_knext ? k_end - seg_kstart : p.seg[seg].klen;
      if (cf != 0.f && hi > lo) {
        kc = (int)lo;
        klen = (int)hi;
        return;
      }
    }
    kc = 0;
    klen = 0;
  };
  next_seg();

  float4 ra[D][A_F4], rb[D][B_F4];
  float cf_tile[D];
  float ssq = 0.f;
  auto add_ssq = [&](const float4 (&xa)[A_F4], float c) {
    float q = 0.f;
#pragma unroll
    for (int j = 0; j < A_F4; j++) q += xa[j].x * xa[j].x + xa[j].y * xa[j].y + xa[j].z * xa[j].z + xa[j].w * xa[j].w;
    ssq += c * c * q;
  };
  const float *aptr[A_F4], *bptr[B_F4];
  int astep[A_F4], bstep[B_F4];
  int ptr_seg = -1;
  auto setup_ptrs = [&]() {
    const GemmSeg sg = p.seg[seg];
    const float *zero = reinterpret_cast<const float *>(&g_zero4);
#pragma unroll
    for (int j = 0; j < A_F4; j++) {
      const int idx = t + 256 * j, row = idx / KF4, m = m0 + row;
      const bool rv = (BM * BK / 4 % 256 == 0 || idx < BM * BK / 4) && m < p.M && m >= sg.m_lo && m < sg.m_hi;
      aptr[j] = rv ? p.A + sg.a_off + (long long)m * p.lda + (idx % KF4) * 4 : zero;
      astep[j] = rv ? 1 : 0;
    }
#pragma unroll
    for (int j = 0; j < B_F4; j++) {
      const int idx = t + 256 * j;
      bool rv;
      if (B_KC) {
        const int n = n0 + idx / KF4;
        rv = (BN * BK / 4 % 256 == 0 || idx < BN * BK / 4) && n < p.N;
        bptr[j] = rv ? p.B + sg.b_off + (long long)n * p.ldb + (idx % KF4) * 4 : zero;
        bstep[j] = rv ? 1 : 0;
      } else {
        const int kr = idx / (BN / 4), n = n0 + (idx % (BN / 4)) * 4;
        rv = (BN * BK / 4 % 256 == 0 || idx < BN * BK / 4) && n + 3 < p.N;
        bptr[j] = rv ? p.B + sg.b_off + (long long)kr * p.ldb + n : zero;
        bstep[j] = rv ? (int)p.ldb : 0;
      }
    }
    ptr_seg = seg;
  };
  const bool fast_ok = VEC == 4 && (B_KC || p.N % 4 == 0);
  auto load_tile = [&](float4 (&ra)[A_F4], float4 (&rb)[B_F4], float &cf_tile) {
    if (fast_ok && kc + BK <= klen) {
      if (ptr_seg != seg) setup_ptrs();
#pragma unroll
      for (int j = 0; j < A_F4; j++) ra[j] = *reinterpret_cast<const float4 *>(aptr[j] + (long long)kc * astep[j]);
#pragma unroll
      for (int j = 0; j < B_F4; j++) rb[j] = *reinterpret_cast<const float4 *>(bptr[j] + (long long)kc * bstep[j]);
      cf_tile = cf;
      return;
    }
    const GemmSeg sg = p.seg[seg];
    const float *Ab = p.A + sg.a_off;
    const float *Bb = p.B + sg.b_off;
#pragma unroll
    for (int j = 0; j < A_F4; j++) {
      const int idx = t + 256 * j;
      const int row = idx / KF4, k = kc + (idx % KF4) * 4;
      const int m = m0 + row;
      const bool rv = (BM * BK / 4 % 256 == 0 || idx < BM * BK / 4) && m < p.M && m >= sg.m_lo && m < sg.m_hi;
      const float *ptr = Ab + (long long)m * p.lda + k;
      ra[j] = ld4(ptr, rv && k < klen, rv && k + 1 < klen, rv && k + 2 < klen, rv && k + 3 < klen, VEC == 4);
    }
    if (B_KC) {
#pragma unroll
      for (int j = 0; j < B_F4; j++) {
        const int idx = t + 256 * j;
        const int row = idx / KF4, k = kc + (idx % KF4) * 4;
        const int n = n0 + row;
// ... 226 lines not shown
```

Baseline: 1.622 million.

## Fuse BatchNorm-ReLU backward column reductions into the backprop-data GEMM epilogue

Adds a BNB epilogue variant of the rows GEMM that computes the five per-column partial sums needed by BatchNorm/ReLU backward (z*d, d, d^2, x, x>0) while the input-derivative tile is still in registers/LDS. The separate bn_relu_bwd reduce pass over x and dz is then skipped, and the finalize step consumes the per-tile partials. This removes one full read of the activation derivative. In exchange the GEMM epilogue reads the relu output, uses more registers and LDS, and is only enabled for large, aligned, non-split-k shapes. It is on by default via a new option.

```diff
diff --git a/include/tdnnf_hip.h b/include/tdnnf_hip.h
--- a/include/tdnnf_hip.h
+++ b/include/tdnnf_hip.h
@@ -52,6 +52,14 @@
 int tdnnf_tdnn_backprop_data(const tdnnf_tdnn_indexes *indexes, const tdnnf_mat *out_deriv,
                              const float *linear_params_dev, int ldw, int Do, int Di,
                              const float *eff_coef_dev, tdnnf_mat *in_deriv, tdnnf_stream stream);
+
+size_t tdnnf_bn_relu_backward_workspace_bytes(int rows, int cols);
+int tdnnf_tdnn_backprop_data_bn_relu(const tdnnf_tdnn_indexes *indexes, const tdnnf_mat *out_deriv,
+                                     const float *linear_params_dev, int ldw, int Do, int Di, int overwrite,
+                                     const tdnnf_mat *add, float add_scale, int add_lo, tdnnf_mat *in_deriv,
+                                     const tdnnf_mat *relu_out, float *memo_dev, double *relu_stats_dev, int store_relu_stats,
+                                     tdnnf_mat *d_aff, float *bias_acc_dev, void *workspace_dev, size_t workspace_bytes,
+                                     double *sums_out_dev, int *fused_out, tdnnf_stream stream);
 
 size_t tdnnf_tdnn_update_workspace_bytes(int Do, int Di, int K, int num_rows);
 int tdnnf_tdnn_update_simple(const tdnnf_tdnn_indexes *indexes, const tdnnf_mat *in_value,
diff --git a/tdnn-f_nas_amd/csrc/abi_tdnn.hip b/tdnn-f_nas_amd/csrc/abi_tdnn.hip
--- a/tdnn-f_nas_amd/csrc/abi_tdnn.hip
+++ b/tdnn-f_nas_amd/csrc/abi_tdnn.hip
@@ -80,7 +80,7 @@
   Options &o = options();
   if (!name) return nullptr;
   const struct { const char *n; int *p; } table[] = {{"ng_grouped", &o.ng_grouped}, {"ng_fuse", &o.ng_fuse}, {"ng_early_in", &o.ng_early_in},
-                                                     {"wgrad_stream", &o.wgrad_stream}, {"gemm_ring", &o.gemm_ring}, {"planes", &o.planes}, {"den_split", &o.den_split}, {"phase_events", &o.phase_events}, {"wgrad_lag", &o.wgrad_lag}, {"ng_bk", &o.ng_bk}, {"ng_valu", &o.ng_valu}, {"ng_pform", &o.ng_pform}, {"planes_group", &o.planes_group}, {"xent_behind_den", &o.xent_behind_den}, {"ng_early_fork", &o.ng_early_fork}, {"ng_diag_skip", &o.ng_diag_skip}, {"wgrad_small", &o.wgrad_small}, {"splitk_per_cu", &o.splitk_per_cu}, {"gemm_alt_taps", &o.gemm_alt_taps}, {"reverse_passes", &o.reverse_passes}, {"splitk_partial_round", &o.splitk_partial_round}, {"wgrad_on_caller", &o.wgrad_on_caller}, {"den_mw_test_abort", &o.den_mw_test_abort}, {"planes_check_bound", &o.planes_check_bound}, {"den_gamma_pairs", &o.den_gamma_pairs}, {"num_form", &o.num_form}, {"num_frontier_cap", &o.num_frontier_cap}};
+                                                     {"wgrad_stream", &o.wgrad_stream}, {"gemm_ring", &o.gemm_ring}, {"planes", &o.planes}, {"den_split", &o.den_split}, {"phase_events", &o.phase_events}, {"wgrad_lag", &o.wgrad_lag}, {"ng_bk", &o.ng_bk}, {"ng_valu", &o.ng_valu}, {"ng_pform", &o.ng_pform}, {"planes_group", &o.planes_group}, {"xent_behind_den", &o.xent_behind_den}, {"ng_early_fork", &o.ng_early_fork}, {"ng_diag_skip", &o.ng_diag_skip}, {"wgrad_small", &o.wgrad_small}, {"splitk_per_cu", &o.splitk_per_cu}, {"gemm_alt_taps", &o.gemm_alt_taps}, {"reverse_passes", &o.reverse_passes}, {"splitk_partial_round", &o.splitk_partial_round}, {"wgrad_on_caller", &o.wgrad_on_caller}, {"den_mw_test_abort", &o.den_mw_test_abort}, {"planes_check_bound", &o.planes_check_bound}, {"den_gamma_pairs", &o.den_gamma_pairs}, {"num_form", &o.num_form}, {"num_frontier_cap", &o.num_frontier_cap}, {"bn_bwd_epilogue", &o.bn_bwd_epilogue}};
   for (auto &e : table)
     if (strcmp(e.n, name) == 0) return e.p;
   return nullptr;
@@ -151,12 +151,13 @@
 namespace tdnnf {
 int tdnn_backprop_data_impl(const tdnnf_tdnn_indexes *ix, const tdnnf_mat *out_deriv, const float *W, int ldw, int Do,
                             int Di, const float *eff_coef, int overwrite, const tdnnf_mat *add, float add_scale, int add_lo,
-                            tdnnf_mat *in_deriv, tdnnf_stream stream) {
+                            tdnnf_mat *in_deriv, tdnnf_stream stream, const BnbEpilogue *bnb) {
   TDNNF_REQUIRE(mat_ok(in_deriv) && mat_ok(out_deriv) && W, "tdnn_backprop_data: bad matrices");
   TDNNF_REQUIRE(Do > 0 && Di > 0 && in_deriv->cols == Di && out_deriv->cols == Do, "tdnn_backprop_data: bad dims");
   TDNNF_REQUIRE(tdnn_rows_ok(ix, in_deriv->rows, out_deriv->rows), "tdnn_backprop_data: in_deriv has too few rows for the time offsets");
   TDNNF_REQUIRE(ldw >= ix->num_offsets * Di, "tdnn_backprop_data: ldw < K*Di");
   const int rho = ix->row_stride, N = out_deriv->rows, K = ix->num_offsets;
+  if (bnb && bnb->chunks) *bnb->chunks = 0;
   if (N == 0) return TDNNF_OK;
   for (int cls = 0; cls < rho; cls++) {
     RowsGemmArgs a;
@@ -211,6 +212,10 @@
     if (!eff_coef || contiguous) {
       a.coef = eff_coef ? eff_coef + seg_tap[0] : nullptr;
       a.nseg = nseg;
+      if (bnb && rho == 1 && u_max == in_deriv->rows) {
+        a.bnb_x = bnb->x; a.bnb_ldx = bnb->ldx; a.bnb_mean = bnb->mean; a.bnb_scale = bnb->scale;
+        a.bnb_partial = bnb->partial; a.bnb_chunks = bnb->chunks;
+      }
       TDNNF_HIP(rows_gemm(a, WT != nullptr, (hipStream_t)stream));
     } else {
       for (int s = 0; s < nseg; s++) {
diff --git a/tdnn-f_nas_amd/csrc/common.h b/tdnn-f_nas_amd/csrc/common.h
--- a/tdnn-f_nas_amd/csrc/common.h
+++ b/tdnn-f_nas_amd/csrc/common.h
@@ -68,6 +68,7 @@
   int den_split = -1;
   int num_form = 0;
   int num_frontier_cap = 0;
+  int bn_bwd_epilogue = 1;
   int den_gamma_pairs = 0;
 };
 Options &options();
@@ -198,8 +199,15 @@
 int tdnn_update_simple_impl(const tdnnf_tdnn_indexes *ix, const tdnnf_mat *in_value, const tdnnf_mat *out_deriv, int Do, int Di,
                             const float *eff_coef, float lr, float *W_acc, int ldw, float *bias_acc, void *ws, size_t ws_bytes,
                             const int *active_dev, int max_active, tdnnf_stream stream, bool overwrite = false);
+struct BnbEpilogue {
+  const float *x;
+  long long ldx;
+  const float *mean, *scale;
+  float *partial;
+  int *chunks;
+};
 int tdnn_backprop_data_impl(const tdnnf_tdnn_indexes *ix, const tdnnf_mat *out_deriv, const float *W, int ldw, int Do, int Di,
                             const float *eff_coef, int overwrite, const tdnnf_mat *add, float add_scale, int add_lo,
-                            tdnnf_mat *in_deriv, tdnnf_stream stream);
-
-}
+                            tdnnf_mat *in_deriv, tdnnf_stream stream, const BnbEpilogue *bnb = nullptr);
+
+}
diff --git a/tdnn-f_nas_amd/csrc/fused.h b/tdnn-f_nas_amd/csrc/fused.h
--- a/tdnn-f_nas_amd/csrc/fused.h
+++ b/tdnn-f_nas_amd/csrc/fused.h
@@ -34,6 +34,10 @@
                        void *ws, size_t ws_bytes, hipStream_t s, const float *mask = nullptr, int B = 1,
                        const NgFuse *ng = nullptr,
                        double *oderiv_stats = nullptr,
-                       const BwdPlanes *planes = nullptr);
+                       const BwdPlanes *planes = nullptr,
+                       int epi_chunks = 0,
+                       double *sums_out = nullptr);
+hipError_t bn_relu_bwd_reduce_rows(MatView x, MatView dz, const float *mean, const float *scale, int rows_per_chunk, int chunk_stride, float *partial,
+                                   hipStream_t s);
 
 }
diff --git a/tdnn-f_nas_amd/csrc/fused.hip b/tdnn-f_nas_amd/csrc/fused.hip
--- a/tdnn-f_nas_amd/csrc/fused.hip
+++ b/tdnn-f_nas_amd/csrc/fused.hip
@@ -453,42 +453,59 @@
 size_t bn_relu_bwd_workspace_bytes(int rows, int cols) {
   ColReducePlan p = colreduce_plan(rows, cols);
   const size_t blocks128 = ((size_t)rows + 127) / 128;
-  return sizeof(float) * (5 * (size_t)p.chunks + std::max((size_t)p.chunks, blocks128)) * cols + 64;
+  return sizeof(float) * 6 * std::max((size_t)p.chunks, blocks128) * cols + 64;
+}
+
+hipError_t bn_relu_bwd_reduce_rows(MatView x, MatView dz, const float *mean, const float *scale, int rows_per_chunk, int chunk_stride, float *partial,
+                                   hipStream_t s) {
+  if (x.rows <= 0) return hipSuccess;
+  if (!(vec4_ok(x) && vec4_ok(dz)) || rows_per_chunk < 1) return hipErrorInvalidValue;
+  const dim3 grid((x.cols + 255) / 256, (x.rows + rows_per_chunk - 1) / rows_per_chunk);
+  hipLaunchKernelGGL((bn_relu_bwd_reduce_kernel<4, true>), grid, dim3(256), 0, s, x, dz, mean, scale, rows_per_chunk, chunk_stride, partial, (const float *)nullptr, 1);
+  return hipGetLastError();
 }
 
 hipError_t bn_relu_bwd(MatView x, MatView dz, float *memo, float target_rms, bool bn_test_mode, double *relu_stats, bool store_relu_stats,
                        bool self_repair, float self_repair_scale, MatView d_aff, float *bias_acc, float bias_scale,
-                       void *ws, size_t ws_bytes, hipStream_t s, const float *mask, int B, const NgFuse *ng, double *oderiv_stats, const BwdPlanes *planes) {
+                       void *ws, size_t ws_bytes, hipStream_t s, const float *mask, int B, const NgFuse *ng, double *oderiv_stats, const BwdPlanes *planes,
+                       int epi_chunks, double *sums_out) {
   if (x.rows == 0) return hipSuccess;
   if (ws_bytes < bn_relu_bwd_workspace_bytes(x.rows, x.cols)) return hipErrorInvalidValue;
+  if (epi_chunks && (mask || epi_chunks != (x.rows + 127) / 128)) return hipErrorInvalidValue;
   if (ng && (!bn_relu_bwd_ng_ok(x, dz, d_aff, ng->Rp) || (reinterpret_cast<uintptr_t>(memo) & 15) || (reinterpret_cast<uintptr_t>(ng->W) & 15) || ng->ldw % 4))
     return hipErrorInvalidValue;
   const int D = x.cols;
-  ProfHbmRange prof(5, 4.0 * x.rows * x.cols * 5.0, s);
+  ProfHbmRange prof(5, 4.0 * x.rows * x.cols * (epi_chunks ? 3.0 : 5.0), s);
   ColReducePlan pl = colreduce_plan(x.rows, D);
+  const int fin_chunks = epi_chunks ? epi_chunks : pl.chunks;
   const bool vec = vec4_ok(x) && vec4_ok(dz) && vec4_ok(d_aff);
   const int per = vec ? 256 : 64;
   dim3 grid((D + per - 1) / per, pl.chunks), block(256);
   float *partial = (float *)ws;
-  float *bias_partial = partial + 5 * (size_t)pl.chunks * D;
-  if (store_relu_stats) {
+  float *bias_partial = partial + 5 * (size_t)fin_chunks * D;
+  if (epi_chunks) {
+  } else if (store_relu_stats) {
     if (vec) hipLaunchKernelGGL((bn_relu_bwd_reduce_kernel<4, true>), grid, block, 0, s, x, dz, memo, memo + 2 * D, pl.rows_per_chunk, pl.chunks, partial, mask, B);
     else hipLaunchKernelGGL((bn_relu_bwd_reduce_kernel<1, true>), grid, block, 0, s, x, dz, memo, memo + 2 * D, pl.rows_per_chunk, pl.chunks, partial, mask, B);
   } else {
     if (vec) hipLaunchKernelGGL((bn_relu_bwd_reduce_kernel<4, false>), grid, block, 0, s, x, dz, memo, memo + 2 * D, pl.rows_per_chunk, pl.chunks, partial, mask, B);
     else hipLaunchKernelGGL((bn_relu_bwd_reduce_kernel<1, false>), grid, block, 0, s, x, dz, memo, memo + 2 * D, pl.rows_per_chunk, pl.chunks, partial, mask, B);
   }
+  if (sums_out)
+    hipLaunchKernelGGL(bn_relu_bwd_finalize_kernel, dim3(finalize_grid(D)), dim3(kFinThreads), 0, s, partial, fin_chunks, D, x.rows, target_rms, memo,
+                       store_relu_stats ? sums_out : (double *)nullptr , 0,
+                       (double *)nullptr, sums_out, (const double *)nullptr, 0);
   double *fro2 = fro_bound_buf();
   if (fro2 && fro_bound_blocks()) *fro_bound_blocks() = (int)finalize_grid(D);
   const float repair_abs = self_repair ? 2.0f * fabsf(self_repair_scale) : 0.f;
   if (BnSync *sy = bn_test_mode ? nullptr : bn_sync_current()) {
-    hipLaunchKernelGGL(bn_relu_bwd_finalize_kernel, dim3(finalize_grid(D)), dim3(kFinThreads), 0, s, partial, pl.chunks, D, x.rows, target_rms, memo,
+    hipLaunchKernelGGL(bn_relu_bwd_finalize_kernel, dim3(finalize_grid(D)), dim3(kFinThreads), 0, s, partial, fin_chunks, D, x.rows, target_rms, memo,
                        store_relu_stats ? relu_stats : (double *)nullptr, 0, (double *)nullptr, sy->buf, (const double *)nullptr, 0);
     if (sy->fn(sy->ctx, sy->buf, 3LL * D, (tdnnf_stream)s)) return hipErrorUnknown;
-    hipLaunchKernelGGL(bn_relu_bwd_finalize_kernel, dim3(finalize_grid(D)), dim3(kFinThreads), 0, s, partial, pl.chunks, D, x.rows * sy->world, target_rms, memo,
+    hipLaunchKernelGGL(bn_relu_bwd_finalize_kernel, dim3(finalize_grid(D)), dim3(kFinThreads), 0, s, partial, fin_chunks, D, x.rows * sy->world, target_rms, memo,
                        store_relu_stats ? relu_stats : (double *)nullptr, 0, oderiv_stats, (double *)nullptr, (const double *)sy->buf, x.rows, fro2, repair_abs);
   } else {
-    hipLaunchKernelGGL(bn_relu_bwd_finalize_kernel, dim3(finalize_grid(D)), dim3(kFinThreads), 0, s, partial, pl.chunks, D, x.rows, target_rms, memo,
+    hipLaunchKernelGGL(bn_relu_bwd_finalize_kernel, dim3(finalize_grid(D)), dim3(kFinThreads), 0, s, partial, fin_chunks, D, x.rows, target_rms, memo,
                        store_relu_stats ? relu_stats : (double *)nullptr, bn_test_mode ? 1 : 0, oderiv_stats, (double *)nullptr, (const double *)nullptr, 0, fro2,
                        repair_abs);
   }
@@ -526,3 +543,28 @@
 }
 
 }
+
+using namespace tdnnf;
+
+extern "C" {
+
+size_t tdnnf_bn_relu_backward_workspace_bytes(int rows, int cols) { return bn_relu_bwd_workspace_bytes(rows, cols); }
+
+int tdnnf_tdnn_backprop_data_bn_relu(const tdnnf_tdnn_indexes *ix, const tdnnf_mat *out_deriv, const float *W, int ldw, int Do, int Di, int overwrite,
+                                     const tdnnf_mat *add, float add_scale, int add_lo, tdnnf_mat *in_deriv, const tdnnf_mat *relu_out, float *memo,
+                                     double *relu_stats, int store_relu_stats, tdnnf_mat *d_aff, float *bias_acc, void *ws, size_t ws_bytes,
+                                     double *sums_out, int *fused_out, tdnnf_stream stream) {
+  TDNNF_REQUIRE(mat_ok(in_deriv) && mat_ok(relu_out) && mat_ok(d_aff) && memo && relu_stats && ws, "tdnn_backprop_data_bn_relu: bad arguments");
+  TDNNF_REQUIRE(same_dim(in_deriv, relu_out) && same_dim(in_deriv, d_aff) && in_deriv->cols == Di, "tdnn_backprop_data_bn_relu: in_deriv, relu_out and d_aff must have one shape");
+  TDNNF_REQUIRE(ws_bytes >= bn_relu_bwd_workspace_bytes(in_deriv->rows, Di), "tdnn_backprop_data_bn_relu: workspace too small");
+  int chunks = 0;
+  const BnbEpilogue be{relu_out->data, relu_out->stride, memo, memo + 2 * Di, (float *)ws, &chunks};
+  int rc = tdnn_backprop_data_impl(ix, out_deriv, W, ldw, Do, Di, nullptr, overwrite, add, add_scale, add_lo, in_deriv, stream, &be);
+  if (rc != TDNNF_OK) return rc;
+  if (fused_out) *fused_out = chunks;
+  TDNNF_HIP(bn_relu_bwd(view(relu_out), view(in_deriv), memo, 1.0f, false, relu_stats, store_relu_stats != 0, false, 0.f, view(d_aff), bias_acc, 1.0f, ws, ws_bytes,
+                        (hipStream_t)stream, nullptr, 1, nullptr, nullptr, nullptr, chunks, sums_out));
+  return TDNNF_OK;
+}
+
+}
diff --git a/tdnn-f_nas_amd/csrc/gemm_f32.h b/tdnn-f_nas_amd/csrc/gemm_f32.h
--- a/tdnn-f_nas_amd/csrc/gemm_f32.h
+++ b/tdnn-f_nas_amd/csrc/gemm_f32.h
@@ -52,6 +52,12 @@
   const float *col_offset;
   int post_add;
   const int *row_map;
+  const float *bnb_x;
+  long long bnb_ldx;
+  const float *bnb_mean, *bnb_scale;
+  float *bnb_partial;
+  int *bnb_chunks;
+  int bnb_stride;
 };
 inline bool rows_gemm_has_post(const RowsGemmArgs &a) { return a.col_scale || a.col_offset || a.post_add || a.row_map; }
 
diff --git a/tdnn-f_nas_amd/csrc/net_step.hip b/tdnn-f_nas_amd/csrc/net_step.hip
--- a/tdnn-f_nas_amd/csrc/net_step.hip
+++ b/tdnn-f_nas_amd/csrc/net_step.hip
@@ -301,6 +301,7 @@
   PlanesOperand po_next;
   float *prev = nullptr;
   int fused_comp = -1;
+  int bnb_chunks = 0;
   bool den_joined = false;
   bool caller_used = false;
   float *d_cur = n->dA, *d_next = n->dB;
@@ -757,6 +758,8 @@
                        int relu_index, const float *mask, FroBound *fb, PlanesOperand *po) {
     const bool store = coin() || step == 0;
     const bool repair = c.relu_self_repair_scale > 0.f && coin();
+    const int epi_chunks = bnb_chunks;
+    bnb_chunks = 0;
     tdnnf_mat x = M(relu_out, d_in.rows, Hd);
     NgFuse f;
     const int fuse = out_stats_fuse(comp, view(&x), view(&d_in), view(&d_out), f);
@@ -766,7 +769,7 @@
     PlanesOperand tmp;
     CK(bwd_planes(d_out, lead, &bp, &tmp));
     TDNNF_HIP(bn_relu_bwd(view(&x), view(&d_in), memo, 1.0f, cv, relu_stats, store, repair, c.relu_self_repair_scale, view(&d_out), bias_acc, 1.0f,
-                          n->ws, n->ws_bytes, s, mask, B, fuse ? &f : nullptr, oderiv_of(relu_stats, relu_index), bp.P ? &bp : nullptr));
+                          n->ws, n->ws_bytes, s, mask, B, fuse ? &f : nullptr, oderiv_of(relu_stats, relu_index), bp.P ? &bp : nullptr, epi_chunks));
     if (bp.P) *po = tmp;
     if (bp.P && options().planes_check_bound) TDNNF_HIP(planes_check_bound(view(&d_out), bp.rec, n->planes_ws, s));
     return TDNNF_OK;
@@ -1095,8 +1098,15 @@
     tdnnf_mat d_byp = sub_grid_view(d_next, L.gin, L.gout, B, Hd);
     if (d_byp.rows == d_out.rows) {
       const int row0 = (int)((d_byp.data - d_in.data) / d_in.stride);
+      BnbEpilogue be{nullptr, 0, nullptr, nullptr, nullptr, nullptr};
+      const bool cover = l > 0 && options().bn_bwd_epilogue != 0 && !cv && !pl_on && c.gemm_precision == 0 && !L.lin.darts && !lin_eff && c.bn_num_choices <= 0 &&
+                         !mask_of(l) && n->layers[l - 1].aff.rows_out == ni && n->ws_bytes >= bn_relu_bwd_workspace_bytes(ni, Hd);
+      if (cover) {
+        const tdnnf_mat xr = M(n->layers[l - 1].relu_out, ni, Hd);
+        be = BnbEpilogue{xr.data, xr.stride, n->layers[l - 1].bn_memo, n->layers[l - 1].bn_memo + 2 * Hd, (float *)n->ws, &bnb_chunks};
+      }
       CK(tdnn_backprop_data_impl(&L.lin.ix, &d_lin, net_W(n, L.lin.comp), L.lin.K * Hd, L.bn, Hd, lin_eff, 1, &d_out, c.bypass_scale, row0,
-                                 &d_in, s));
+                                 &d_in, s, cover ? &be : nullptr));
     } else {
       CK(tdnn_backprop_data_impl(&L.lin.ix, &d_lin, net_W(n, L.lin.comp), L.lin.K * Hd, L.bn, Hd, lin_eff, 1, nullptr, 0.f, 0, &d_in, s));
       tdnnf_mat d_o = tdnnf_mat{d_cur, L.gout.n, d_byp.cols, B * ldpad(Hd)};
diff --git a/tdnn-f_nas_amd/csrc/rows_gemm.hip b/tdnn-f_nas_amd/csrc/rows_gemm.hip
--- a/tdnn-f_nas_amd/csrc/rows_gemm.hip
+++ b/tdnn-f_nas_amd/csrc/rows_gemm.hip
@@ -4,6 +4,7 @@
 
 #include "common.h"
 #include "device.h"
+#include "fused.h"
 #include "gemm_f32.h"
 #include "gemm_ring.h"
 #include "planes_gemm.h"
@@ -77,9 +78,23 @@
     else hipLaunchKernelGGL((rows_gemm_kernel<WM, WN, TM, TN, BK, false, 1, TAG>), grid, block, lds_nc, s, a, ntm, ntn);
   }
 }
+constexpr bool kBnbTile(int WM, int WN, int TM, int TN, int BK) { return WM == 2 && WN == 2 && TM == 2 && TN == 2 && BK == 16; }
+void launch_rows_kernel_bnb(dim3 grid, const RowsGemmArgs &a, int ntm, int ntn, bool b_kc, hipStream_t s) {
+  constexpr size_t lds_kc = rows_lds_bytes<128, 128, 16>(true), lds_nc = rows_lds_bytes<128, 128, 16>(false);
+  static const bool opted = opt_in_lds(rows_gemm_bnb_kernel<true>, lds_kc) && opt_in_lds(rows_gemm_bnb_kernel<false>, lds_nc);
+  (void)opted;
+  if (b_kc) hipLaunchKernelGGL((rows_gemm_bnb_kernel<true>), grid, dim3(256), lds_kc, s, a, ntm, ntn);
+  else hipLaunchKernelGGL((rows_gemm_bnb_kernel<false>), grid, dim3(256), lds_nc, s, a, ntm, ntn);
+}
 template <int WM, int WN, int TM, int TN, int BK>
 void launch_rows_kernel(dim3 grid, const RowsGemmArgs &a, int ntm, int ntn, bool b_kc, bool vec, hipStream_t s) {
   const bool ng = prof_class_override() == 3;
+  if constexpr (kBnbTile(WM, WN, TM, TN, BK)) {
+    if (a.bnb_partial && a.ksplit <= 1) {
+      launch_rows_kernel_bnb(grid, a, ntm, ntn, b_kc, s);
+      return;
+    }
+  }
   if (a.prec == 1 && b_kc && vec) {
     if (ng) launch_rows_x3_tagged<WM, WN, TM, TN, BK, 2, 1>(grid, a, ntm, ntn, s);
     else launch_rows_x3_tagged<WM, WN, TM, TN, BK, 2, 0>(grid, a, ntm, ntn, s);
@@ -119,6 +134,7 @@
   at.kchunk = (int)(((kt + S - 1) / S) * BK);
   at.ksplit = (int)((ktot + at.kchunk - 1) / at.kchunk);
   at.partial = scratch;
+  at.bnb_partial = nullptr;
   launch_rows_kernel<WM, WN, TM, TN, BK>(dim3(ntm * ntn * at.ksplit), at, ntm, ntn, b_kc, vec, s);
   const long long total = (long long)at.M * at.N;
   hipLaunchKernelGGL(splitk_reduce_kernel, dim3((unsigned)std::min<long long>((total + 255) / 256, 2048)), dim3(256), 0, s, at);
@@ -164,12 +180,14 @@
   const int tiles = ntm * ntn;
   const int q = tiles / slots, r = tiles % slots;
   const bool stats = a.colstats != nullptr;
+  const bool bnb = a.bnb_partial != nullptr;
+  if (bnb) *a.bnb_chunks = ntm;
   const auto [ktot, k4] = k_range(a);
   const int main_mt = (q * slots) / ntn;
   float *scratch = nullptr;
   size_t scratch_bytes = 0;
   int S_partial = 0;
-  if (!stats && q == 0 && tiles * 4 > slots && k4 && options().splitk_partial_round) {
+  if (!stats && !bnb && q == 0 && tiles * 4 > slots && k4 && options().splitk_partial_round) {
     const int cus = device_cus();
     const long long kt = (ktot + BK - 1) / BK;
     double best = (double)((tiles + cus - 1) / cus);
@@ -182,7 +200,7 @@
       }
     }
   }
-  if (!stats && (tiles * 4 <= slots || S_partial >= 2) && k4 && ktot >= 16 * BK && (scratch = splitk_scratch(&scratch_bytes))) {
+  if (!stats && !bnb && (tiles * 4 <= slots || S_partial >= 2) && k4 && ktot >= 16 * BK && (scratch = splitk_scratch(&scratch_bytes))) {
     const long long kt = (ktot + BK - 1) / BK;
     int S = S_partial >= 2 ? S_partial : slots / tiles;
     if (S_partial < 2 && options().splitk_per_cu == 1) S = std::max(2, device_cus() / tiles);
@@ -209,6 +227,7 @@
       am.colstats_stride = main_mt + (tail_split ? tail_plan.chunks : (tail_rows + BM - 1) / BM);
       *a.colstats_rows = am.colstats_stride;
     }
+    am.bnb_stride = ntm;
     {
       ProfScope ps(cls, flops * m_main / a.M, s);
       hipError_t e = launch_rows<WM, WN, TM, TN, BK>(am, b_kc, vec, s);
@@ -227,6 +246,11 @@
     if (stats) {
       at.colstats = a.colstats + (long long)main_mt * a.N;
       at.colstats_stride = am.colstats_stride;
+    }
+    if (bnb) {
+      at.bnb_x = a.bnb_x + (long long)m_main * a.bnb_ldx;
+      at.bnb_partial = a.bnb_partial + (long long)main_mt * a.N;
+      at.bnb_stride = ntm;
     }
     if (tail_split) {
       {
@@ -238,19 +262,24 @@
         hipError_t e = colreduce_partial_into(1, ct, ct, tail_plan.chunks, tail_plan.rows_per_chunk, am.colstats_stride, at.colstats, s);
         if (e != hipSuccess) return e;
       }
+      if (bnb) {
+        const MatView xt{const_cast<float *>(at.bnb_x), at.M, at.N, (int)at.bnb_ldx}, ct{at.C, at.M, at.N, (int)at.ldc};
+        hipError_t e = bn_relu_bwd_reduce_rows(xt, ct, a.bnb_mean, a.bnb_scale, BM, ntm, at.bnb_partial, s);
+        if (e != hipSuccess) return e;
+      }
       return hipGetLastError();
     }
     ProfScope ps(cls, flops * at.M / a.M, s);
     return launch_rows<WM, WN, TM, TN, BK>(at, b_kc, vec, s);
   }
   ProfScope ps(cls, flops, s);
+  RowsGemmArgs as = a;
+  as.bnb_stride = ntm;
   if (stats) {
-    RowsGemmArgs as = a;
     as.colstats_stride = ntm;
     *a.colstats_rows = ntm;
-    return launch_rows<WM, WN, TM, TN, BK>(as, b_kc, vec, s);
-  }
-  return launch_rows<WM, WN, TM, TN, BK>(a, b_kc, vec, s);
+  }
+  return launch_rows<WM, WN, TM, TN, BK>(as, b_kc, vec, s);
 }
 
 template <int WM, int WN, int TM, int TN, int BK>
@@ -476,8 +505,9 @@
   const bool vec = operands_vec4(a);
   const int waste128 = ((a.N + 127) / 128) * 128 - a.N, waste160 = ((a.N + 159) / 160) * 160 - a.N;
   const long long ktot = k_range(a).ktot;
-  double flops = 0;
+  double flops = 0, prof_bytes = 0;
   for (int i = 0; i < a.nseg; i++) flops += 2.0 * usable_rows(a.seg[i], a.M) * a.N * a.seg[i].klen;
+  if (a.bnb_chunks) *a.bnb_chunks = 0;
   if (prof_on()) {
     double a_elems = 0, b_elems = 0;
     bool taps = true;
@@ -497,7 +527,8 @@
     }
     double c_elems = (double)a.M * a.N * (a.init_mode == 0 ? 2.0 : 1.0);
     if (a.add) c_elems += (double)(std::min(a.add_hi, a.M) - std::max(a.add_lo, 0)) * a.N;
-    prof_next_gemm(flops, 4.0 * (a_elems + b_elems + c_elems));
+    prof_bytes = 4.0 * (a_elems + b_elems + c_elems);
+    prof_next_gemm(flops, prof_bytes);
   }
   a.serial_epilogue = 0;
   a.alt_seg_order = options().gemm_alt_taps && is_two_tap_shift(a);
@@ -505,6 +536,7 @@
     if (!b_kc || a.init_mode == 0 || a.sumsq || a.ksplit > 1 || (a.init_mode == 1 && !a.bias)) return hipErrorInvalidValue;
     a.prec = 0;
     a.colstats = nullptr;
+    a.bnb_partial = nullptr;
     if (a.colstats_rows) *a.colstats_rows = 0;
     a.c_vec = a.c_vec && (!a.col_scale || aligned16(a.col_scale)) && (!a.col_offset || aligned16(a.col_offset));
     if (waste160 < waste128) return launch_rows_post<4, 1, 1, 5, 16>(a, vec, 1, flops, s);
@@ -519,9 +551,18 @@
     if (planes_try_rows(a, b_kc, a.prec == 4 ? 2 : 3, flops, s, &pe)) return pe;
     if (a.prec == 4) a.prec = 0;
   }
+  const long long tiles128 = (long long)((a.M + 127) / 128) * ((a.N + 127) / 128);
   if (!(b_kc && vec)) a.prec = 0;
   if (a.colstats_rows) *a.colstats_rows = 0;
   if (!a.colstats_rows || a.prec != 0 || a.sumsq || a.N <= 32 || waste160 < waste128 || a.ksplit > 1) a.colstats = nullptr;
+  {
+    const int opt = options().bn_bwd_epilogue;
+    const bool ok = a.bnb_partial && a.bnb_chunks && a.bnb_x && a.bnb_mean && a.bnb_scale && opt != 0 && a.prec == 0 && !a.sumsq && !a.colstats && a.ksplit <= 1 && vec &&
+                    a.c_vec && aligned16(a.bnb_x) && a.bnb_ldx % 4 == 0 && waste160 >= waste128 && a.N > 32 && ktot <= 512 && prof_class_override() != 3 &&
+                    !ring_applies(a, b_kc, vec, 128) && (opt == 2 || tiles128 >= 768);
+    if (!ok) a.bnb_partial = nullptr;
+    else if (prof_on()) prof_next_gemm(flops, prof_bytes + 4.0 * a.M * a.N);
+  }
   if (a.sumsq) {
     if (a.N > 128) return hipErrorInvalidValue;
     a.sumsq_cap = rows_gemm_sumsq_blocks(a.M);
@@ -537,8 +578,8 @@
     return (options().ng_bk & 1) ? launch_rows<4, 1, 1, 1, 64>(a, b_kc, vec, s) : launch_rows<4, 1, 1, 1, 32>(a, b_kc, vec, s);
   }
   if (waste160 < waste128) return launch_rows_balanced<4, 1, 1, 5, 16>(a, b_kc, vec, 1, flops, s);
+  if (a.bnb_partial) return launch_rows_balanced<2, 2, 2, 2, 16>(a, b_kc, vec, 0, flops, s);
   {
-    const long long tiles128 = (long long)((a.M + 127) / 128) * ((a.N + 127) / 128);
     const bool small = tiles128 < 768;
     if (small && a.prec == 0 && !a.sumsq) return launch_rows_balanced<2, 2, 1, 2, 16>(a, b_kc, vec, 0, flops, s);
     if ((ktot <= 512 && a.prec == 0) || a.prec == 3) return launch_rows_balanced<2, 2, 2, 2, 16>(a, b_kc, vec, 0, flops, s);
@@ -581,6 +622,7 @@
     a.prec = 0;
     a.colstats = nullptr;
     a.colstats_rows = nullptr;
+    a.bnb_partial = nullptr;
     a.alt_seg_order = options().gemm_alt_taps && is_two_tap_shift(a);
     prep[i] = a;
     first[i + 1] = first[i] + (a.M + 127) / 128;
diff --git a/tdnn-f_nas_amd/csrc/rows_gemm_kernels.h b/tdnn-f_nas_amd/csrc/rows_gemm_kernels.h
--- a/tdnn-f_nas_amd/csrc/rows_gemm_kernels.h
+++ b/tdnn-f_nas_amd/csrc/rows_gemm_kernels.h
@@ -30,7 +30,7 @@
   if (mo >= 0) p.C[(long long)mo * p.ldc + n] = x;
 }
 
-template <int WM, int WN, int TM, int TN, int BK, bool B_KC, int VEC, bool POST = false>
+template <int WM, int WN, int TM, int TN, int BK, bool B_KC, int VEC, bool POST = false, bool BNB = false>
 __device__ __forceinline__ void rows_gemm_block(const RowsGemmArgs &p, int ntm, int ntn, int bx, int gx) {
   constexpr int BM = WM * TM * 32, BN = WN * TN * 32;
   constexpr int LDAS = BK + 4;
@@ -279,6 +279,34 @@
   constexpr bool kColStats = 256 % (BN / 4) == 0 && (HALF * (BN / 4)) % 256 == 0;
   const bool colstats = kColStats && p.colstats && p.ksplit <= 1;
   float cs[4] = {0.f, 0.f, 0.f, 0.f}, cq[4] = {0.f, 0.f, 0.f, 0.f};
+  static_assert(!BNB || (kColStats && !POST), "the BatchNorm backward sums need a thread's column group fixed over its row segments");
+  float bs[BNB ? 5 : 1][4], bmu[4], bsc[4];
+  if constexpr (BNB) {
+#pragma unroll
+    for (int e = 0; e < 4; e++)
+#pragma unroll
+      for (int q = 0; q < 5; q++) bs[q][e] = 0.f;
+  }
+  auto bnb_cols = [&]() {
+    if constexpr (BNB) {
+#pragma unroll
+      for (int e = 0; e < 4; e++) {
+        const int n = n0 + (t % (BN / 4)) * 4 + e;
+        bmu[e] = n < p.N ? p.bnb_mean[n] : 0.f;
+        bsc[e] = n < p.N ? p.bnb_scale[n] : 0.f;
+      }
+    }
+  };
+  auto bnb_add = [&](int e, float dv, float xv) {
+    if constexpr (BNB) {
+      const float z = (xv - bmu[e]) * bsc[e];
+      bs[0][e] += z * dv;
+      bs[1][e] += dv;
+      bs[2][e] += dv * dv;
+      bs[3][e] += xv;
+      bs[4][e] += xv > 0.f ? 1.f : 0.f;
+    }
+  };
 #pragma unroll
   for (int pass = 0; pass < BM / HALF; pass++) {
     if ((wm * TM * 32) / HALF == pass) {
@@ -293,7 +321,8 @@
           }
     }
     constexpr int kSeg = HALF * (BN / 4) / 256;
-    constexpr int kGrp = kSeg % 8 == 0 ? 8 : (kSeg % 5 == 0 ? 5 : (kSeg % 4 == 0 ? 4 : (kSeg % 2 == 0 ? 2 : 1)));
+    constexpr int kGrpX = kSeg % 8 == 0 ? 8 : (kSeg % 5 == 0 ? 5 : (kSeg % 4 == 0 ? 4 : (kSeg % 2 == 0 ? 2 : 1)));
+    constexpr int kGrp = BNB && kGrpX == 8 ? 4 : kGrpX;
     constexpr bool kFastShape = (HALF * (BN / 4)) % 256 == 0;
     const bool fast_tile = kFastShape && cvec && p.ksplit <= 1 && !p.serial_epilogue && m0 + BM <= p.M && n0 + BN <= p.N;
     if (fast_tile) {
@@ -329,12 +358,32 @@
             cs[0] += v.x; cs[1] += v.y; cs[2] += v.z; cs[3] += v.w;
             cq[0] += v.x * v.x; cq[1] += v.y * v.y; cq[2] += v.z * v.z; cq[3] += v.w * v.w;
           }
+          if constexpr (BNB) *reinterpret_cast<float4 *>(Cs + row * LDCS + c4) = v;
+        }
+      }
+      if constexpr (BNB) {
+        bnb_cols();
+#pragma unroll
+        for (int g = 0; g < kSeg; g += kGrp) {
+          float4 xv[kGrp];
+#pragma unroll
+          for (int u = 0; u < kGrp; u++) {
+            const int idx = t + 256 * (g + u), m = m0 + pass * HALF + idx / (BN / 4), n = n0 + (idx % (BN / 4)) * 4;
+            xv[u] = *reinterpret_cast<const float4 *>(p.bnb_x + (long long)m * p.bnb_ldx + n);
+          }
+#pragma unroll
+          for (int u = 0; u < kGrp; u++) {
+            const int idx = t + 256 * (g + u), row = idx / (BN / 4), c4 = (idx % (BN / 4)) * 4;
+            const float4 v = *reinterpret_cast<const float4 *>(Cs + row * LDCS + c4);
+            bnb_add(0, v.x, xv[u].x); bnb_add(1, v.y, xv[u].y); bnb_add(2, v.z, xv[u].z); bnb_add(3, v.w, xv[u].w);
+          }
         }
       }
       if (pass + 1 < BM / HALF) __syncthreads();
       continue;
     }
     __syncthreads();
+    bnb_cols();
     for (int idx = t; idx < HALF * (BN / 4); idx += 256) {
       const int row = idx / (BN / 4), c4 = (idx % (BN / 4)) * 4;
       const int m = m0 + pass * HALF + row, n = n0 + c4;
@@ -378,6 +427,10 @@
           cs[0] += v.x; cs[1] += v.y; cs[2] += v.z; cs[3] += v.w;
           cq[0] += v.x * v.x; cq[1] += v.y * v.y; cq[2] += v.z * v.z; cq[3] += v.w * v.w;
         }
+        if constexpr (BNB) {
+          const float4 x4 = *reinterpret_cast<const float4 *>(p.bnb_x + (long long)m * p.bnb_ldx + n);
+          bnb_add(0, v.x, x4.x); bnb_add(1, v.y, x4.y); bnb_add(2, v.z, x4.z); bnb_add(3, v.w, x4.w);
+        }
       } else {
         const float vv[4] = {v.x, v.y, v.z, v.w};
 #pragma unroll
@@ -390,6 +443,7 @@
             if (p.relu) x = floor_keep_nan(x, 0.f);
             c[e] = x;
             if (colstats) { cs[e] += x; cq[e] += x * x; }
+            if constexpr (BNB) bnb_add(e, x, p.bnb_x[(long long)m * p.bnb_ldx + n + e]);
           }
         }
       }
@@ -417,11 +471,37 @@
       p.colstats[((long long)p.colstats_stride + tile_m) * p.N + n0 + t] = a1;
     }
   }
+  if constexpr (BNB) {
+    if (p.ksplit <= 1) {
+      constexpr int G = BN / 4, R = 256 / G;
+      static_assert(5 * R * BN <= SMEM_FLOATS, "the BatchNorm backward sums do not fit the staging LDS");
+      __syncthreads();
+      float *red = smem;
+#pragma unroll
+      for (int q = 0; q < 5; q++)
+#pragma unroll
+        for (int e = 0; e < 4; e++) red[(q * R + t / G) * BN + (t % G) * 4 + e] = bs[q][e];
+      __syncthreads();
+      if (t < BN && n0 + t < p.N) {
+#pragma unroll
+        for (int q = 0; q < 5; q++) {
+          float a = 0.f;
+#pragma unroll
+          for (int g = 0; g < R; g++) a += red[(q * R + g) * BN + t];
+          p.bnb_partial[((long long)q * p.bnb_stride + tile_m) * p.N + n0 + t] = a;
+        }
+      }
+    }
+  }
 }
 
 template <int WM, int WN, int TM, int TN, int BK, bool B_KC, int VEC, int TAG = 0>
 __global__ __launch_bounds__(256) void rows_gemm_kernel(const RowsGemmArgs p, int ntm, int ntn) {
   rows_gemm_block<WM, WN, TM, TN, BK, B_KC, VEC>(p, ntm, ntn, (int)blockIdx.x, (int)gridDim.x);
+}
+template <bool B_KC>
+__global__ __launch_bounds__(256, 3) void rows_gemm_bnb_kernel(const RowsGemmArgs p, int ntm, int ntn) {
+  rows_gemm_block<2, 2, 2, 2, 16, B_KC, 4, false, true>(p, ntm, ntn, (int)blockIdx.x, (int)gridDim.x);
 }
 template <int WM, int WN, int TM, int TN, int BK, int VEC>
 __global__ __launch_bounds__(256) void rows_gemm_post_kernel(const RowsGemmArgs p, int ntm, int ntn) {
```

New measurement: 1.636 million (median of 6 runs). Within noise of the previous version (+0.9%).
